# atom501/v-img

Measured on AMD Instinct MI355X. Metric: Mrays/sec (primary+secondary) at 512 spp, higher is better.
Workload: dtype f32; 1 GPU; disney_spheres.json, mis integrator, 512 spp, 1800x800; integrator=mis, spp=512, depth=unbounded, bvh=sweep SAH (host)

## Files before the change

v-img_amd/csrc/device_scene.h:

```cpp
#pragma once
#include <hip/hip_runtime.h>
#include <stdint.h>

#include "../../include/vimg_scene.h"
#include "material_record.h"

namespace vimg {

#define VIMG_GLOBAL __attribute__((address_space(1)))
#define VIMG_LDS __attribute__((address_space(3)))
template <typename T>
using gptr = const VIMG_GLOBAL T*;
typedef float v4f __attribute__((ext_vector_type(4)));
typedef uint32_t v2u __attribute__((ext_vector_type(2)));
typedef uint32_t v4u __attribute__((ext_vector_type(4)));

struct __attribute__((aligned(16))) DNode {
  v4f a;
  v4f b;
  v4f c;
  uint32_t left_ref, right_ref, pad0, pad1;
};
static_assert(sizeof(DNode) == 64, "DNode must be one 64-byte line");

struct __attribute__((aligned(16))) DLeafPrim {
  v4f a, b;
  float c0;
  uint32_t prim;
  uint32_t kind;
  uint32_t cls;
};
static_assert(sizeof(DLeafPrim) == 48, "DLeafPrim must be 48 bytes");

struct __attribute__((aligned(16))) DTriShade {
  float p[9];
  uint32_t mesh;
  uint32_t i0, i1, i2;
  float n[3];
};
static_assert(sizeof(DTriShade) == 64, "DTriShade must be 64 bytes");

struct __attribute__((aligned(16))) DLight {
  v4f a, b, c, d;
  uint32_t kind, index, pad0, pad1;
};
static_assert(sizeof(DLight) == 80, "DLight must be 80 bytes");

struct DScene {
  float cam_to_world[16];
  float p_size0, p_size1;
  float cone_spread;
  float aperture_radius, focal_dist;
  int32_t res_x, res_y;

  float root_min[3], root_max[3];
  uint32_t num_nodes, max_depth;
  uint32_t root_ref;
  gptr<DNode> nodes;
  gptr<DLeafPrim> leaf_prims;

  gptr<VimgPrim> prims;
  gptr<DTriShade> tri_shade;
  gptr<float> tri_area_pdf;
  gptr<VimgMesh> meshes;
  gptr<float> normals;
  gptr<float> uvs;
  gptr<VimgSphere> spheres;
  gptr<VimgMaterial> materials;
  gptr<uint32_t> material_flags;
  gptr<DMaterial> dmaterials;
  gptr<VimgTexture> textures;
  gptr<float> texels;
  gptr<VimgTextureRG> rg_textures;
  gptr<float> rg_texels;
  gptr<VimgLight> lights;
  gptr<DLight> dlights;
  uint32_t num_lights;
  gptr<float> cdf_pool;
  VimgBackground background;
  uint32_t background_emissive;
};

enum : uint32_t {
  MATF_NEEDS_UV = 1u,
  MATF_NEEDS_FRAME = 2u,
};

struct RenderArgs {
  uint32_t integrator, samples, depth;
  uint32_t tile_rank, tile_world;
  uint32_t tiles_x, tiles_y;
  uint32_t num_local_tiles;
  uint32_t full_stats;
  uint32_t stack_entries;
  uint32_t lds_nodes;
  uint32_t stack_lds;
  VIMG_GLOBAL uint32_t* stack_ovf;
  VIMG_GLOBAL v4u* pool_cold;
  uint32_t lds_leaf;
  VIMG_GLOBAL v4u* pool_state;
  uint32_t pool_segments;
  uint32_t pool_seg_len;
  uint32_t pool_epoch;
  uint32_t pool_slots;
  uint32_t pool_refill;
  uint32_t pool_vbatch;
  uint32_t pool_boxmin;
  uint32_t pool_starve;
  uint32_t pool_gbreak;
  uint32_t pool_classes;
  uint32_t cu_walkers;
  uint32_t cu_flex;
  uint32_t cu_lowwater;
  uint32_t cu_patience;
  uint32_t cu_join;
  uint32_t cu_sleep;
  uint32_t cu_watchdog;
  uint32_t cu_magic_v, cu_shift_v;
  uint32_t cu_magic_w, cu_shift_w;
  int32_t single_x, single_y;
  uint32_t sample_base;
  float spp_div;
  const VIMG_GLOBAL v4u* prog_in;
  VIMG_GLOBAL v4u* prog_out;
  const VIMG_GLOBAL uint32_t* item_list;
  uint32_t item_count;
};

struct DeviceStats {
  unsigned long long closest, shadow, internal, leaf, prim, sphere, nan_samples;
  unsigned long long trip_descend, trip_prim, iterations;
  unsigned long long prof[28];
  unsigned long long wait_cyc[5], wait_n[5];
  unsigned long long px_done[3];
  unsigned long long px_hops[3];
  unsigned long long ray_cyc[2];
  unsigned long long pv_cyc[7];
  unsigned long long walk_cyc[4];
};

}
```

v-img_amd/csrc/hip_internal.h:

```cpp
#pragma once
#include <hip/hip_runtime.h>

#include <algorithm>
#include <string>
#include <utility>
#include <vector>

#include "../../include/vimg_hip.h"
#include "device_mem.h"
#include "device_scene.h"
#include "kernel_tus.h"

#pragma GCC visibility push(hidden)
struct VimgDeviceScene {
  vimg::DScene d{};
  vimg::DevBuf nodes, leaf_prims;
  vimg::DevBuf chain_leaf;
  std::vector<vimg::DevBuf> tables;
  size_t total_bytes = 0;
  bool textured = false;
  VimgHipOptions opt{};
  int waves_per_simd = 2;
  bool too_wide = false;
  bool force_general = false;
  uint32_t num_cus = 0;
  uint32_t num_leaf_prims = 0;
  vimg::DevBuf stats;
  vimg::DevBuf counter;
  vimg::DevBuf root_box;
  vimg::DevBuf frame;
  vimg::DevBuf pool_cold;
  vimg::DevBuf stack_ovf;
  vimg::DevBuf pool_state;
  uint32_t pool_epoch = 0;
  uint64_t generation = 0;
  uint32_t num_vertices = 0, num_tris = 0, num_spheres = 0;
  std::vector<std::pair<uint32_t, uint32_t>> normal_rows;
  uint32_t n_internal = 0;
  uint32_t n_chain = 0;
  std::vector<uint32_t> level_begin;
  std::vector<VimgMaterial> materials;
  std::vector<VimgTexture> textures;
  std::vector<VimgLight> lights;
  uint32_t num_rg_textures = 0;
  uint64_t num_texels = 0, num_cdf = 0;
  size_t lights_table = 0, dlights_table = 0, dmaterials_table = 0;
  int query_launch = -1;
  bool query_ready = false;
  vimg::RenderArgs query_args{};
  uint32_t query_lds = 0;
  uint32_t query_per_cu[3] = {0, 0, 0};
};

struct VimgProgressive {
  VimgDeviceScene* scene = nullptr;
  VimgRenderParams params{};
  uint64_t items = 0;
  vimg::DevBuf rec[2];
  int cur = 0;
  uint32_t samples = 0;
  vimg::DevBuf scratch;
  uint64_t generation = 0;
  bool uniform = true;
  uint64_t valid_items = 0;
  uint64_t launches = 0;
  vimg::DevBuf item_list;
  vimg::DevBuf block_counts;
  vimg::DevBuf ctl;
};

namespace vimg {

extern hipStream_t g_stream;
extern int g_device;
inline hipStream_t stream_of(void* stream) { return stream ? static_cast<hipStream_t>(stream) : g_stream; }

inline uint32_t tiles_of(int n) { return (static_cast<uint32_t>(n) + 7u) / 8u; }
uint32_t local_tiles(const VimgDeviceScene* s, const VimgRenderParams* p);
inline bool is_feature_integrator(uint32_t i) { return i >= VIMG_INTEGRATOR_ALBEDO && i <= VIMG_INTEGRATOR_COVERAGE; }
inline uint32_t opt_or(int32_t v, uint32_t dflt) { return v == VIMG_OPT_AUTO ? dflt : static_cast<uint32_t>(v); }

struct LaunchCfg {
  RenderArgs args;
  uint32_t grid, lds_bytes;
  int sched;
  int wps;
  bool deep;
  int cu_waves;
  bool feature;
  size_t cold_bytes;
  size_t ovf_bytes;
};

struct DeviceTree {
  DevBuf nodes, bb, obj_indices;
  uint32_t num_nodes = 0, max_depth = 0;
  std::vector<uint32_t> level_internal;
};
int build_tree_device(uint32_t builder , uint32_t n, const float* d_bounds6, DeviceTree* out);

int validate_materials(const VimgMaterial* materials, uint32_t num_materials, const VimgTexture* textures, uint32_t num_textures,
                       uint32_t num_rg_textures);
int validate_lights(const VimgLight* lights, uint32_t num_lights, uint32_t num_prims);
bool tables_textured(const VimgMaterial* materials, uint32_t num_materials, const VimgTexture* textures, const VimgBackground& bg);
bool background_is_emissive(const VimgBackground& bg);

struct RelightPlan {
  bool any = false;
  DevBuf new_lights, new_dlights;
  DevBuf new_dmaterials;
  DevBuf sin_elev, lum, row_int, row_tot;
  std::vector<float> sin_table;
};
int check_relight(const VimgDeviceScene* s, const VimgGeometryUpdate* u);
int prepare_relight(const VimgDeviceScene* s, const VimgGeometryUpdate* u, RelightPlan* plan);
int enqueue_relight(VimgDeviceScene* s, const VimgGeometryUpdate* u, RelightPlan* plan, hipStream_t st);
void commit_relight(VimgDeviceScene* s, const VimgGeometryUpdate* u, RelightPlan* plan);
int enqueue_material_bake(const DScene& d, uint32_t num_materials, DMaterial* out, hipStream_t st);

struct EnvCdfScratch {
  float* sin_elev;
  float* lum;
  float* row_int;
  float* row_tot;
};
void enqueue_mip_levels(float* texels, const uint64_t* level_offset, uint32_t levels, uint32_t w, uint32_t h, uint32_t wrap_u,
                        uint32_t wrap_v, hipStream_t st);
std::vector<float> env_sin_table(uint32_t h);
void enqueue_env_cdfs(const float* img, uint32_t w, uint32_t h, const EnvCdfScratch& t, float* row_cdf, float* col_cdfs, hipStream_t st);

struct ProgLaunch {
  uint32_t base;
  const void* in;
  void* out;
  const uint32_t* item_list = nullptr;
  uint32_t item_count = 0;
  bool keep_stats = false;
};
int check_params(const VimgDeviceScene* s, const VimgRenderParams* p);
int check_render(const VimgDeviceScene* s, const VimgRenderParams* p, const void* d_out);
struct RenderLaunch {
  float* d_out;
  hipStream_t st;
  bool stats = false;
  int sx = -1, sy = -1;
  hipEvent_t ev0 = nullptr, ev1 = nullptr;
  const ProgLaunch* prog = nullptr;
};
int enqueue_render(VimgDeviceScene* s, const VimgRenderParams* p, const RenderLaunch& r);
int check_kernel_error(VimgDeviceScene* s);
uint64_t fetch_shard_pixels(const VimgDeviceScene* s, const VimgRenderParams* p);
int fetch_stats(VimgDeviceScene* s, const VimgRenderParams* p, VimgRenderStats* out);

LaunchCfg make_launch(const VimgDeviceScene* s, const VimgRenderParams* p, int sx, int sy);
LaunchCfg make_launch_lane(const VimgDeviceScene* s, const VimgRenderParams* p, int sx, int sy);
LaunchCfg make_launch_feature(const VimgDeviceScene* s, const VimgRenderParams* p, int sx, int sy);
RenderArgs base_args(const VimgDeviceScene* s, const VimgRenderParams* p, int sx, int sy);
uint32_t segments_for(const VimgDeviceScene* s, const VimgRenderParams* p, uint64_t items, uint64_t in_flight,
                      double per_gen, double most, RenderArgs* a);
const void* kernel_of(const VimgDeviceScene* s, const LaunchCfg& c);
const void* launched_kernel_of(const VimgDeviceScene* s, const LaunchCfg& c, bool stats);
bool plain_launch_serves(const VimgDeviceScene* s, const LaunchCfg& c, bool stats);

}
#pragma GCC visibility pop
```

v-img_amd/csrc/launch_policy.hip:

```cpp
#include <cmath>

#include "hip_internal.h"
#include "render_cu_kernel.h"

namespace vimg {

uint32_t local_tiles(const VimgDeviceScene* s, const VimgRenderParams* p) {
  const uint32_t total = tiles_of(s->d.res_x) * tiles_of(s->d.res_y);
  if (p->tile_rank >= total) return 0;
  return (total - p->tile_rank + p->tile_world - 1) / p->tile_world;
}

RenderArgs base_args(const VimgDeviceScene* s, const VimgRenderParams* p, int sx, int sy) {
  const VimgHipOptions& o = s->opt;
  RenderArgs a{};
  a.integrator = p->integrator;
  a.samples = p->samples;
  a.spp_div = static_cast<float>(p->samples);
  a.depth = p->depth;
  a.tile_rank = p->tile_rank;
  a.tile_world = p->tile_world;
  a.tiles_x = tiles_of(s->d.res_x);
  a.tiles_y = tiles_of(s->d.res_y);
  a.num_local_tiles = local_tiles(s, p);
  a.full_stats = 0;
  a.single_x = sx;
  a.single_y = sy;
  a.stack_entries = s->d.max_depth + 2;
  a.stack_ovf = nullptr;
  a.pool_refill = 16u;
  a.pool_vbatch = std::min(64u, std::max(1u, opt_or(o.pool_vbatch, 64u)));
  a.pool_boxmin = std::min(64u, opt_or(o.pool_boxmin, 16u));
  a.pool_segments = 1;
  a.pool_seg_len = p->samples;
  return a;
}

uint32_t segments_for(const VimgDeviceScene* s, const VimgRenderParams* p, uint64_t items, uint64_t in_flight,
                      double per_gen, double most, RenderArgs* a) {
  const double gens = double(items) / double(in_flight);
  uint32_t k = gens >= 10.0 ? 1u : uint32_t(std::min(most, std::max(1.0, std::floor(per_gen / gens + 0.5))));
  k = std::min<uint32_t>(k, std::max<uint32_t>(p->samples / 4u, 1u));
  if (items * 2u < in_flight * 3u) k = 1u;
  if (s->opt.pool_segments != VIMG_OPT_AUTO) k = uint32_t(std::max(1, s->opt.pool_segments));
  k = std::min<uint32_t>(k, 4096u);
  while (k > 1u && items * k >= 0xfff00000ull) --k;
  const uint32_t len = std::max<uint32_t>((p->samples + k - 1) / k, 1u);
  a->pool_seg_len = len;
  a->pool_segments = std::max<uint32_t>((p->samples + len - 1) / len, 1u);
  return len;
}

namespace {

CuKernel pick_cu_kernel(const VimgDeviceScene* s, bool deep, int nw, bool diag = false, bool early = false, bool plain = false) {
  if (plain) return early ? vimg_cu_kernel_plain_early() : vimg_cu_kernel_plain();
  return diag ? vimg_cu_kernel_diag(s->textured, deep, nw)
              : (early ? vimg_cu_kernel_early(s->textured, deep, nw) : vimg_cu_kernel(s->textured, deep, nw));
}

void magic_div(uint32_t d, uint32_t* magic, uint32_t* shift) {
  uint32_t l = 0;
  while ((1ull << l) < d) ++l;
  *magic = static_cast<uint32_t>((1ull << (31u + l)) / d + 1ull);
  *shift = l - 1u;
}

LaunchCfg make_launch_cu(const VimgDeviceScene* s, const VimgRenderParams* p, int sx, int sy) {
  LaunchCfg c{};
  const VimgHipOptions& o = s->opt;
  const uint64_t items = (sx >= 0) ? 1 : uint64_t(local_tiles(s, p)) * 64u;
  c.sched = VIMG_SCHED_CU;
  c.wps = 4;
  c.cu_waves = 16;
  const uint32_t nw = uint32_t(c.cu_waves);
  RenderArgs& a = c.args = base_args(s, p, sx, sy);
  a.stack_lds = std::min(a.stack_entries, std::max(1u, opt_or(o.lds_stack, 32u)));
  a.cu_walkers = 0;
  a.cu_flex = opt_or(o.cu_flex, 1u);
  a.cu_lowwater = std::max(1u, opt_or(o.cu_lowwater, 64u));
  a.cu_patience = opt_or(o.cu_patience, 4u);
  a.cu_join = std::max(1u, opt_or(o.cu_join, 1u));
  a.cu_sleep = std::min(127u, std::max(1u, opt_or(o.cu_sleep, 4u)));
  a.pool_starve = std::min(64u, std::max(1u, opt_or(o.pool_starve, 16u)));
  a.pool_classes = std::min(3u, std::max(1u, opt_or(o.pool_classes, 3u)));
  const uint32_t share = (160u * 1024u) / (16u / nw) - 1024u;
  uint32_t node_budget = 4608u;
  if (o.lds_budget_kb != VIMG_OPT_AUTO) node_budget = uint32_t(std::max(1, o.lds_budget_kb)) * 1024u;
  a.lds_nodes = std::min(node_budget / 56u, s->d.num_nodes);
  const uint32_t node_bytes = (a.lds_nodes * 56u + 255u) & ~255u;
  c.deep = a.lds_nodes < s->d.num_nodes || a.stack_lds < a.stack_entries;
  a.cu_walkers = std::min(nw, std::max(1u, opt_or(o.cu_walkers, c.deep ? 10u : 9u)));
  a.pool_refill = std::max(1u, opt_or(o.pool_refill, c.deep ? 2u : 16u));
  const uint32_t stack_rows = cu_stack_rows_of(a.stack_entries, a.stack_lds);
  uint32_t leaf_bytes = 0;
  a.lds_leaf = 0;
  if (s->num_leaf_prims * 48u <= 4096u && o.lds_leaf != 0) {
    a.lds_leaf = s->num_leaf_prims;
    leaf_bytes = a.lds_leaf * 48u;
  }
  auto slots_with = [&](uint32_t walkers) {
    const uint32_t fixed = node_bytes + walkers * stack_rows * 256u + cu_pool_bytes(0, nw) + leaf_bytes + 64u;
    uint32_t n = share > fixed ? (share - fixed) / CU_LDS_BYTES : 0u;
    n = std::min(n, 4096u);
    if (!c.deep && o.pool_slots == VIMG_OPT_AUTO) n = std::min(n, 1280u);
    if (o.pool_slots != VIMG_OPT_AUTO) n = std::min(n, uint32_t(std::max(0, o.pool_slots)));
    return n;
  };
  const uint32_t groups = s->num_cus * (16u / nw);
  const uint64_t per_group = (items + groups - 1) / groups;
  if (o.cu_walkers == VIMG_OPT_AUTO && !c.deep && o.pool_slots == VIMG_OPT_AUTO && per_group + 8u <= slots_with(nw)) a.cu_walkers = nw;
  if (a.cu_walkers == nw) a.cu_flex |= 1u;
  const uint32_t stack_bytes = a.cu_walkers * stack_rows * 256u;
  uint32_t slots = slots_with(a.cu_walkers);
  if (o.pool_slots == VIMG_OPT_AUTO && per_group > slots && per_group * 10u < uint64_t(slots) * 27u)
    slots = static_cast<uint32_t>(per_group * 10u / 27u);
  slots = static_cast<uint32_t>(std::min<uint64_t>(slots, per_group + 8u));
  slots = std::max(slots & ~7u, 8u);
  if (o.cu_flex == VIMG_OPT_AUTO && (c.deep || per_group * 10u <= uint64_t(slots) * 30u)) a.cu_flex |= 32u;
  if (c.deep && o.pool_boxmin == VIMG_OPT_AUTO && per_group + 8u >= slots && per_group <= slots) a.pool_boxmin = 8u;
  a.pool_slots = slots;
  magic_div(slots, &a.cu_magic_v, &a.cu_shift_v);
  magic_div(2u * slots, &a.cu_magic_w, &a.cu_shift_w);
  c.lds_bytes = node_bytes + stack_bytes + cu_pool_bytes(slots, nw) + leaf_bytes;
  int per_cu = 0;
  hipError_t oe = hipOccupancyMaxActiveBlocksPerMultiprocessor(&per_cu, launched_kernel_of(s, c, false), int(nw * 64u), c.lds_bytes);
  if (oe != hipSuccess || per_cu < 1) per_cu = 1;
  per_cu = std::min<int>(per_cu, int(16u / nw));
  const uint64_t need_blocks = (items + slots - 1) / slots;
  c.grid = static_cast<uint32_t>(std::max<uint64_t>(1, std::min<uint64_t>(need_blocks, uint64_t(s->num_cus) * per_cu)));
  a.cu_watchdog = static_cast<uint32_t>(1000000000ull >> 20);
  if (sx < 0) {
    const uint32_t len = segments_for(s, p, items, uint64_t(c.grid) * slots, 176.0, 64.0, &a);
    a.cu_watchdog = static_cast<uint32_t>(std::min<uint64_t>((1000000000ull + 5000000ull * len) >> 20, 0x7fffffffull));
  }
  return c;
}

void cu_scratch(const VimgDeviceScene* s, LaunchCfg& c) {
  const RenderArgs& a = c.args;
  c.cold_bytes = size_t(c.grid) * cu_cold_records(s->textured) * a.pool_slots * 16u;
  if (a.stack_lds < a.stack_entries)
    c.ovf_bytes = size_t(c.grid) * a.cu_walkers * (a.stack_entries - a.stack_lds) * 256u;
}

}

const void* kernel_of(const VimgDeviceScene* s, const LaunchCfg& c) {
  if (c.feature) return reinterpret_cast<const void*>(vimg_feature_kernel(s->textured));
  if (c.sched == VIMG_SCHED_CU) return reinterpret_cast<const void*>(pick_cu_kernel(s, c.deep, c.cu_waves));
  return reinterpret_cast<const void*>(vimg_lane_kernel(s->textured, c.wps));
}

bool plain_launch_serves(const VimgDeviceScene* s, const LaunchCfg& c, bool stats) {
  return plain_build_serves(plain_launch_of(c.sched == VIMG_SCHED_CU, s->textured, c.deep, c.cu_waves, stats, s->force_general, c.args));
}

const void* launched_kernel_of(const VimgDeviceScene* s, const LaunchCfg& c, bool stats) {
  if (c.sched != VIMG_SCHED_CU) return kernel_of(s, c);
  return reinterpret_cast<const void*>(pick_cu_kernel(s, c.deep, c.cu_waves, stats, (c.args.cu_flex & 32u) != 0u,
                                                      plain_launch_serves(s, c, stats)));
}

namespace {

LaunchCfg lane_shaped_launch(const VimgDeviceScene* s, const VimgRenderParams* p, int sx, int sy, bool feature) {
  LaunchCfg c{};
  c.feature = feature;
  const VimgHipOptions& o = s->opt;
  const uint64_t items = (sx >= 0) ? 1 : uint64_t(local_tiles(s, p)) * 64u;
  c.sched = VIMG_SCHED_LANE;
  c.wps = s->waves_per_simd;
  if (o.waves_per_simd != VIMG_OPT_AUTO) c.wps = o.waves_per_simd >= 3 ? 3 : 2;
  RenderArgs& a = c.args = base_args(s, p, sx, sy);
  a.stack_lds = a.stack_entries;
  const uint32_t stack_bytes = 4u * a.stack_entries * 64u * 4u;
  uint32_t budget = 40u * 1024u;
  if (o.lds_budget_kb != VIMG_OPT_AUTO) budget = uint32_t(std::max(1, o.lds_budget_kb)) * 1024u;
  uint32_t nodes = 0;
  if (stack_bytes + 512 < budget) nodes = (budget - stack_bytes - 256) / 56u;
  a.lds_nodes = std::min(nodes, s->d.num_nodes);
  c.lds_bytes = ((a.lds_nodes * 56u + 255u) & ~255u) + stack_bytes;
  int per_cu = 0;
  hipError_t oe = hipOccupancyMaxActiveBlocksPerMultiprocessor(&per_cu, kernel_of(s, c), 256, c.lds_bytes);
  if (oe != hipSuccess || per_cu < 1) per_cu = 1;
  const uint64_t need_blocks = (items + 255) / 256;
  c.grid = static_cast<uint32_t>(
      std::max<uint64_t>(1, std::min<uint64_t>(need_blocks, uint64_t(s->num_cus) * per_cu)));
  return c;
}

}

LaunchCfg make_launch_lane(const VimgDeviceScene* s, const VimgRenderParams* p, int sx, int sy) {
  return lane_shaped_launch(s, p, sx, sy, false);
}

LaunchCfg make_launch_feature(const VimgDeviceScene* s, const VimgRenderParams* p, int sx, int sy) {
  return lane_shaped_launch(s, p, sx, sy, true);
}

LaunchCfg make_launch(const VimgDeviceScene* s, const VimgRenderParams* p, int sx, int sy) {
  if (is_feature_integrator(p->integrator)) return make_launch_feature(s, p, sx, sy);
  if (s->too_wide || s->opt.scheduler == VIMG_SCHED_LANE) return make_launch_lane(s, p, sx, sy);
  LaunchCfg c = make_launch_cu(s, p, sx, sy);
  cu_scratch(s, c);
  return c;
}

}

using namespace vimg;

extern "C" {

const char* vimg_hip_launch_kernel(const VimgDeviceScene* s, const VimgRenderParams* p) {
  if (!s || !p) return "";
  static const char* lane_names[2][2] = {{"render_kernel<false,2>", "render_kernel<false,3>"},
                                         {"render_kernel<true,2>", "render_kernel<true,3>"}};
  static const char* cu_names[2][2] = {{"render_cu_kernel<false>", "render_cu_kernel<false,deep>"},
                                       {"render_cu_kernel<true>", "render_cu_kernel<true,deep>"}};
  if (p->tile_world == 0 || p->tile_rank >= p->tile_world) return "";
  if (is_feature_integrator(p->integrator)) return s->textured ? "feature_kernel<true>" : "feature_kernel<false>";
  const LaunchCfg c = make_launch(s, p, -1, -1);
  if (c.sched == VIMG_SCHED_CU && !s->textured && !c.deep && !plain_launch_serves(s, c, false)) return "render_cu_kernel<false,general>";
  if (c.sched == VIMG_SCHED_CU) return cu_names[s->textured ? 1 : 0][c.deep ? 1 : 0];
  return lane_names[s->textured ? 1 : 0][c.wps >= 3 ? 1 : 0];
}

const char* vimg_hip_scene_kernel(const VimgDeviceScene* s) {
  const VimgRenderParams whole{VIMG_INTEGRATOR_MIS, 64, 1, 0, 1};
  return vimg_hip_launch_kernel(s, &whole);
}

}
```

v-img_amd/csrc/plain_build.h:

```cpp
#pragma once
#include <cstdint>

namespace vimg {

enum : uint32_t {
  PF_INTEGRATOR = 1u,
  PF_CLASSES = 2u,
  PF_LEAF_LDS = 4u,
  PF_SINGLE = 8u,
  PF_ITEMS = 16u,
  PF_FLEX = 32u,
};
#ifdef VIMG_PLAIN_FOLD
constexpr uint32_t PLAIN_FOLD = VIMG_PLAIN_FOLD;
#else
constexpr uint32_t PLAIN_FOLD = PF_INTEGRATOR | PF_CLASSES | PF_LEAF_LDS | PF_SINGLE | PF_ITEMS | PF_FLEX;
#endif

struct PlainLaunch {
  bool cu_sched;
  bool textured, deep;
  int cu_waves;
  bool stats;
  bool force_general;
  uint32_t integrator, pool_classes, lds_leaf, cu_flex;
  int single_x;
  bool has_item_list;
};
constexpr uint32_t PLAIN_INTEGRATOR_MIS = 3u;
constexpr uint32_t PLAIN_FLEX_DEFAULT = 1u;

constexpr bool plain_build_serves(const PlainLaunch& l, uint32_t fold = PLAIN_FOLD) {
  if (l.force_general || !l.cu_sched || l.textured || l.deep || l.cu_waves != 16 || l.stats) return false;
  if ((fold & PF_INTEGRATOR) && l.integrator != PLAIN_INTEGRATOR_MIS) return false;
  if ((fold & PF_CLASSES) && l.pool_classes != 3u) return false;
  if ((fold & PF_LEAF_LDS) && l.lds_leaf == 0u) return false;
  if ((fold & PF_SINGLE) && l.single_x >= 0) return false;
  if ((fold & PF_ITEMS) && l.has_item_list) return false;
  if ((fold & PF_FLEX) && (l.cu_flex & ~32u) != PLAIN_FLEX_DEFAULT) return false;
  return true;
}

template <class Args>
constexpr PlainLaunch plain_launch_of(bool cu_sched, bool textured, bool deep, int cu_waves, bool stats, bool force_general,
                                      const Args& a) {
  return PlainLaunch{cu_sched, textured, deep, cu_waves, stats || a.full_stats != 0u, force_general,
                     a.integrator, a.pool_classes, a.lds_leaf, a.cu_flex, a.single_x, a.item_list != nullptr};
}

}
```

v-img_amd/csrc/render_cu_kernel.h:

```cpp
#pragma once
#include <type_traits>

#include "plain_build.h"
#include "render_kernels.h"

namespace vimg {

enum : uint32_t {
  SC_THROUGHPUT = 0,
  SC_RESULT,
  SC_NEE,
  SC4_RNG,
  SC4_MAIN
};
__host__ __device__ constexpr uint32_t cu_cold_records(bool tex) { return SC4_MAIN + 1u + (tex ? 1u : 0u); }
__host__ __device__ constexpr uint32_t cu_stack_rows_of(uint32_t entries, uint32_t in_lds) { return in_lds < entries ? in_lds + 1u : entries; }
constexpr uint32_t SLOT_IDLE = 0xffffffffu;

VD void state_store(VIMG_GLOBAL uint32_t* p, uint32_t v) {
  __hip_atomic_store(p, v, __ATOMIC_RELAXED, __HIP_MEMORY_SCOPE_AGENT);
}
VD uint32_t state_load(VIMG_GLOBAL uint32_t* p) {
  return __hip_atomic_load(p, __ATOMIC_RELAXED, __HIP_MEMORY_SCOPE_AGENT);
}
VD uint32_t lane_rank(unsigned long long mask, uint32_t lane) {
  return __popcll(mask & ((1ull << lane) - 1ull));
}

enum : uint32_t {
  CF_PRIMARY = 1u, CF_NONSPEC = 2u, CF_HAS_S = 4u, CF_HAS_R = 8u, CF_OCCLUDED = 16u, CF_FOUND = 32u,
  CF_FRESH = 64u, CF_KIND_SPHERE = 128u, CF_DONE_S = 256u, CF_DONE_R = 512u,
  CF_CLS_SHIFT = 10u,
  CF_DONE_V = 4096u,
  CF_KILL_R = 8192u,
  CF_BOUNCE_SHIFT = 16u
};
enum : uint32_t {
  CR_ORG = 0,
  CR_DIR,
  CR_SHD,
  CR_HIT,
  CR_COUNT
};
constexpr uint32_t CU_EMPTY = 0xffffu;
constexpr uint32_t CU_RAY_S = 0x8000u;
constexpr uint32_t CQ_WALK = 4u, CQ_COUNT = 5u;
constexpr uint32_t CU_LDS_BYTES = CR_COUNT * 16u + 8u + 4u * 2u + 2u * 2u + 4u;

struct CuCtl {
  int32_t avail[8];
  uint32_t tail[CQ_COUNT], head[CQ_COUNT];
  uint32_t live;
  uint32_t pixels_left;
  uint32_t abort;
  uint32_t t0_lo, t0_hi;
  uint32_t pad[1];
};
static_assert(sizeof(CuCtl) == 96, "CuCtl layout");
struct CuWaveRec {
  unsigned long long cyc[6], nbatch[4], nslots[4];
  uint32_t internal, leaf, prim, sphere;
  unsigned long long box_pass, box_lanes, leaf_round, leaf_lanes, sessions, refills, refill_rays, pad;
  unsigned long long looks, q_sum[4];
  unsigned long long w_cyc[4];
  unsigned long long wait_cyc[5], wait_n[5];
  unsigned long long ray_cyc, ray_n;
  unsigned long long pv_cyc[6], pv_n;
};
static_assert(sizeof(CuWaveRec) == 416, "CuWaveRec layout");
__host__ __device__ constexpr uint32_t cu_pool_bytes(uint32_t slots, uint32_t waves) {
  return CU_LDS_BYTES * slots + uint32_t(sizeof(CuCtl)) + waves * uint32_t(sizeof(CuWaveRec));
}
VD uint32_t cu_mod(uint32_t n, uint32_t d, uint32_t magic, uint32_t shift) { return n - d * (__umulhi(n, magic) >> shift); }
VD int32_t lds_add_rtn(VIMG_LDS int32_t* p, int32_t v) { return __hip_atomic_fetch_add(p, v, __ATOMIC_RELAXED, __HIP_MEMORY_SCOPE_WORKGROUP); }
VD uint32_t lds_add_rtn(VIMG_LDS uint32_t* p, uint32_t v) { return __hip_atomic_fetch_add(p, v, __ATOMIC_RELAXED, __HIP_MEMORY_SCOPE_WORKGROUP); }
VD uint32_t lds_load(VIMG_LDS uint32_t* p) { return __hip_atomic_load(p, __ATOMIC_RELAXED, __HIP_MEMORY_SCOPE_WORKGROUP); }
VD int32_t lds_load(VIMG_LDS int32_t* p) { return __hip_atomic_load(p, __ATOMIC_RELAXED, __HIP_MEMORY_SCOPE_WORKGROUP); }
VD uint32_t cu_uni(uint32_t v) { return static_cast<uint32_t>(__builtin_amdgcn_readfirstlane(static_cast<int>(v))); }

static_assert(PLAIN_INTEGRATOR_MIS == uint32_t(VIMG_INTEGRATOR_MIS), "plain_build.h");
template <uint32_t PLAIN> VD uint32_t opt_integrator(const RenderArgs& A) {
  if constexpr (PLAIN & PF_INTEGRATOR) return uint32_t(VIMG_INTEGRATOR_MIS); else return A.integrator;
}
template <uint32_t PLAIN> VD uint32_t opt_classes(const RenderArgs& A) {
  if constexpr (PLAIN & PF_CLASSES) return 3u; else return A.pool_classes;
}
template <uint32_t PLAIN> VD bool opt_leaf_in_lds(const RenderArgs& A) {
  if constexpr (PLAIN & PF_LEAF_LDS) return true; else return A.lds_leaf != 0u;
}
template <uint32_t PLAIN> VD bool opt_single(const RenderArgs& A) {
  if constexpr (PLAIN & PF_SINGLE) return false; else return A.single_x >= 0;
}
template <uint32_t PLAIN> VD bool opt_has_items(const RenderArgs& A) {
  if constexpr (PLAIN & PF_ITEMS) return false; else return A.item_list != nullptr;
}
template <uint32_t PLAIN> VD uint32_t opt_flex(const RenderArgs& A) {
  if constexpr (PLAIN & PF_FLEX) return PLAIN_FLEX_DEFAULT; else return A.cu_flex;
}


struct CuKArgs {
  DScene g;
  RenderArgs A;
  float* out;
  DeviceStats* stats;
  unsigned int* work_counter;
};
typedef const __attribute__((address_space(4))) CuKArgs* CuKPtr;
VD CuKPtr cu_kargs() {
  unsigned long long p = reinterpret_cast<unsigned long long>(__builtin_amdgcn_kernarg_segment_ptr());
  asm volatile("" : "+s"(p));
  return (CuKPtr)p;
}

#define CU_STAGE_LOCALS(K)                                                                                              \
  extern __shared__ __attribute__((aligned(16))) unsigned char lds_raw[];                                               \
  [[maybe_unused]] const DScene& g = *(const DScene*)&(K)->g;                                                           \
  [[maybe_unused]] const RenderArgs& A = *(const RenderArgs*)&(K)->A;                                                   \
  [[maybe_unused]] float* __restrict__ out = (K)->out;                                                                  \
  [[maybe_unused]] unsigned int* __restrict__ work_counter = (K)->work_counter;                                         \
  [[maybe_unused]] const uint32_t lane = threadIdx.x & 63, wave = cu_uni(threadIdx.x >> 6);                             \
  [[maybe_unused]] const bool full_stats = DIAG && A.full_stats != 0;    \
  [[maybe_unused]] const uint32_t stat_inc = full_stats ? 1u : 0u;                                                      \
  [[maybe_unused]] const uint32_t W = static_cast<uint32_t>(g.res_x), H = static_cast<uint32_t>(g.res_y);               \
  [[maybe_unused]] const bool single = opt_single<PLAIN>(A);                                                            \
  [[maybe_unused]] const uint32_t total_items =                                                                         \
      single ? 1u : (opt_has_items<PLAIN>(A) ? A.item_count : A.num_local_tiles * 64u);                                 \
  [[maybe_unused]] const uint32_t n_seg = A.pool_segments, seg_len = A.pool_seg_len;                                    \
  [[maybe_unused]] const uint32_t total_claims = total_items * n_seg;                                                   \
  [[maybe_unused]] constexpr uint32_t roulette_threshold = 5;                                                           \
  [[maybe_unused]] const bool material_mode = (opt_integrator<PLAIN>(A) == VIMG_INTEGRATOR_MATERIAL);                   \
  [[maybe_unused]] const uint32_t P = A.pool_slots;                                                                     \
  [[maybe_unused]] const bool can_walk = wave < A.cu_walkers;                                                           \
  const uint32_t stack_rows_ = cu_stack_rows_of(A.stack_entries, A.stack_lds);                                          \
  const uint32_t node_bytes_ = (lds_node_bytes(A.lds_nodes) + 255u) & ~255u;                                            \
  [[maybe_unused]] VIMG_LDS uint32_t* stack0 =                                                                          \
      reinterpret_cast<VIMG_LDS uint32_t*>((VIMG_LDS unsigned char*)lds_raw + node_bytes_) +                            \
      size_t(can_walk ? wave : 0u) * stack_rows_ * 64u + lane;                                                          \
  VIMG_LDS unsigned char* base_ = (VIMG_LDS unsigned char*)lds_raw + node_bytes_ + A.cu_walkers * stack_rows_ * 256u;   \
  [[maybe_unused]] VIMG_LDS v4u* recs = reinterpret_cast<VIMG_LDS v4u*>(base_);                                         \
  [[maybe_unused]] VIMG_LDS v2u* hitx = reinterpret_cast<VIMG_LDS v2u*>(recs + CR_COUNT * P);                           \
  [[maybe_unused]] VIMG_LDS uint16_t* ring_v = reinterpret_cast<VIMG_LDS uint16_t*>(hitx + P);                          \
  [[maybe_unused]] VIMG_LDS uint16_t* ring_w = ring_v + 4u * P;                                                         \
  [[maybe_unused]] VIMG_LDS uint32_t* tq = reinterpret_cast<VIMG_LDS uint32_t*>(ring_w + 2u * P);                       \
  [[maybe_unused]] VIMG_LDS CuCtl* G = reinterpret_cast<VIMG_LDS CuCtl*>(tq + P);                                       \
  [[maybe_unused]] VIMG_LDS CuWaveRec* wrec = reinterpret_cast<VIMG_LDS CuWaveRec*>(G + 1) + wave;                      \
  [[maybe_unused]] VIMG_LDS v4f* lds_leaf = reinterpret_cast<VIMG_LDS v4f*>(reinterpret_cast<VIMG_LDS CuWaveRec*>(G + 1) + NW); \
  [[maybe_unused]] VIMG_LDS uint32_t* recw = reinterpret_cast<VIMG_LDS uint32_t*>(recs);                                \
  [[maybe_unused]] auto rd = [&](uint32_t r, uint32_t slot) -> v4u { return recs[r * P + slot]; };                      \
  [[maybe_unused]] auto wr = [&](uint32_t r, uint32_t slot, v4u v) { recs[r * P + slot] = v; };                         \
  [[maybe_unused]] auto flag_word = [&](uint32_t slot) -> VIMG_LDS uint32_t* { return recw + (CR_DIR * P + slot) * 4u + 3u; }; \
  [[maybe_unused]] auto fu = [](float f) { return __float_as_uint(f); };                                                \
  [[maybe_unused]] auto uf = [](uint32_t u) { return __uint_as_float(u); };                                             \
  [[maybe_unused]] auto mod_v = [&](uint32_t t) { return cu_mod(t, P, A.cu_magic_v, A.cu_shift_v); };                   \
  [[maybe_unused]] auto mod_w = [&](uint32_t t) { return cu_mod(t, 2u * P, A.cu_magic_w, A.cu_shift_w); };              \
  [[maybe_unused]] auto ring_at = [&](uint32_t q, uint32_t t) -> VIMG_LDS uint16_t* {                                   \
    return q >= CQ_WALK ? ring_w + mod_w(t) : ring_v + q * P + mod_v(t);                                                \
  };                                                                                                                    \
  [[maybe_unused]] const bool leaf_in_lds = opt_leaf_in_lds<PLAIN>(A);                                                  \
  [[maybe_unused]] const uint32_t box_min = A.pool_boxmin;                                                              \
                                                  \
  [[maybe_unused]] VIMG_GLOBAL v4u* cold = A.pool_cold + size_t(blockIdx.x) * (size_t(cu_cold_records(TEX)) * P);       \
  [[maybe_unused]] VIMG_GLOBAL v4u* cold_acc = cold + size_t(SC4_MAIN) * P;                                             \
  [[maybe_unused]] VIMG_GLOBAL v4u* cold_cone = cold_acc + P;                                                           \
  [[maybe_unused]] auto crd = [&](uint32_t r, uint32_t slot) -> v4u { return cold[slot * SC4_MAIN + r]; };              \
  [[maybe_unused]] auto cwr = [&](uint32_t r, uint32_t slot, v4u v) { cold[slot * SC4_MAIN + r] = v; };                 \
                          \
  [[maybe_unused]] auto raise = [&](uint32_t bit) {                                                                     \
    atomicOr(work_counter + 1, bit);                                                                                    \
    __hip_atomic_store(&G->abort, 1u, __ATOMIC_RELAXED, __HIP_MEMORY_SCOPE_WORKGROUP);                                  \
  };                                                                                                                    \
                                                         \
  [[maybe_unused]] auto push = [&](uint32_t q, unsigned long long mask, uint32_t entry) {                               \
    const uint32_t n_ = static_cast<uint32_t>(__popcll(mask));                                                          \
    if (n_ == 0u) return;                                                                                               \
    uint32_t t_ = 0;                                                                                                    \
    if (lane == 0) {                                                                                                    \
      t_ = lds_add_rtn(&G->tail[q], n_);                                                                                \
      if (t_ > 0x7ff00000u) raise(8u);                   \
    }                                                                                                                   \
    t_ = cu_uni(t_);                                                                                                    \
    if ((mask >> lane) & 1ull) *ring_at(q, t_ + lane_rank(mask, lane)) = static_cast<uint16_t>(entry);                  \
    __builtin_amdgcn_fence(__ATOMIC_RELEASE, "workgroup");                                                              \
    if (lane == 0) lds_add_rtn(&G->avail[q], static_cast<int32_t>(n_));                                                 \
  };                                                                                                                    \
                                         \
  [[maybe_unused]] auto slot_complete = [&](uint32_t nw) -> bool {                                                      \
    return (nw & CF_DONE_V) && (!(nw & CF_HAS_S) || (nw & CF_DONE_S)) && (!(nw & CF_HAS_R) || (nw & CF_DONE_R));        \
  };                                                                                                                    \
    \
  [[maybe_unused]] auto hand_to_vertex = [&](bool complete, uint32_t nw, uint32_t slot_) {                              \
    uint32_t cls_ = 0;                                                                                                  \
    if (complete && (nw & CF_FOUND) && !(nw & CF_KILL_R) && opt_integrator<PLAIN>(A) >= VIMG_INTEGRATOR_MATERIAL) {     \
      cls_ = (nw >> CF_CLS_SHIFT) & 3u;                                                                                 \
      if (cls_ == 0 && material_mode) cls_ = 3;                            \
      if (cls_ != 0) {                                                                                                  \
        if (opt_classes<PLAIN>(A) == 1) cls_ = 1;                                                                       \
        else if (opt_classes<PLAIN>(A) == 2) cls_ = (cls_ == 2) ? 2u : 1u;                                              \
      }                                                                                                                 \
    }                                                                                                                   \
    const unsigned long long m0_ = __ballot(complete && cls_ == 0), m1_ = __ballot(complete && cls_ == 1),              \
                             m2_ = __ballot(complete && cls_ == 2), m3_ = __ballot(complete && cls_ == 3);              \
    if ((m0_ | m1_ | m2_ | m3_) == 0ull) return;                                                                        \
    const uint32_t n_me_ = static_cast<uint32_t>(__popcll(lane == 0 ? m0_ : (lane == 1 ? m1_ : (lane == 2 ? m2_ : m3_)))); \
    uint32_t t_me_ = 0;                                                                                                 \
    if (lane < 4u && n_me_ != 0u) {                                                                                     \
      t_me_ = lds_add_rtn(&G->tail[lane], n_me_);                                                                       \
      if (t_me_ > 0x7ff00000u) raise(8u);                                                                               \
    }                                                                                                                   \
    const uint32_t t0_ = __shfl(t_me_, 0), t1_ = __shfl(t_me_, 1), t2_ = __shfl(t_me_, 2), t3_ = __shfl(t_me_, 3);      \
    if (complete) {                                                                                                     \
      const uint32_t tt_ = cls_ == 0 ? t0_ : (cls_ == 1 ? t1_ : (cls_ == 2 ? t2_ : t3_));                               \
      const unsigned long long mm_ = cls_ == 0 ? m0_ : (cls_ == 1 ? m1_ : (cls_ == 2 ? m2_ : m3_));                     \
      *ring_at(cls_, tt_ + lane_rank(mm_, lane)) = static_cast<uint16_t>(slot_);                                        \
      if (full_stats) tq[slot_] = static_cast<uint32_t>(__builtin_readcyclecounter());                                  \
    }                                                                                                                   \
    __builtin_amdgcn_fence(__ATOMIC_RELEASE, "workgroup");                                                              \
    if (lane < 4u && n_me_ != 0u) lds_add_rtn(&G->avail[lane], static_cast<int32_t>(n_me_));                            \
  };                                                                                                                    \
                     \
  [[maybe_unused]] auto push_rays = [&](bool is_s, bool is_r, uint32_t slot_) {                                         \
    const unsigned long long ms_ = __ballot(is_s), mr_ = __ballot(is_r);                                                \
    const uint32_t n_s_ = static_cast<uint32_t>(__popcll(ms_)), n_r_ = static_cast<uint32_t>(__popcll(mr_));            \
    if (n_s_ + n_r_ == 0u) return;                                                                                      \
    uint32_t t_ = 0;                                                                                                    \
    if (lane == 0) {                                                                                                    \
      t_ = lds_add_rtn(&G->tail[CQ_WALK], n_s_ + n_r_);                                                                 \
      if (t_ > 0x7ff00000u) raise(8u);                                                                                  \
    }                                                                                                                   \
    t_ = cu_uni(t_);                                                                                                    \
    if (is_s) *ring_at(CQ_WALK, t_ + lane_rank(ms_, lane)) = static_cast<uint16_t>(slot_ | CU_RAY_S);                   \
// ... 41 lines not shown
VD void cu_vertex(uint32_t n, uint32_t slot, bool& all_pending, uint32_t& n_nan, uint32_t& n_dead) {
  const CuKPtr K = cu_kargs();
  CU_STAGE_LOCALS(K);
  constexpr bool finisher_batch = FIN;
  constexpr bool CAN_SPLIT = !FIN && MTC != int(VIMG_MAT_LAMBERTIAN);
  const bool split = CAN_SPLIT && n <= 32u && !(opt_flex<PLAIN>(A) & 16u);
  const bool mirror = split && lane >= 32u;
  if (split) slot = static_cast<uint32_t>(__shfl(static_cast<int>(slot), static_cast<int>(lane & 31u)));
  const bool on = (split ? (lane & 31u) : lane) < n;
  if (!on) slot = 0u;
  const v4u r_ray = on ? rd(CR_DIR, slot) : v4u{0u, 0u, 0u, 0u};
  uint32_t flags = r_ray.w;
  const bool fresh = on && (flags & CF_FRESH);
  const bool have = on && !fresh;
  uint32_t px = 0, py = 0, smp = 0, item = 0, bounce = 0;
  Rng rng{0};
  f3 acc{0.f, 0.f, 0.f}, ray_o{0.f, 0.f, 0.f}, ray_d{0.f, 0.f, 1.f};
  f3 throughput{1.f, 1.f, 1.f}, result{0.f, 0.f, 0.f};
  RayCone cone{0.f, 0.f};
  float eta_scale = 1.f, prev_pdf = 0.f;
  bool primary = true, non_specular_bounce = false;
  v4u r_origin{0u, 0u, 0u, 0u}, r_hit{0u, 0u, 0u, 0u}, r_nee{0u, 0u, 0u, 0u};
  v2u r_hx{0u, 0u};
  constexpr bool PV = DIAG && MTC == int(VIMG_MAT_PRINCIPLED);
  [[maybe_unused]] unsigned long long pv_t = PV ? __builtin_readcyclecounter() : 0ull;
  [[maybe_unused]] auto pv_lap = [&](int k) {
    if constexpr (PV) {
      if (full_stats) {
        const unsigned long long now = __builtin_readcyclecounter();
        if (lane == 0) wrec->pv_cyc[k] += now - pv_t;
        pv_t = now;
      }
    }
  };
  uint32_t hops = 0;
  if (full_stats && have) hops = recw[(CR_SHD * P + slot) * 4u + 3u] + 1u;
  if (have) {
    const v4u r_t = crd(SC_THROUGHPUT, slot), r_r = crd(SC_RESULT, slot);
    v4u r_a{0u, 0u, 0u, 0u};
    if (finisher_batch) r_a = cold_acc[slot];
    if (r_ray.w & CF_HAS_S) r_nee = crd(SC_NEE, slot);
    r_origin = rd(CR_ORG, slot);
    r_hit = rd(CR_HIT, slot);
    r_hx = hitx[slot];
    const v4u r_g = crd(SC4_RNG, slot);
    px = r_g.z & 0xffffu, py = r_g.z >> 16;
    smp = r_g.w;
    item = r_a.w;
    rng.s = uint64_t(r_g.x) | (uint64_t(r_g.y) << 32);
    acc = f3{uf(r_a.x), uf(r_a.y), uf(r_a.z)};
    ray_o = f3{uf(r_origin.x), uf(r_origin.y), uf(r_origin.z)};
    ray_d = f3{uf(r_ray.x), uf(r_ray.y), uf(r_ray.z)};
    throughput = f3{uf(r_t.x), uf(r_t.y), uf(r_t.z)};
    result = f3{uf(r_r.x), uf(r_r.y), uf(r_r.z)};
    eta_scale = uf(r_t.w);
    prev_pdf = uf(r_r.w);
    bounce = flags >> CF_BOUNCE_SHIFT;
    primary = (flags & CF_PRIMARY) != 0;
    non_specular_bounce = (flags & CF_NONSPEC) != 0;
    if constexpr (TEX) {
      const v4u r_c = cold_cone[slot];
      cone = RayCone{uf(r_c.x), uf(r_c.y)};
    }
  }

  pv_lap(0);
  bool finish = false, at_vertex = false;
  Hit hit;
  hit.p = f3{0.f, 0.f, 0.f};
  if (have) {
    if ((flags & CF_HAS_S) && !(flags & CF_OCCLUDED))
      result = result + f3{uf(r_nee.x), uf(r_nee.y), uf(r_nee.z)};
    if (!(flags & CF_HAS_R) || (flags & CF_KILL_R)) {
      finish = true;
    } else {
      const bool hit_any = (flags & CF_FOUND) != 0;
      if (hit_any) {
        HitRec hr;
        hr.e0 = uf(r_hit.x), hr.e1 = uf(r_hit.y), hr.e2 = uf(r_hit.z);
        hr.inv_det = uf(r_hit.w);
        hr.prim = r_hx.x;
        hr.kind = (flags & CF_KIND_SPHERE) ? 1u : 0u;
        TravRay tr{ray_o, ray_d, 0.0001f, uf(r_hx.y)};
        make_hit_info<TEX>(g, hr, tr, hit);
      }
      if (material_mode) {
        if (!hit_any) {
          result = throughput * background_emit<TEX>(g, ray_d, cone);
          finish = true;
        } else {
          at_vertex = true;
        }
      } else if (opt_integrator<PLAIN>(A) != VIMG_INTEGRATOR_MIS) {
        if (hit_any) {
          f3 nn = (opt_integrator<PLAIN>(A) == VIMG_INTEGRATOR_G_NORMAL) ? hit.ng : hit.ns;
          result = (nn + 1.0f) / 2.0f;
        } else {
          f3 unit_dir = normalize(ray_d);
          float a = 0.5 * (unit_dir.y + 1.0);
          result = (1.0f - a) * f3{1.0f, 1.0f, 1.0f} + a * f3{0.5f, 0.7f, 1.0f};
        }
        finish = true;
      } else if (primary) {
        if (!hit_any) {
          result = background_emit<TEX>(g, ray_d, cone);
          finish = true;
        } else {
          gptr<VimgMaterial> m = g.materials + hit.mat;
          if (m->type == VIMG_MAT_DIFFUSE_LIGHT) {
            result = mat_emitted(m, ray_d, hit.ns);
            finish = true;
          } else {
            bounce = 0;
            at_vertex = true;
          }
        }
      } else {
        if (hit_any) {
          gptr<VimgMaterial> m = g.materials + hit.mat;
          if (m->type == VIMG_MAT_DIFFUSE_LIGHT) {
            const f3 le = mat_emitted(m, ray_d, hit.ns);
            if (prev_pdf != 0) {
              float light_pdf = surf_pdf(g, hit.prim, ray_o, hit.p, ray_d) / g.num_lights;
              float Gt = geometric_term(ray_o, hit.p, hit.ng);
              float mis_weight = balance_heuristic(prev_pdf * Gt, light_pdf);
              result = result + throughput * mis_weight * le;
            } else {
              result = result + throughput * le;
            }
            finish = true;
          } else {
            bool survive = true;
            if (bounce > roulette_threshold) {
              float rr = static_cast<float>(pcg_next(rng)) / 4294967296.0f;
              f3 rr_t = (1.f / eta_scale) * throughput;
              float max_val = sel_min(sel_max(sel_max(rr_t.x, rr_t.y), rr_t.z), 0.95f);
              if (rr > max_val)
                survive = false;
              else
                throughput = throughput / max_val;
            }
            if (survive) {
              bounce += 1;
              at_vertex = true;
            } else {
              finish = true;
            }
          }
        } else {
          if (prev_pdf != 0 && g.background_emissive) {
            float light_pdf = background_pdf<TEX>(g, ray_d) / g.num_lights;
            float mis_weight = balance_heuristic(prev_pdf, light_pdf);
            result = result + throughput * mis_weight * background_emit<TEX>(g, ray_d, cone);
          }
          finish = true;
        }
      }
      if (at_vertex && !(bounce < A.depth)) {
        at_vertex = false;
        finish = true;
      }
    }
  }

  pv_lap(1);
  if constexpr (!finisher_batch) {
    if (have && !mirror) {
      VIMG_GLOBAL uint32_t* rw = reinterpret_cast<VIMG_GLOBAL uint32_t*>(cold + (slot * SC4_MAIN + SC_RESULT));
      rw[0] = fu(result.x), rw[1] = fu(result.y), rw[2] = fu(result.z);
    }
  }
  bool has_s = false, has_r = false;
  bool early = false, pushed_r = false;
  bool rec_written = false;
  f3 shadow_d{0.f, 0.f, 1.f}, nee_contrib{0.f, 0.f, 0.f};
  float shadow_max_t = 0.f;
  if constexpr (!finisher_batch) {
    if (material_mode && at_vertex) {
      gptr<VimgMaterial> m = g.materials + hit.mat;
      const f3 emitted_col = mat_emitted(m, ray_d, hit.ns);
      Scatter sc = sample_mat<TEX>(g, hit, ray_d, rng, non_specular_bounce);
      if (!sc.valid) {
        result = throughput * emitted_col;
        finish = true;
      } else {
        if (!sc.is_specular) non_specular_bounce = true;
        if constexpr (TEX) {
          const float hd = length(ray_o - hit.p);
          const float ssa = spread_angle_from_curvature(hit.curvature, cone.cone_width, ray_d, hit.ns);
          if (sc.eta != 0.f)
            cone = propagate_refract_cone(cone, ray_d, ssa, sc.eta, sc.wo);
          else
            cone = propagate_reflect_cone(cone, ssa * 2.f, hd);
        }
        if (sc.eta != 0.f) eta_scale /= (sc.eta * sc.eta);
        f3 fdiv{0.f, 0.f, 0.f};
        const uint32_t type = m->type;
        if (type == VIMG_MAT_LAMBERTIAN) {
          fdiv = col_at_ray_hit<TEX>(g, m->tex, ray_d, cone, hit);
        } else if (type == VIMG_MAT_DIELECTRIC) {
          fdiv = splat3(1.f);
        } else if (type == VIMG_MAT_PRINCIPLED) {
          f3 f;
          float pdf;
          principled_eval_pdf<TEX>(g, m, ray_d, sc.wo, hit, cone, non_specular_bounce, f, pdf);
          fdiv = f / pdf;
        }
        throughput = throughput * (emitted_col + fdiv);
        bool survive = true;
        if (bounce > roulette_threshold) {
          float rr = static_cast<float>(pcg_next(rng)) / 4294967296.0f;
          f3 rr_t = (1.f / eta_scale) * throughput;
          float max_val = sel_min(sel_max(sel_max(rr_t.x, rr_t.y), rr_t.z), 0.95f);
          if (rr > max_val)
            survive = false;
          else
            throughput = throughput / max_val;
        }
        bounce += 1;
        if (!survive || !(bounce < A.depth)) {
          result = f3{0.f, 0.f, 0.f};
          finish = true;
        } else {
          ray_o = hit.p;
          ray_d = sc.wo;
          primary = false;
          has_r = true;
        }
      }
      at_vertex = false;
    }
    constexpr int MT = MTC;
    constexpr bool LAMB = MT == int(VIMG_MAT_LAMBERTIAN);
    constexpr bool LIGHT_FIRST = EARLY == 0 && LAMB;
    const bool early_on = EARLY == 2 ? (A.cu_flex & 32u) != 0u : (EARLY == 1);
    uint32_t mat_type = 0u;
    float hit_dist = 0.f, surface_spread_angle = 0.f;
    f3 light_col{0.f, 0.f, 0.f};
    EmitterInfo li{f3{0.f, 0.f, 1.f}, 0.f, 0.f, 0.f};
    bool nee = false, reg_before = false;
    RayCone nee_cone = cone;
    Scatter sc = no_scatter();
    Rng rng_l{0};
    if (at_vertex) {
      mat_type = MT >= 0 ? uint32_t(MT) : g.materials[hit.mat].type;
      if constexpr (TEX) {
        hit_dist = length(ray_o - hit.p);
        surface_spread_angle = spread_angle_from_curvature(hit.curvature, cone.cone_width, ray_d, hit.ns);
      }
      reg_before = non_specular_bounce;
      if constexpr (LIGHT_FIRST) {
        lights_sample<TEX>(g, hit.p, rng, light_col, li);
        nee = (li.pdf != 0.f);
      } else {
        rng_l = rng;
        if (mat_type != VIMG_MAT_DIELECTRIC) pcg_skip6(rng);
      }
      sc = sample_mat<TEX, MT>(g, hit, ray_d, rng, reg_before);
      if constexpr (TEX) nee_cone = propagate_reflect_cone(cone, surface_spread_angle * 2.f, hit_dist);
      if (sc.valid) {
        if (!sc.is_specular) non_specular_bounce = true;
        if (sc.eta != 0.f) {
          eta_scale /= (sc.eta * sc.eta);
          if constexpr (TEX) cone = propagate_refract_cone(cone, ray_d, surface_spread_angle, sc.eta, sc.wo);
        } else {
          if constexpr (TEX) cone = nee_cone;
        }
      }
    }
    early = early_on && at_vertex && !mirror;
    pushed_r = early && sc.valid;
    rec_written = at_vertex && !mirror;
    if (rec_written) {
      wr(CR_ORG, slot, v4u{fu(hit.p.x), fu(hit.p.y), fu(hit.p.z), 0u});
      wr(CR_DIR, slot, v4u{fu(sc.wo.x), fu(sc.wo.y), fu(sc.wo.z),
                           (sc.valid ? CF_HAS_R : 0u) | (non_specular_bounce ? CF_NONSPEC : 0u) | (bounce << CF_BOUNCE_SHIFT)});
      if (full_stats && early) tq[slot] = static_cast<uint32_t>(__builtin_readcyclecounter());
    }
    if (early_on) push_rays(false, pushed_r, slot);
    pv_lap(3);
    if constexpr (!LIGHT_FIRST) {
      if (at_vertex && mat_type != VIMG_MAT_DIELECTRIC) {
        lights_sample<TEX>(g, hit.p, rng_l, light_col, li);
        nee = (li.pdf != 0.f);
      }
    }
    if (rec_written && nee) {
      recw[(CR_ORG * P + slot) * 4u + 3u] = fu(li.dist - 0.0001f);
      wr(CR_SHD, slot, v4u{fu(li.wi.x), fu(li.wi.y), fu(li.wi.z), hops});
      if (early) __hip_atomic_fetch_or(flag_word(slot), CF_HAS_S, __ATOMIC_RELEASE, __HIP_MEMORY_SCOPE_WORKGROUP);
    } else if (rec_written && full_stats) {
      recw[(CR_SHD * P + slot) * 4u + 3u] = hops;
    }
    if (early_on) push_rays(early && nee, false, slot);
    pv_lap(2);
    if (at_vertex) {
      f3 f_l{0.f, 0.f, 0.f}, f_s{0.f, 0.f, 0.f};
      float pdf_l = 0.f, pdf_s = 0.f;
      if constexpr (LAMB) {
        if (nee || sc.valid) {
          gptr<DMaterial> dm = g.dmaterials + hit.mat;
          const f3 col = (dm->bits & DMAT_COLOUR) ? load3(dm->base)
                                                  : col_at_ray_hit<TEX>(g, g.materials[hit.mat].tex, ray_d, nee_cone, hit);
          const float cos_l = sel_max(0.0f, dot(li.wi, hit.ns)), cos_s = sel_max(0.0f, dot(sc.wo, hit.ns));
          const float dp_l = static_cast<float>(cos_l / kPi), dp_s = static_cast<float>(cos_s / kPi);
          if (nee) f_l = col * dp_l, pdf_l = dp_l;
          if (sc.valid) f_s = col * dp_s, pdf_s = dp_s;
        }
      } else {
#pragma unroll 1
        for (int pass = 0; pass < (split ? 1 : 2); ++pass) {
          const bool second = split ? mirror : (pass == 1);
          const bool run = second ? sc.valid : nee;
          f3 f{0.f, 0.f, 0.f};
          float pdf = 0.f;
          if (run) {
            const v4u w4 = rd(second ? CR_DIR : CR_SHD, slot);
            const f3 wo{uf(w4.x), uf(w4.y), uf(w4.z)};
            const RayCone c = second ? cone : nee_cone;
            const bool reg = second ? non_specular_bounce : reg_before;
            eval_pdf_pair<TEX, MT>(g, hit, ray_d, wo, c, reg, f, pdf);
          }
          if (second) f_s = f, pdf_s = pdf;
          else f_l = f, pdf_l = pdf;
        }
      }
      pv_lap(4);
      if (split) {
        const float sx = __shfl_xor(f_s.x, 32), sy = __shfl_xor(f_s.y, 32), sz = __shfl_xor(f_s.z, 32), sp = __shfl_xor(pdf_s, 32);
        if (!mirror) f_s = f3{sx, sy, sz}, pdf_s = sp;
      }
      if (nee) {
        if (pdf_l != 0 && !is_nan(pdf_l)) {
          float Gt = li.G;
          float mis_weight = balance_heuristic(li.pdf, pdf_l * Gt);
          nee_contrib = throughput * f_l * mis_weight * Gt * light_col / li.pdf;
        }
      }
      if (sc.valid) {
        if (is_nan(pdf_s)) {
          sc.valid = false;
        } else {
          throughput = throughput * (f_s / pdf_s);
          prev_pdf = pdf_s;
        }
      }
      has_s = nee;
      has_r = sc.valid;
      primary = false;
      if (!has_s && !has_r) finish = true;
    }
  }

  bool need_pixel = fresh;
  bool retire = false;
  bool have_claim = fresh && (flags & CF_PRIMARY);
  uint32_t claim = have_claim ? crd(SC4_RNG, slot).w : 0u;
  bool pending = false;
  if constexpr (!finisher_batch) {
    if (finish) has_s = false, has_r = false;
    all_pending = false;
  } else {
    bool pixels_left = cu_uni(lds_load(&G->pixels_left)) != 0u;
    bool is_nan_sample = false;
    if (finish) {
      is_nan_sample = is_nan(result.x) || is_nan(result.y) || is_nan(result.z);
      acc = acc + result;
      smp += 1;
      if (smp == A.samples) {
        const f3 px_col = acc / A.spp_div;
        if (A.prog_out) {
          A.prog_out[size_t(item) * 2u] = v4u{static_cast<uint32_t>(rng.s), static_cast<uint32_t>(rng.s >> 32), 0u, 0u};
          A.prog_out[size_t(item) * 2u + 1u] = v4u{fu(acc.x), fu(acc.y), fu(acc.z), 0u};
        }
        size_t o;
        if (single)
          o = 0;
        else if (A.tile_world == 1)
          o = (size_t(px) + size_t(H - 1 - py) * W) * 3;
        else
          o = size_t(item) * 3;
        out[o + 0] = px_col.x;
        out[o + 1] = px_col.y;
        out[o + 2] = px_col.z;
        need_pixel = true;
        if (full_stats) {
          const unsigned long long dt = __builtin_amdgcn_s_memrealtime() - (static_cast<unsigned long long>(G->t0_lo) | (static_cast<unsigned long long>(G->t0_hi) << 32));
          DeviceStats* __restrict__ stp = K->stats;
          if (stp) {
            atomicAdd(&stp->px_done[0], dt), atomicAdd(&stp->px_done[1], 1ull), atomicMax(&stp->px_done[2], dt);
            atomicMax(&stp->px_hops[2], (dt << 24) | static_cast<unsigned long long>(hops & 0xffffffu));
            atomicAdd(&stp->px_hops[0], static_cast<unsigned long long>(hops)), atomicMax(&stp->px_hops[1], static_cast<unsigned long long>(hops));
          }
          hops = 0;
        }
      } else if (n_seg > 1u && smp % seg_len == 0u) {
        VIMG_GLOBAL uint32_t* st = reinterpret_cast<VIMG_GLOBAL uint32_t*>(A.pool_state + size_t(item) * 2u);
        state_store(st + 0, static_cast<uint32_t>(rng.s));
        state_store(st + 1, static_cast<uint32_t>(rng.s >> 32));
        state_store(st + 4, fu(acc.x));
        state_store(st + 5, fu(acc.y));
        state_store(st + 6, fu(acc.z));
        __builtin_amdgcn_fence(__ATOMIC_RELEASE, "workgroup");
        __builtin_amdgcn_s_waitcnt(0x0F70);
// ... 314 lines not shown
          }
          ray.max_t = hit ? t : ray.max_t;
          w_found = w_found || hit;
          const bool keep_rec = hit && !w_any;
          rec.e0 = keep_rec ? e0 : rec.e0, rec.e1 = keep_rec ? e1 : rec.e1;
          rec.e2 = keep_rec ? e2 : rec.e2, rec.inv_det = keep_rec ? idet : rec.inv_det;
          rec.prim = keep_rec ? lp_prim : rec.prim;
          rec.kind = keep_rec ? kind : rec.kind;
          w_cls = keep_rec ? lp_cls : w_cls;
          stop = hit && w_any;
        }
        const uint32_t sp_below = sp != 0 ? sp - 1 : 0u;
        uint32_t popped = stack0[(DEEP ? (sp_below < S ? sp_below : S) : sp_below) * 64];
        if constexpr (DEEP) {
          if (!stop && sp_below >= S) popped = ovf0[(sp_below - S) * 64];
        }
        cur = (stop || sp == 0) ? REF_DONE : popped;
        sp = sp_below;
      }
      wlap(wc2);
      const uint32_t n_fin = static_cast<uint32_t>(__popcll(__ballot(w_slot != SLOT_IDLE && cur == REF_DONE)));
      const uint32_t n_act = static_cast<uint32_t>(__popcll(__ballot(w_slot != SLOT_IDLE && cur != REF_DONE)));
      if (n_act == 0 || n_fin >= A.pool_refill) break;
    }

    {
      const bool done = w_slot != SLOT_IDLE && cur == REF_DONE;
      bool complete = false;
      uint32_t nw = 0;
      if (done) {
        uint32_t orv;
        if (w_type == 0u) {
          orv = CF_DONE_S | (w_found ? CF_OCCLUDED : 0u);
        } else {
          orv = CF_DONE_R;
          if (w_found) {
            orv |= CF_FOUND | (rec.kind == 1 ? CF_KIND_SPHERE : 0u) | (w_cls << CF_CLS_SHIFT);
            wr(CR_HIT, w_slot, v4u{fu(rec.e0), fu(rec.e1), fu(rec.e2), fu(rec.inv_det)});
            hitx[w_slot] = v2u{rec.prim, fu(ray.max_t)};
          }
        }
        nw = __hip_atomic_fetch_or(flag_word(w_slot), orv, __ATOMIC_ACQ_REL, __HIP_MEMORY_SCOPE_WORKGROUP) | orv;
        complete = slot_complete(nw);
      }
      if (__any(done)) {
        hand_to_vertex(complete, nw, w_slot);
        if (full_stats && done) d_rayc += static_cast<unsigned long long>(static_cast<uint32_t>(__builtin_readcyclecounter()) - t_in), d_rayn += 1u;
        if (done) w_slot = SLOT_IDLE;
      }
    }
    wlap(wc3);
    if (cu_uni(lds_load(&G->abort)) != 0u) break;
  }
  if (full_stats) {
    if (lane == 0) wrec->w_cyc[0] += wc0, wrec->w_cyc[1] += wc1, wrec->w_cyc[2] += wc2, wrec->w_cyc[3] += wc3;
    auto wsum = [](unsigned long long v) {
      for (int o = 32; o; o >>= 1) v += __shfl_xor(v, o);
      return v;
    };
    const unsigned long long s_int = wsum(c_internal), s_leaf = wsum(c_leaf), s_prim = wsum(c_prim), s_sph = wsum(c_sphere);
    const unsigned long long s_wc = wsum(d_waitc), s_wn = wsum(d_waitn), s_rc = wsum(d_rayc), s_rn = wsum(d_rayn);
    if (lane == 0) {
      wrec->internal += static_cast<uint32_t>(s_int), wrec->leaf += static_cast<uint32_t>(s_leaf);
      wrec->prim += static_cast<uint32_t>(s_prim), wrec->sphere += static_cast<uint32_t>(s_sph);
      wrec->wait_cyc[4] += s_wc, wrec->wait_n[4] += s_wn, wrec->ray_cyc += s_rc, wrec->ray_n += s_rn;
    }
    if (lane == 0) {
      wrec->box_pass += d_box, wrec->box_lanes += d_boxl, wrec->leaf_round += d_leaf, wrec->leaf_lanes += d_leafl;
      wrec->sessions += 1, wrec->refills += d_ref, wrec->refill_rays += d_refr;
    }
  }
}

template <bool TEX, bool DEEP, int NW, int WPS, bool DIAG, int EARLY, uint32_t PLAIN = 0u>
__global__ void __launch_bounds__(NW * 64, WPS)
render_cu_kernel(const CuKArgs ka) {
  {
    const CuKPtr K = cu_kargs();
    CU_STAGE_LOCALS(K);
    stage_lds(g, A, (VIMG_LDS unsigned char*)lds_raw);
    for (uint32_t i = lane; i < sizeof(CuWaveRec) / 4u; i += 64u) reinterpret_cast<VIMG_LDS uint32_t*>(wrec)[i] = 0u;
    for (uint32_t i = threadIdx.x; i < A.lds_leaf * 3u; i += blockDim.x)
      lds_leaf[i] = reinterpret_cast<gptr<v4f>>(g.leaf_prims)[i];
    for (uint32_t s = threadIdx.x; s < P; s += blockDim.x) {
      recw[(CR_DIR * P + s) * 4u + 3u] = CF_FRESH;
      ring_v[s] = static_cast<uint16_t>(s);
      ring_v[P + s] = CU_EMPTY, ring_v[2u * P + s] = CU_EMPTY, ring_v[3u * P + s] = CU_EMPTY;
      ring_w[s] = CU_EMPTY, ring_w[P + s] = CU_EMPTY;
      tq[s] = static_cast<uint32_t>(__builtin_readcyclecounter());
    }
    if (threadIdx.x == 0) {
      for (uint32_t q = 0; q < 8u; ++q) G->avail[q] = (q == 0u) ? static_cast<int32_t>(P) : 0;
      G->live = P, G->pixels_left = 1u, G->abort = 0u;
      for (uint32_t q = 0; q < CQ_COUNT; ++q) G->tail[q] = (q == 0u) ? P : 0u, G->head[q] = 0u;
      const unsigned long long t0 = __builtin_amdgcn_s_memrealtime();
      G->t0_lo = static_cast<uint32_t>(t0), G->t0_hi = static_cast<uint32_t>(t0 >> 32);
    }
    __syncthreads();
  }
  uint32_t n_closest = 0, n_shadow = 0, n_nan = 0, iter_wave = 0;
  uint32_t n_dead = 0;
  unsigned long long t_mark = __builtin_readcyclecounter();
  bool skip_fin = false;
  uint32_t polls = 0;
  unsigned long long idle_since = 0;
  for (;;) {
    const CuKPtr K = cu_kargs();
    CU_STAGE_LOCALS(K);
    auto lap = [&](uint32_t k) {
      if (full_stats) {
        const unsigned long long now = __builtin_readcyclecounter();
        if (lane == 0) wrec->cyc[k] += now - t_mark;
        t_mark = now;
      }
    };
    if (cu_uni(lds_load(&G->abort)) != 0u) break;
    const v4u av4 = *reinterpret_cast<VIMG_LDS v4u*>(&G->avail[0]);
    const int32_t a0 = skip_fin ? 0 : static_cast<int32_t>(cu_uni(av4.x)), a1 = static_cast<int32_t>(cu_uni(av4.y)),
                  a2 = static_cast<int32_t>(cu_uni(av4.z)), a3 = static_cast<int32_t>(cu_uni(av4.w));
    const int32_t aw = static_cast<int32_t>(cu_uni(static_cast<uint32_t>(lds_load(&G->avail[CQ_WALK]))));
    const int32_t m01 = a0 > a1 ? a0 : a1, m23 = a2 > a3 ? a2 : a3, qmax = m01 > m23 ? m01 : m23;
    if (full_stats && lane == 0) {
      wrec->looks += 1;
      wrec->q_sum[0] += static_cast<uint32_t>(a0 > 0 ? a0 : 0), wrec->q_sum[1] += static_cast<uint32_t>(a1 > 0 ? a1 : 0);
      wrec->q_sum[2] += static_cast<uint32_t>(a2 > 0 ? a2 : 0), wrec->q_sum[3] += static_cast<uint32_t>(aw > 0 ? aw : 0);
    }
    if (can_walk && aw > 0 && (aw >= static_cast<int32_t>(A.cu_join) || polls >= A.cu_patience)) {
      lap(5);
      skip_fin = false, polls = 0, idle_since = 0;
      if (full_stats) iter_wave++;
      if (opt_flex<PLAIN>(A) & 4u) __builtin_amdgcn_s_setprio(1);
      cu_walk<TEX, DEEP, NW, DIAG, PLAIN>(n_closest, n_shadow);
      if (opt_flex<PLAIN>(A) & 4u) __builtin_amdgcn_s_setprio(0);
      lap(4);
      continue;
    }
    const bool may_shade = !can_walk || (opt_flex<PLAIN>(A) & 1u);
    const bool run = may_shade && qmax > 0 &&
                     (qmax >= static_cast<int32_t>(A.pool_vbatch) ||
                      (aw < static_cast<int32_t>(A.cu_lowwater) && (qmax >= static_cast<int32_t>(A.pool_starve) || polls >= A.cu_patience)));
    if (run) {
      const uint32_t cls = (a0 == qmax) ? 0u : (a1 == qmax ? 1u : (a2 == qmax ? 2u : 3u));
      const uint32_t want = qmax < 64 ? static_cast<uint32_t>(qmax) : 64u;
      uint32_t e = 0;
      const uint32_t n = pop(cls, want, ~0ull, e);
      if (n == 0u) continue;
      lap(5);
      if (full_stats) iter_wave++;
      if (full_stats && lane == 0) wrec->nbatch[cls] += 1, wrec->nslots[cls] += n;
      if (full_stats) {
        unsigned long long w = lane < n ? static_cast<unsigned long long>(static_cast<uint32_t>(__builtin_readcyclecounter()) - tq[e]) : 0ull;
        for (int o = 32; o; o >>= 1) w += __shfl_xor(w, o);
        if (lane == 0) wrec->wait_cyc[cls] += w, wrec->wait_n[cls] += n;
      }
      bool all_pending = false;
      const bool by_class = opt_classes<PLAIN>(A) == 3u;
      if (opt_flex<PLAIN>(A) & 2u) __builtin_amdgcn_s_setprio(1);
      if (cls == 0u)
        cu_vertex<TEX, NW, DIAG, EARLY, true, -1, PLAIN>(n, e, all_pending, n_nan, n_dead);
      else if (cls == 1u && by_class)
        cu_vertex<TEX, NW, DIAG, EARLY, false, int(VIMG_MAT_LAMBERTIAN), PLAIN>(n, e, all_pending, n_nan, n_dead);
      else if (cls == 2u && by_class)
        cu_vertex<TEX, NW, DIAG, EARLY, false, int(VIMG_MAT_PRINCIPLED), PLAIN>(n, e, all_pending, n_nan, n_dead);
      else
        cu_vertex<TEX, NW, DIAG, EARLY, false, -1, PLAIN>(n, e, all_pending, n_nan, n_dead);
      if (opt_flex<PLAIN>(A) & 2u) __builtin_amdgcn_s_setprio(0);
// ... 58 lines not shown
```

v-img_amd/csrc/render_kernels.h:

```cpp
#pragma once
#include "device_math.h"
#include "device_scene.h"
#include "material_terms.h"

namespace vimg {


struct Rng {
  uint64_t s;
};
VD uint32_t pcg_next(Rng& r) {
  uint64_t old = r.s;
  r.s = old * 6364136223846793005ULL + 1ULL;
  uint32_t xorshifted = static_cast<uint32_t>(((old >> 18u) ^ old) >> 27u);
  uint32_t rot = static_cast<uint32_t>(old >> 59u);
  return (xorshifted >> rot) | (xorshifted << ((0u - rot) & 31u));
}
VD void pcg_seed(Rng& r, uint64_t initstate) {
  r.s = 0;
  pcg_next(r);
  r.s += initstate;
  pcg_next(r);
}
constexpr uint64_t kPcgA = 6364136223846793005ULL;
constexpr uint64_t pcg_a_pow(int n) { uint64_t r = 1; for (int i = 0; i < n; ++i) r *= kPcgA; return r; }
constexpr uint64_t pcg_c_sum(int n) { uint64_t r = 0; for (int i = 0; i < n; ++i) r += pcg_a_pow(i); return r; }
constexpr uint64_t pcg_step_n(uint64_t s, int n) { for (int i = 0; i < n; ++i) s = s * kPcgA + 1ULL; return s; }
static_assert(pcg_step_n(0x853c49e6748fea9bULL, 6) == 0x853c49e6748fea9bULL * pcg_a_pow(6) + pcg_c_sum(6), "six LCG steps in one");
VD void pcg_skip6(Rng& r) { r.s = r.s * pcg_a_pow(6) + pcg_c_sum(6); }
VD float rand_float(Rng& r) {
  uint64_t r1 = pcg_next(r);
  uint64_t r2 = pcg_next(r);
  uint64_t u = (r1 << 32) | r2;
  uint32_t z = (u == 0) ? 64u : static_cast<uint32_t>(__builtin_clzll(u));
  if (z <= 40) {
    uint32_t e = 126 - z;
    uint32_t m = static_cast<uint32_t>(u) & 0x7fffffu;
    return __uint_as_float((e << 23) | m);
  }
  return 0x1.0p-64f * static_cast<float>(static_cast<uint32_t>(u));
}
VD f2 random_x_y_r2(uint32_t n) {
  constexpr float g = 1.32471795724474602596;
  constexpr float a1 = 1.0 - (1.0 / g);
  constexpr float a2 = 1.0 - (1.0 / (g * g));
  float x = a1 * static_cast<float>(n);
  float y = a2 * static_cast<float>(n);
  return f2{x - __builtin_floorf(x), y - __builtin_floorf(y)};
}

VD f2 sample_disk(float rand1, float rand2) {
  float r = sqrt_f(rand1);
  float phi = 2.f * kPi * rand2;
  double sn, cs;
  D_sincos(phi, sn, cs);
  return f2{r * static_cast<float>(cs), r * static_cast<float>(sn)};
}
VD f3 sample_sphere(float rand1, float rand2) {
  float phi = 2 * kPi * rand1;
  float cos_theta = 2 * rand2 - 1;
  float sin_theta = static_cast<float>(__builtin_sqrt(static_cast<double>(1 - cos_theta * cos_theta)));
  double sn, cs;
  D_sincos(phi, sn, cs);
  float x = cs * sin_theta;
  float y = sn * sin_theta;
  return f3{x, y, cos_theta};
}
VD float std_lerp(float a, float b, float t) {
  if ((a <= 0 && b >= 0) || (a >= 0 && b <= 0)) return t * b + (1 - t) * a;
  if (t == 1) return b;
  const float x = a + t * (b - a);
  return (t > 1) == (b > a) ? (b < x ? x : b) : (b > x ? x : b);
}
VD f3 sample_sphere_cap(float rand1, float rand2, float cos_theta_max) {
  float phi = 2 * kPi * rand1;
  float cos_theta = std_lerp(cos_theta_max, 1.0f, rand2);
  float sin_theta = sqrt_f(1 - cos_theta * cos_theta);
  double sn, cs;
  D_sincos(phi, sn, cs);
  float x = cs * sin_theta;
  float y = sn * sin_theta;
  return f3{x, y, cos_theta};
}

struct RayCone {
  float cone_width, spread_angle;
// ... 372 lines not shown
  uint32_t cur = g.root_ref;
  bool found = false;
  const uint32_t stat_inc = full_stats ? 1u : 0u;
  auto box_loop = [&](auto exact_possible) {
    while (cur != REF_DONE && ref_count(cur) == 0) {
      v4f na, nb, nc;
      v2u refs;
      if (cur < L.n_nodes) {
        na = L.na[cur], nb = L.nb[cur], nc = L.nc[cur];
        refs = L.nm[cur];
      } else {
        gptr<DNode> n = g.nodes + cur;
        na = n->a, nb = n->b, nc = n->c;
        refs = v2u{n->left_ref, n->right_ref};
      }
      const uint32_t sp_below = sp != 0 ? sp - 1 : 0u;
      const uint32_t popped = L.stack[sp_below * 64];
      cnt.internal += stat_inc;
      float h1, h2;
      if (decltype(exact_possible)::value && exact_slab) {
        h1 = slab(f3{na.x, na.y, na.z}, f3{na.w, nb.x, nb.y}, ray.o, inv, ray.min_t, ray.max_t);
        h2 = slab(f3{nb.z, nb.w, nc.x}, f3{nc.y, nc.z, nc.w}, ray.o, inv, ray.min_t, ray.max_t);
      } else {
        h1 = slab_fast(f3{na.x, na.y, na.z}, f3{na.w, nb.x, nb.y}, ray.o, inv, ray.min_t, ray.max_t);
        h2 = slab_fast(f3{nb.z, nb.w, nc.x}, f3{nc.y, nc.z, nc.w}, ray.o, inv, ray.min_t, ray.max_t);
      }
      const bool in1 = !is_inf(h1), in2 = !is_inf(h2);
      const uint32_t c1 = refs.x, c2 = refs.y;
      const bool both = in1 && in2, any = in1 || in2;
      const bool first_is_near = ANY_HIT ? false : (h2 > h1);
      const uint32_t near_c = first_is_near ? c1 : c2;
      const uint32_t far_c = first_is_near ? c2 : c1;
      L.stack[sp * 64] = far_c;
      const uint32_t one_c = in1 ? c1 : c2;
      cur = both ? near_c : (any ? one_c : (sp != 0 ? popped : REF_DONE));
      sp = both ? sp + 1 : (any ? sp : sp_below);
    }
  };
  while (cur != REF_DONE) {
    if (__any(exact_slab))
      box_loop(std::true_type{});
    else
      box_loop(std::false_type{});
    if (cur != REF_DONE) {
      const uint32_t first = ref_index(cur), count = ref_count(cur);
      cnt.leaf += stat_inc;
      for (uint32_t i = 0; i < count; ++i) {
        gptr<DLeafPrim> lp = g.leaf_prims + (first + i);
        const v4f a = lp->a, b = lp->b;
        const float c0 = lp->c0;
        const uint32_t kind = lp->kind;
        cnt.prim += stat_inc;
        bool hit = false;
        float t = 0.f, e0 = 0.f, e1 = 0.f, e2 = 0.f, idet = 0.f;
        if (kind == 0) {
          hit = tri_test_flat(f3{a.x, a.y, a.z}, f3{a.w, b.x, b.y}, f3{b.z, b.w, c0}, ray, rc, t, e0,
                              e1, e2, idet);
        } else if (kind == 1) {
          cnt.sphere += stat_inc;
          hit = sphere_test(f3{a.x, a.y, a.z}, a.w, ray, dir_len2, t);
        }
        if (hit) {
          ray.max_t = t;
          found = true;
          if (ANY_HIT) break;
          rec.e0 = e0, rec.e1 = e1, rec.e2 = e2, rec.inv_det = idet;
          rec.prim = lp->prim;
          rec.kind = kind;
        }
      }
      if (ANY_HIT && found) {
        cur = REF_DONE;
      } else if (sp != 0) {
        --sp;
        cur = L.stack[sp * 64];
      } else {
        cur = REF_DONE;
      }
    }
  }
  return found;
}

VD f2 load_uv(const DScene& g, gptr<VimgMesh> m, uint32_t set, uint32_t vtx) {
  gptr<float> p = g.uvs + 2 * (size_t(m->uv_offset[set]) + (vtx - m->first_vertex));
  return f2{p[0], p[1]};
}
template <bool TEX>
VD void tri_hit_info(const DScene& g, uint32_t tri, const HitRec& rec, uint32_t prim_id, Hit& h) {
  gptr<DTriShade> ts = g.tri_shade + tri;
  const f3 p0{ts->p[0], ts->p[1], ts->p[2]}, p1{ts->p[3], ts->p[4], ts->p[5]},
      p2{ts->p[6], ts->p[7], ts->p[8]};
  gptr<VimgMesh> mesh = g.meshes + ts->mesh;
  const uint32_t i0 = ts->i0, i1 = ts->i1, i2 = ts->i2;
  const uint32_t mat = mesh->material;
  const uint32_t mflags = g.material_flags[mat];
  f3 edge1 = p1 - p0, edge2 = p2 - p0;
  float u = rec.e0 * rec.inv_det, v = rec.e1 * rec.inv_det, w = rec.e2 * rec.inv_det;
  const f3 tri_normal{ts->n[0], ts->n[1], ts->n[2]};
  f3 n0 = tri_normal, n1 = tri_normal, n2 = tri_normal, shading_normal = tri_normal;
  if (mesh->has_normals) {
    n0 = load3(g.normals + 3 * size_t(i0));
    n1 = load3(g.normals + 3 * size_t(i1));
    n2 = load3(g.normals + 3 * size_t(i2));
    shading_normal = normalize(u * n0 + v * n1 + w * n2);
  }
  h.p = u * p0 + v * p1 + w * p2;
  h.ng = tri_normal;
  h.mat = mat;
  h.prim = prim_id;
  h.ns = shading_normal;
  const bool need = TEX || (mflags & (MATF_NEEDS_UV | MATF_NEEDS_FRAME));
  if (!need) return;
  f2 uv{u, v};
  f2 uv0{0.f, 0.f}, uv1{1.f, 0.f}, uv2{1.f, 1.f};
  const uint32_t cset = mesh->color_tex_uv;
  if (cset != VIMG_NO_UV) {
    uv0 = load_uv(g, mesh, cset, i0), uv1 = load_uv(g, mesh, cset, i1), uv2 = load_uv(g, mesh, cset, i2);
    uv = u * uv0 + v * uv1 + w * uv2;
  }
  h.uv = uv;
  h.mr_uv = uv;
  if constexpr (TEX) {
    const uint32_t mset = mesh->metallic_roughness_tex_uv;
    if (mset != VIMG_NO_UV) {
      f2 m0 = load_uv(g, mesh, mset, i0), m1 = load_uv(g, mesh, mset, i1),
         m2 = load_uv(g, mesh, mset, i2);
      h.mr_uv = u * m0 + v * m1 + w * m2;
    }
  }
  f2 duvds = uv2 - uv0;
  f2 duvdt = uv2 - uv1;
  float det = duvds.x * duvdt.y - duvdt.x * duvds.y;
  float dsdu = 0.f, dtdu = 0.f, dsdv = 0.f, dtdv = 0.f;
  f3 dpdu, dpdv;
  if (absf(det) > 1e-8f && !is_nan(det)) {
    dsdu = duvdt.y / det;
    dtdu = -duvds.y / det;
    dsdv = duvdt.x / det;
    dtdv = -duvds.x / det;
    f3 dpds = p2 - p0;
    f3 dpdt = p2 - p1;
    dpdu = dpds * dsdu + dpdt * dtdu;
    dpdv = dpds * dsdv + dpdt * dtdv;
  } else {
    get_axis(shading_normal, dpdu, dpdv);
  }
  if constexpr (TEX) {
    const int nmap = g.materials[mat].normal_map;
    if (nmap >= 0) {
      f2 n_uv{u, v};
      const uint32_t nset = mesh->normal_tex_uv;
      if (nset != VIMG_NO_UV) {
        f2 q0 = load_uv(g, mesh, nset, i0), q1 = load_uv(g, mesh, nset, i1),
           q2 = load_uv(g, mesh, nset, i2);
        n_uv = u * q0 + v * q1 + w * q2;
      }
      f3 n_tangent_space = normalize(col_at_uv_mipmap(g, g.textures + nmap, 0, n_uv));
      Onb onb_n_map = init_onb(shading_normal);
      f3 local_space_normal = xform_with_onb(onb_n_map, n_tangent_space);
      float ulen = length(dpdu), vlen = length(dpdv);
      dpdu = normalize(gram_schmidt(dpdu, local_space_normal)) * ulen;
      dpdv = normalize(cross(local_space_normal, dpdu)) * vlen;
      shading_normal = local_space_normal;
      h.ns = shading_normal;
    }
  }
  f3 tangent = normalize(dpdu - shading_normal * dot(shading_normal, dpdu));
  f3 bitangent = normalize(cross(shading_normal, tangent));
  h.tu = tangent;
  h.tv = bitangent;
  if constexpr (TEX) {
    f3 dnds = n2 - n0;
    f3 dndt = n2 - n1;
    f3 dndu = dnds * dsdu + dndt * dtdu;
    f3 dndv = dnds * dsdv + dndt * dtdv;
    h.curvature = (dot(dndu, tangent) + dot(dndv, bitangent)) / 2.f;
    h.prim_area = length(cross(p1 - p0, p2 - p0));
    h.tex_area = absf((uv1.x - uv0.x) * (uv2.y - uv0.y) - (uv2.x - uv0.x) * (uv1.y - uv0.y));
  }
}
template <bool TEX>
VD void sphere_hit_info(const DScene& g, uint32_t sphere, const TravRay& r, uint32_t prim_id,
                        Hit& h) {
  gptr<VimgSphere> sp = g.spheres + sphere;
  const f3 center = load3(sp->center);
  const float radius = sp->radius;
  const uint32_t mat = sp->material;
  const uint32_t mflags = g.material_flags[mat];
  h.p = r.o + r.d * r.max_t;
  const f3 normal = normalize(h.p - center);
  h.ns = normal;
  h.ng = normal;
  h.mat = mat;
  h.prim = prim_id;
  if (TEX || (mflags & MATF_NEEDS_UV)) {
    float theta = F_acos(-normal.y);
    float phi = F_atan2(-normal.z, normal.x) + kPi;
    float u = phi / (2.f * kPi);
    float v = theta / kPi;
    h.uv = f2{u, v};
    h.mr_uv = f2{u, v};
  }
  if (TEX || (mflags & MATF_NEEDS_FRAME)) {
    f3 dpdu{-radius * normal.y, radius * normal.x, 0.f};
    f3 tangent = normalize(dpdu - normal * dot(normal, dpdu));
    h.tu = tangent;
    h.tv = normalize(cross(normal, tangent));
  }
  if constexpr (TEX) {
    h.curvature = 1.f / radius;
    h.prim_area = 1.f;
    h.tex_area = 0.000001f;
  }
}
template <bool TEX>
VD void make_hit_info(const DScene& g, const HitRec& rec, const TravRay& ray, Hit& h) {
  const VimgPrim p = load_prim(g.prims + rec.prim);
  if (p.type == VIMG_PRIM_TRIANGLE)
    tri_hit_info<TEX>(g, p.index, rec, rec.prim, h);
  else
    sphere_hit_info<TEX>(g, p.index, ray, rec.prim, h);
}

VD f3 mat_emitted(gptr<VimgMaterial> m, f3 ray_dir, f3 shading_normal) {
  if (m->type != VIMG_MAT_DIFFUSE_LIGHT) return f3{0.f, 0.f, 0.f};
  return (dot(shading_normal, ray_dir) < 0) ? load3(m->emit) : f3{0.f, 0.f, 0.f};
}

VD f3 reflect_dir(f3 wi, f3 n) { return wi - (2.f * dot(wi, n) * n); }
VD float schlick_apprx(float cosine, float in_ior, float out_ior) {
  float r0 = (in_ior - out_ior) / (in_ior + out_ior);
  r0 = r0 * r0;
  return r0 + (1.f - r0) * pow5(1.f - cosine);
}
VD f3 refract_dir(f3 wi, f3 n, float i_over_o, float cos_i, float sin2_t) {
  float normal_mul = (i_over_o * cos_i) - sqrt_f(1.f - sin2_t);
  return (i_over_o * wi) + (normal_mul * n);
}
VD Scatter dielectric_sample(gptr<VimgMaterial> m, const Hit& hit, f3 wi, Rng& rng) {
  const float ior = m->ior;
  f3 wo;
  float eta;
  bool front_face = dot(wi, hit.ns) < 0;
  f3 n = front_face ? hit.ns : -hit.ns;
  const float cos_i = -1.f * (dot(wi, n));
  float randf = rand_float(rng);
  if (front_face) {
    eta = ior;
    const float schlick = schlick_apprx(cos_i, 1.0f, ior);
    if (schlick > randf) {
      wo = reflect_dir(wi, n);
    } else {
      const float i_over_o = 1.f / ior;
      const float sin2 = (i_over_o * i_over_o) * (1.f - (cos_i * cos_i));
      wo = refract_dir(wi, n, i_over_o, cos_i, sin2);
    }
  } else {
    eta = 1.f / ior;
    const float i_over_o = ior;
    const float sin2 = (i_over_o * i_over_o) * (1.f - (cos_i * cos_i));
    if ((sin2 > 1.f) || (schlick_apprx(sqrt_f(1.f - sin2), ior, 1.f) > randf)) {
      wo = reflect_dir(wi, n);
    } else {
      wo = refract_dir(wi, n, i_over_o, cos_i, sin2);
    }
  }
  return Scatter{wo, eta, true, true};
}

VD float g_w(f3 w, float alphax, float alphay, const Onb& frame) {
  const f3 wl = project_onto_onb(frame, w);
  float vec_alpha = ((wl.x * alphax) * (wl.x * alphax) + (wl.y * alphay) * (wl.y * alphay))
                    / (wl.z * wl.z);
  float caret = (__builtin_sqrt(1. + static_cast<double>(vec_alpha)) - 1.) / 2.;
  return 1. / (1. + static_cast<double>(caret));
}

VD void sincos_azimuth(float phi_f, double& s_out, double& c_out) {
  const double x = static_cast<double>(phi_f);
  const double kd = __builtin_rint(x * 6.36619772367581382433e-01);
  const int k = static_cast<int>(kd);
  double r = __builtin_fma(-kd, 1.57079632673412561417e+00, x);
  r = __builtin_fma(-kd, 6.07710050650619224932e-11, r);
  const double z = r * r;
  double ps = __builtin_fma(z, 1.58969099521155010221e-10, -2.50507602534068634195e-08);
  ps = __builtin_fma(z, ps, 2.75573137070700676789e-06);
  ps = __builtin_fma(z, ps, -1.98412698298579493134e-04);
  ps = __builtin_fma(z, ps, 8.33333333332248946124e-03);
  const double sn = __builtin_fma(z * r, __builtin_fma(z, ps, -1.66666666666666324348e-01), r);
  double pc = __builtin_fma(z, -1.13596475577881948265e-11, 2.08757232129817482790e-09);
  pc = __builtin_fma(z, pc, -2.75573143513906633035e-07);
  pc = __builtin_fma(z, pc, 2.48015872894767294178e-05);
  pc = __builtin_fma(z, pc, -1.38888888888741095749e-03);
  pc = __builtin_fma(z, pc, 4.16666666666666019037e-02);
  const double hz = 0.5 * z;
  const double wv = 1.0 - hz;
  const double cs = wv + (((1.0 - wv) - hz) + z * (z * pc));
  const bool swap = (k & 1) != 0;
  double s = swap ? cs : sn;
  double c = swap ? sn : cs;
  if (k & 2) s = -s;
  if ((k + 1) & 2) c = -c;
  s_out = s, c_out = c;
}

enum : uint32_t {
  LOBE_NONE = 0,
  LOBE_COSINE = 1,
  LOBE_CLEARCOAT = 2,
  LOBE_METAL = 3,
  LOBE_GLASS = 4,
  LOBE_DIELECTRIC = 5
};

VD float fresnel_dielectric(float n_dot_i, float eta) {
  float n_dot_t_sq = 1.f - (1.f - n_dot_i * n_dot_i) / (eta * eta);
  if (n_dot_t_sq < 0) return 1;
  float n_dot_t = sqrt_f(n_dot_t_sq);
  n_dot_i = absf(n_dot_i);
  float rs = (n_dot_i - eta * n_dot_t) / (n_dot_i + eta * n_dot_t);
  float rp = (eta * n_dot_i - n_dot_t) / (eta * n_dot_i + n_dot_t);
  return (rs * rs + rp * rp) / 2;
}
VD float fd_term(f3 n, f3 w, float fd90) {
  return 1.f + (fd90 - 1.f) * pow5(1.f - sel_max(dot(n, w), 0.f));
}

VD DMatCoat load_coat(gptr<DMatCoat> p) {
  DMatCoat c;
  c.alpha_g = p->alpha_g, c.ag2 = p->ag2, c.ag2m1 = p->ag2m1, c.pad = 0.f, c.ag2m1_d = p->ag2m1_d, c.pi_log = p->pi_log;
  return c;
}
VD DMatWeights load_weights(gptr<DMatWeights> p) {
  DMatWeights w;
  w.choose_diff = p->choose_diff, w.choose_clearcoat = p->choose_clearcoat, w.choose_metal = p->choose_metal;
  w.choose_glass = p->choose_glass, w.sum2 = p->sum2, w.sum3 = p->sum3, w.sum4 = p->sum4;
  w.mix_diff = p->mix_diff, w.mix_sheen = p->mix_sheen, w.mix_coat = p->mix_coat, w.mix_metal = p->mix_metal;
  w.mix_glass = p->mix_glass;
  return w;
}
VD gptr<DMaterial> dmat_at(const DScene& g, uint32_t mat) {
  asm volatile("" : "+v"(mat));
  return g.dmaterials + mat;
}
template <bool TEX>
VD bool dmat_scalars(uint32_t bits) {
  return !TEX || (bits & DMAT_SCALARS) != 0;
}

struct PrincipledCommon {
  f3 dir_in;
  Onb frame;
  float metallic, roughness;
};
template <bool TEX>
VD PrincipledCommon principled_prologue(const DScene& g, gptr<VimgMaterial> m, f3 wi, const Hit& hit) {
  PrincipledCommon p;
  p.dir_in = -wi;
  p.frame = Onb{hit.tu, hit.tv, hit.ns};
  if ((dot(hit.ns, p.dir_in) * dot(hit.ng, p.dir_in)) < 0) {
    p.frame.u = -p.frame.u;
    p.frame.v = -p.frame.v;
    p.frame.w = -p.frame.w;
  }
  f2 m_r{1.f, 1.f};
  if constexpr (TEX) {
    if (m->mr_tex >= 0) m_r = rg_get_at_uv(g, m->mr_tex, hit.mr_uv);
  }
  m_r = m_r * f2{m->metallic_factor, m->roughness_factor};
  p.metallic = m_r.x;
  p.roughness = m_r.y;
  return p;
}

template <bool TEX>
VD void principled_eval_pdf(const DScene& g, gptr<VimgMaterial> m, f3 wi,
                                                 f3 wo, const Hit& hit, RayCone cone,
                                                 bool regularize, f3& f_out, float& pdf_out) {
  const PrincipledCommon pc = principled_prologue<TEX>(g, m, wi, hit);
  const f3 dir_in = pc.dir_in;
  const Onb& frame = pc.frame;
  const float metallic = pc.metallic, roughness = pc.roughness;
  const uint32_t mat = hit.mat;
  const int reg = regularize ? 1 : 0;
  float alphax, alphay;
  f3 base_color;
  bool scalars, colour;
  {
    gptr<DMaterial> dm = dmat_at(g, mat);
    const uint32_t bits = dm->bits;
    scalars = dmat_scalars<TEX>(bits), colour = (bits & DMAT_COLOUR) != 0;
    base_color = colour ? load3(dm->base) : col_at_ray_hit<TEX>(g, m->tex, wi, cone, hit);
    if (scalars) {
      alphax = dm->alpha[reg].ax, alphay = dm->alpha[reg].ay;
    } else {
      mat_alphas(clampf(roughness, 0.01f, 1.f), m->anisotropic, regularize, alphax, alphay);
    }
  }
  auto alpha_products = [&](float& ax2, float& ay2, double& pi_axay) {
    if (scalars) {
      gptr<DMatAlpha> a = dmat_at(g, mat)->alpha + reg;
      ax2 = a->ax2, ay2 = a->ay2, pi_axay = a->pi_axay;
    } else {
      ax2 = alphax * alphax, ay2 = alphay * alphay, pi_axay = kPi * alphax * alphay;
    }
  };
  const f3 half_vector = normalize(dir_in + wo);
  const float g_in = g_w(dir_in, alphax, alphay, frame);
  const float G = g_in * g_w(wo, alphax, alphay, frame);
  const float ng_in = dot(hit.ng, dir_in);
  const float ng_out = dot(hit.ng, wo);

  f3 eval_glass;
  float pdf_glass;
  {
    float in_geo_dot = dot(dir_in, hit.ng);
    bool reflect = (in_geo_dot * dot(hit.ng, wo)) >= 0;
    const DMatEta et = mat_eta_terms(m->eta, in_geo_dot >= 0);
    float ax2, ay2;
    double pi_axay;
    alpha_products(ax2, ay2, pi_axay);
    const float eta = et.eta;
    f3 hv = half_vector;
    if (!reflect) hv = normalize(dir_in + wo * eta);
    float h_dot_in = dot(hv, dir_in);
    float F = fresnel_dielectric(h_dot_in, eta);
    const f3 lh = project_onto_onb(frame, hv);
    float had = (lh.x * lh.x) / ax2 + (lh.y * lh.y) / ay2 + (lh.z * lh.z);
    float D = 1. / (pi_axay * (had * had));
    float normal_in_dot = dot(frame.w, dir_in);
    if (reflect) {
      eval_glass = base_color * (F * D * G) / (4.f * absf(normal_in_dot));
      pdf_glass = (F * D * g_in) / (4.f * absf(normal_in_dot));
    } else {
      float eta_factor = et.inv_eta2;
      float h_dot_out = dot(hv, wo);
      float sqrt_denom = h_dot_in + eta * h_dot_out;
      eval_glass = (colour ? load3(dmat_at(g, mat)->sqrt_base) : mat_sqrt3(base_color))
                   * (eta_factor * (1 - F) * D * G * eta * eta * absf(h_dot_out * h_dot_in))
                   / (absf(normal_in_dot) * sqrt_denom * sqrt_denom);
      float dh_dout = et.eta2 * h_dot_out / (sqrt_denom * sqrt_denom);
      pdf_glass = (1.f - F) * D * g_in * absf(dh_dout * h_dot_in / normal_in_dot);
    }
  }
  if (ng_in < 0) {
    const float mix_glass = mat_weight_terms(metallic, m->specular_transmission, m->clearcoat, m->sheen).mix_glass;
    f_out = mix_glass * eval_glass;
    pdf_out = pdf_glass;
    return;
  }
  const bool below = (ng_in < 0 || ng_out < 0);

  f3 eval_sheen{0.f, 0.f, 0.f};
  f3 eval_diff{0.f, 0.f, 0.f};
  float pdf_diff = 0.f;
  f3 eval_clearcoat{0.f, 0.f, 0.f};
  float pdf_clearcoat = 0.f;
  f3 eval_metal{0.f, 0.f, 0.f};
  float pdf_metal = 0.f;

  if (!below) {
    f3 c_tint{0.f, 0.f, 0.f};
    if (!colour) c_tint = mat_c_tint(base_color);
    {
      const f3 c_sheen = colour ? load3(dmat_at(g, mat)->c_sheen) : mat_c_sheen(c_tint, m->sheen_tint);
      eval_sheen = c_sheen * pow5(1.f - sel_max(dot(half_vector, wo), 0.f))
                   * sel_max(dot(frame.w, wo), 0.f);
    }
    {
      const float subsurface = m->subsurface;
      float normal_dirout_dot = dot(frame.w, wo);
      const float cos_theta_out = sel_max(normal_dirout_dot, 0.f);
      const float cos_theta_in = sel_max(dot(frame.w, dir_in), 0.f);
      const float dot_h_out = sel_max(dot(half_vector, wo), 0.f);
      const float fd90 = 0.5 + 2.0 * roughness * dot_h_out * dot_h_out;
      const f3 base_diffuse = base_color * kInvPiF * fd_term(frame.w, dir_in, fd90)
                              * fd_term(frame.w, wo, fd90) * cos_theta_out;
      const float fss90 = roughness * dot_h_out * dot_h_out;
      f3 ss_diffuse = base_color * 1.25f * kInvPiF
                      * (fd_term(frame.w, dir_in, fss90) * fd_term(frame.w, wo, fss90)
                             * ((1.f / (cos_theta_out + cos_theta_in)) - 0.5f)
                         + 0.5f)
                      * cos_theta_out;
      eval_diff = (1.f - subsurface) * base_diffuse + subsurface * ss_diffuse;
      pdf_diff = sel_max(normal_dirout_dot, 0.f) * kInvPiF;
    }
    {
      constexpr float R0 = ((1.5f - 1.f) * (1.5f - 1.f)) / ((1.5f + 1.f) * (1.5f + 1.f));
      float h_dirout_dot = absf(dot(half_vector, wo));
      float fresnel = R0 + (1. - R0) * pow5(1.f - h_dirout_dot);
      float Gc = g_w(dir_in, 0.25, 0.25, frame) * g_w(wo, 0.25, 0.25, frame);
      const DMatCoat cc = scalars ? load_coat(dmat_at(g, mat)->coat + reg) : mat_coat_terms(m->clearcoat_gloss, regularize);
      const f3 lh = project_onto_onb(frame, half_vector);
      float D = cc.ag2m1 / (cc.pi_log * (1. + cc.ag2m1_d * lh.z * lh.z));
      float clearcoat_eval = (fresnel * D * Gc) / (4.f * absf(dot(frame.w, dir_in)));
      pdf_clearcoat = (D * absf(dot(frame.w, half_vector))) / (4.f * h_dirout_dot);
      eval_clearcoat = splat3(clearcoat_eval);
    }
    {
      const f3 k_s = colour ? load3(dmat_at(g, mat)->k_s) : mat_k_s(c_tint, m->specular_tint);
      const f3 c_0 = mat_c_0(mat_spec_r0(m->specular, mat_r0(m->eta), metallic), k_s, metallic, base_color);
      const f3 one_minus_c_0 = mat_one_minus(c_0);
      f3 fresnel = c_0 + one_minus_c_0 * pow5(1.f - dot(half_vector, wo));
      const f3 lh = project_onto_onb(frame, half_vector);
      float ax2, ay2;
      double pi_axay;
      alpha_products(ax2, ay2, pi_axay);
      float had = (lh.x * lh.x) / ax2 + (lh.y * lh.y) / ay2 + (lh.z * lh.z);
      float D = 1. / (pi_axay * (had * had));
      float d_mul_denominator = D / (4.f * absf(dot(frame.w, dir_in)));
      eval_metal = fresnel * G * d_mul_denominator;
      pdf_metal = g_in * d_mul_denominator;
    }
  }
  const DMatWeights w = mat_weight_terms(metallic, m->specular_transmission, m->clearcoat, m->sheen);
  f3 eval_principled = (w.mix_diff * eval_diff)
                       + (w.mix_sheen * eval_sheen)
                       + (w.mix_coat * eval_clearcoat)
                       + (w.mix_metal * eval_metal)
                       + (w.mix_glass * eval_glass);
  pdf_out = w.choose_diff * pdf_diff + w.choose_clearcoat * pdf_clearcoat + w.choose_metal * pdf_metal
            + w.choose_glass * pdf_glass;
  f_out = eval_principled;
}

template <bool TEX, int MT = -1>
VD Scatter sample_mat(const DScene& g, const Hit& hit, f3 wi, Rng& rng, bool regularize) {
  gptr<VimgMaterial> m = g.materials + hit.mat;
  const uint32_t type = MT >= 0 ? uint32_t(MT) : m->type;
  const f3 dir_in = -wi;
  uint32_t lobe = LOBE_NONE;
  Onb frame{f3{1.f, 0.f, 0.f}, f3{0.f, 1.f, 0.f}, f3{0.f, 0.f, 1.f}};
  float alphax = 0.f, alphay = 0.f, eta = 0.f, alpha_g = 0.f;
  bool lambert_front = true;

  if (type == VIMG_MAT_LAMBERTIAN) {
    lobe = LOBE_COSINE;
    lambert_front = dot(wi, hit.ns) < 0;
    frame = init_onb(lambert_front ? hit.ns : -hit.ns);
  } else if (type == VIMG_MAT_DIELECTRIC) {
    lobe = LOBE_DIELECTRIC;
  } else if (type == VIMG_MAT_PRINCIPLED) {
    const PrincipledCommon pc = principled_prologue<TEX>(g, m, wi, hit);
    frame = pc.frame;
    const float metallic = pc.metallic;
    float roughness = pc.roughness;
    const float ng_in = dot(hit.ng, dir_in);
    gptr<DMaterial> dm = g.dmaterials + hit.mat;
    const bool scalars = dmat_scalars<TEX>(dm->bits);
    const int reg = regularize ? 1 : 0;
    if (ng_in < 0) {
      lobe = LOBE_GLASS;
    } else {
      const DMatWeights w = scalars ? load_weights(&dm->w) : mat_weight_terms(metallic, m->specular_transmission, m->clearcoat, m->sheen);
      float rnd = rand_float(rng);
      if (rnd <= w.choose_diff) {
        lobe = LOBE_COSINE;
      } else if (rnd > w.choose_diff && rnd <= w.sum2) {
        lobe = LOBE_CLEARCOAT;
      } else if (rnd > w.sum2 && rnd <= w.sum3) {
        lobe = LOBE_METAL;
      } else if (rnd > w.sum3 && rnd <= w.sum4) {
        lobe = LOBE_GLASS;
      }
    }
    if (lobe == LOBE_CLEARCOAT) {
      alpha_g = scalars ? dm->coat[reg].alpha_g : mat_alpha_g(m->clearcoat_gloss, regularize);
    } else if (lobe == LOBE_METAL || lobe == LOBE_GLASS) {
      if (scalars) {
        alphax = lobe == LOBE_GLASS ? dm->alpha[reg].ax : dm->salpha[reg][0];
        alphay = lobe == LOBE_GLASS ? dm->alpha[reg].ay : dm->salpha[reg][1];
        eta = dm->eta[ng_in >= 0 ? 0 : 1].eta;
      } else {
        if (lobe == LOBE_GLASS) roughness = clampf(roughness, 0.01f, 1.f);
        mat_alphas(roughness, m->anisotropic, regularize, alphax, alphay);
        eta = mat_eta_terms(m->eta, ng_in >= 0).eta;
      }
    }
  }
  if (lobe == LOBE_DIELECTRIC) return dielectric_sample(m, hit, wi, rng);
  if (lobe == LOBE_NONE) return no_scatter();

  const float ra = rand_float(rng);
  const float rb = rand_float(rng);
  const float phi = 2 * kPi * ((lobe == LOBE_CLEARCOAT) ? rb : ra);
  double sin_phi, cos_phi;
  sincos_azimuth(phi, sin_phi, cos_phi);

  if (lobe == LOBE_COSINE) {
    float cos_theta = sqrt_f(rb);
    float sin_theta = sqrt_f(1 - cos_theta * cos_theta);
    f3 local{static_cast<float>(cos_phi) * sin_theta, static_cast<float>(sin_phi) * sin_theta,
             cos_theta};
    f3 dir = xform_with_onb(frame, local);
    if (type == VIMG_MAT_LAMBERTIAN) {
      if (lambert_front) return Scatter{dir, 0.f, false, true};
      return no_scatter();
    }
    if (dot(hit.ng, dir) <= 0) return no_scatter();
    return Scatter{dir, 0.f, false, true};
  }
  if (lobe == LOBE_CLEARCOAT) {
    const float alpha = alpha_g;
    float cos2 = (1.f - ::pow(static_cast<double>(alpha * alpha), 1. - ra)) / (1.f - (alpha * alpha));
    float cos_elevation = sqrt_f(cos2);
    float sin_elevation = sqrt_f(1 - cos2);
    f3 local_h{sin_elevation * static_cast<float>(cos_phi), sin_elevation * static_cast<float>(sin_phi),
               cos_elevation};
    if (dot(frame.w, dir_in) < 0) {
      frame.u = -frame.u;
      frame.v = -frame.v;
      frame.w = -frame.w;
    }
    const f3 H = normalize(xform_with_onb(frame, local_h));
    f3 reflected = normalize(-dir_in + 2 * dot(dir_in, H) * H);
    if (dot(hit.ng, reflected) <= 0) return no_scatter();
    return Scatter{reflected, 0.f, true, true};
  }
  const f3 local_dir_in = project_onto_onb(frame, dir_in);
  f3 micro;
  {
    float sign = 1.f;
    f3 top = local_dir_in;
    if (local_dir_in.z < 0.f) {
      sign = -1.f;
      top = -top;
    }
    f3 hemi_dir_in = normalize(f3{alphax * top.x, alphay * top.y, top.z});
    float z = __builtin_fmaf((1.0f - rb), (1.0f + hemi_dir_in.z), -hemi_dir_in.z);
    float sin_theta = sqrt_f(clampf(1.0f - z * z, 0.0f, 1.0f));
    float x = sin_theta * cos_phi;
    float y = sin_theta * sin_phi;
    const f3 hemi_n = f3{x, y, z} + hemi_dir_in;
    micro = sign * normalize(f3{alphax * hemi_n.x, alphay * hemi_n.y, sel_max(0.f, hemi_n.z)});
  }
  if (lobe == LOBE_METAL) {
    f3 half_vector = normalize(xform_with_onb(frame, micro));
    f3 reflected = normalize(-dir_in + 2 * dot(dir_in, half_vector) * half_vector);
    if (dot(reflected, hit.ng) <= 0) return no_scatter();
    return Scatter{reflected, 0.f, true, true};
  }
  f3 half_vec = xform_with_onb(frame, micro);
  float h_dot_in = dot(half_vec, dir_in);
  float F = fresnel_dielectric(h_dot_in, eta);
  float rnd = rand_float(rng);
  if (rnd <= F) {
    f3 reflected = normalize(-dir_in + 2 * dot(dir_in, half_vec) * half_vec);
    if (dot(reflected, hit.ng) * dot(dir_in, hit.ng) <= 0) return no_scatter();
    return Scatter{reflected, 0.f, true, true};
  }
  float h_dot_out_sq = 1 - (1 - h_dot_in * h_dot_in) / (eta * eta);
  if (h_dot_out_sq <= 0) return no_scatter();
  if (h_dot_in < 0) half_vec = -half_vec;
  float h_dot_out = static_cast<float>(__builtin_sqrt(static_cast<double>(h_dot_out_sq)));
  f3 refracted = -dir_in / eta + (absf(h_dot_in) / eta - h_dot_out) * half_vec;
  if (dot(refracted, hit.ng) * dot(dir_in, hit.ng) >= 0) return no_scatter();
  f3 generalized_h = normalize(dir_in + refracted * eta);
  float g_h_dot_in = dot(generalized_h, dir_in);
  if ((1 - (1 - g_h_dot_in * g_h_dot_in) / (eta * eta)) <= 0) return no_scatter();
  return Scatter{refracted, eta, true, true};
}
template <bool TEX, int MT = -1>
VD void eval_pdf_pair(const DScene& g, const Hit& hit, f3 wi, f3 wo, RayCone cone, bool regularize,
                      f3& f, float& pdf) {
  gptr<VimgMaterial> m = g.materials + hit.mat;
  const uint32_t type = MT >= 0 ? uint32_t(MT) : m->type;
  if (type == VIMG_MAT_LAMBERTIAN) {
    float dot_product = static_cast<float>(sel_max(0.0f, dot(wo, hit.ns)) / kPi);
    gptr<DMaterial> dm = g.dmaterials + hit.mat;
    const f3 col = (dm->bits & DMAT_COLOUR) ? load3(dm->base) : col_at_ray_hit<TEX>(g, m->tex, wi, cone, hit);
    f = col * dot_product;
    pdf = dot_product;
  } else if (type == VIMG_MAT_PRINCIPLED) {
    principled_eval_pdf<TEX>(g, m, wi, wo, hit, cone, regularize, f, pdf);
  } else {
    f = f3{0.f, 0.f, 0.f};
    pdf = 1.0f;
  }
}

VD void tri_light_sample_with(f3 p0, f3 p1, f3 p2, f3 n0, f3 n1, f3 n2, float pdf, f3 look_from, Rng& rng, f3& hit_n,
                              EmitterInfo& info) {
  float rand1 = rand_float(rng);
  float rand2 = rand_float(rng);
  float u, v;
  if (rand1 < rand2) {
    u = rand1 / 2.f;
    v = rand2 - u;
  } else {
    v = rand2 / 2.f;
    u = rand1 - v;
  }
  float w = 1.f - u - v;
  const f3 hit_p = p0 * u + p1 * v + p2 * w;
  hit_n = normalize(u * n0 + v * n1 + w * n2);
  f3 dir_vec = hit_p - look_from;
  float dist2 = length2(dir_vec);
  dir_vec = normalize(dir_vec);
  float cosine = absf(dot(hit_n, -dir_vec));
  float G = cosine / dist2;
  info = EmitterInfo{dir_vec, pdf, sqrt_f(dist2), G};
}
VD void tri_light_sample_at(f3 p0, f3 p1, f3 p2, f3 tri_normal, float pdf, f3 look_from, Rng& rng, f3& hit_n, EmitterInfo& info) {
  tri_light_sample_with(p0, p1, p2, tri_normal, tri_normal, tri_normal, pdf, look_from, rng, hit_n, info);
}
VD void tri_light_sample(const DScene& g, uint32_t tri, f3 look_from, Rng& rng, f3& le,
                         EmitterInfo& info) {
  gptr<DTriShade> ts = g.tri_shade + tri;
  const f3 p0{ts->p[0], ts->p[1], ts->p[2]}, p1{ts->p[3], ts->p[4], ts->p[5]},
      p2{ts->p[6], ts->p[7], ts->p[8]};
  gptr<VimgMesh> mesh = g.meshes + ts->mesh;
  f3 tri_normal{ts->n[0], ts->n[1], ts->n[2]};
  f3 n0 = tri_normal, n1 = tri_normal, n2 = tri_normal;
  if (mesh->has_normals) {
    n0 = load3(g.normals + 3 * size_t(ts->i0));
    n1 = load3(g.normals + 3 * size_t(ts->i1));
    n2 = load3(g.normals + 3 * size_t(ts->i2));
  }
  f3 hit_n;
  tri_light_sample_with(p0, p1, p2, n0, n1, n2, g.tri_area_pdf[tri] , look_from,
                        rng, hit_n, info);
  le = mat_emitted(g.materials + mesh->material, info.wi, hit_n);
}
VD float tri_surf_pdf(const DScene& g, uint32_t tri) { return g.tri_area_pdf[tri]; }
VD void sphere_light_sample_at(f3 center, float radius, f3 look_from, Rng& rng, f3& shading_normal, EmitterInfo& info) {
  float rand1 = rand_float(rng);
  float rand2 = rand_float(rng);
  if (length2(look_from - center) <= radius * radius) {
    f3 unit = sample_sphere(rand1, rand2);
    f3 point_on_sphere = (unit * radius) + center;
    f3 to_pos = point_on_sphere - look_from;
    shading_normal = unit;
    const float sphere_sa = 4.f * kPi * radius * radius;
    f3 dir_to_surf = normalize(to_pos);
    float dist2 = length2(to_pos);
    float cosine = absf(dot(shading_normal, -dir_to_surf));
    float G = cosine / dist2;
    float pdf = 1.f / sphere_sa;
    info = EmitterInfo{dir_to_surf, pdf, sqrt_f(dist2), G};
  } else {
    float cos_theta_max = static_cast<float>(__builtin_sqrt(
        static_cast<double>(1.0f - ((radius * radius) / length2(look_from - center)))));
    f3 dir_center_to_lf = normalize(look_from - center);
    Onb onb = init_onb(dir_center_to_lf);
    f3 sample_z_dir = sample_sphere_cap(rand1, rand2, cos_theta_max);
    f3 sampled_point = normalize(xform_with_onb(onb, sample_z_dir)) * radius + center;
    float dist2 = length2(sampled_point - look_from);
    shading_normal = normalize(sampled_point - center);
    f3 sampled_dir = normalize(sampled_point - look_from);
    float cosine = absf(dot(shading_normal, -sampled_dir));
    float G = cosine / dist2;
    float pdf_solid_angle = 1.0f / (2.f * kPi * (1.0f - cos_theta_max));
    float pdf = pdf_solid_angle * G;
    info = EmitterInfo{sampled_dir, pdf, sqrt_f(dist2), G};
  }
}
VD float sphere_surf_pdf(gptr<VimgSphere> sp, f3 look_from, f3 point_on_light, f3 dir) {
  const f3 center = load3(sp->center);
  const float radius = sp->radius;
  if (length2(look_from - center) <= radius * radius) {
    const float sphere_sa = 4.f * kPi * radius * radius;
    return 1.f / sphere_sa;
  }
  float cos_theta_max = static_cast<float>(__builtin_sqrt(
      static_cast<double>(1.0f - ((radius * radius) / length2(look_from - center)))));
  float pdf_solid_angle = 1.0f / (2.f * kPi * (1.0f - cos_theta_max));
  f3 shading_normal = normalize(point_on_light - center);
  float cosine = absf(dot(shading_normal, -dir));
  float dist2 = length2(point_on_light - look_from);
  return pdf_solid_angle * cosine / dist2;
}

VD void env_dir_to_uv(const DScene& g, f3 in_dir, float& u, float& v) {
  f3 dir = normalize(mat_dir(g.background.world_to_env, in_dir));
  u = (1.f + F_atan2(-dir.x, dir.z) * kInvPi) * 0.5f;
  v = F_acos(dir.y) * kInvPi;
}
template <bool TEX>
VD f3 background_emit(const DScene& g, f3 in_dir, RayCone cone) {
  if constexpr (TEX) {
    if (g.background.type == VIMG_BG_ENVMAP) {
      gptr<VimgTexture> img = g.textures + g.background.env_tex;
      float u, v;
      env_dir_to_uv(g, in_dir, u, v);
      float lambda = ::log2(absf(cone.spread_angle) * (img->height / kPi));
      lambda = is_nan(lambda) ? 0.f : lambda;
      return col_mipmap_interpolate(g, img, lambda - 2.f, f2{u, v}) * g.background.radiance_scale;
    }
  }
  return load3k(g.background.col);
}
template <bool TEX>
VD float background_pdf(const DScene& g, f3 in_dir) {
  if constexpr (TEX) {
    if (g.background.type == VIMG_BG_ENVMAP) {
      gptr<VimgTexture> img = g.textures + g.background.env_tex;
      const uint32_t W = img->width, H = img->height;
      float u, v;
      env_dir_to_uv(g, in_dir, u, v);
      int pixel_u = u * W;
      int pixel_v = v * H;
      int column_index = clampi(pixel_u, 0, static_cast<int>(W) - 1);
      int row_index = clampi(pixel_v, 0, static_cast<int>(H) - 1);
      gptr<float> row_cdf = g.cdf_pool + g.background.row_cdf_offset;
      gptr<float> col_cdf = g.cdf_pool + g.background.col_cdf_offset + size_t(row_index) * (W + 1);
      float pdf_y = row_cdf[row_index + 1] - row_cdf[row_index];
      float pdf_x = col_cdf[column_index + 1] - col_cdf[column_index];
      float sin_elevation = ::sin(kPi * v);
      return (pdf_y * pdf_x * W * H) / (2.f * kPi * kPi * sin_elevation);
    }
  }
  return 1.f / (4 * kPi);
}
VD void cdf_sample(gptr<float> cdf, uint32_t n_plus_1, float u, uint32_t& index, float& du) {
  uint32_t lo = 0, len = n_plus_1;
  while (len > 0) {
    uint32_t half = len >> 1;
    uint32_t mid = lo + half;
    if (!(u < cdf[mid])) {
      lo = mid + 1;
      len = len - half - 1;
    } else {
      len = half;
    }
  }
  index = lo - 1;
  du = u - cdf[index];
  if (cdf[index + 1] - cdf[index] > 0) du /= cdf[index + 1] - cdf[index];
}
template <bool TEX>
VD void background_sample(const DScene& g, Rng& rng, f3& le, EmitterInfo& info) {
  float r1 = rand_float(rng);
  float r2 = rand_float(rng);
  if constexpr (TEX) {
    if (g.background.type == VIMG_BG_ENVMAP) {
      gptr<VimgTexture> img = g.textures + g.background.env_tex;
      const uint32_t W = img->width, H = img->height;
      gptr<float> row_cdf = g.cdf_pool + g.background.row_cdf_offset;
      uint32_t row_index, column_index;
      float dv, du;
      cdf_sample(row_cdf, H + 1, r1, row_index, dv);
      gptr<float> col_cdf = g.cdf_pool + g.background.col_cdf_offset + size_t(row_index) * (W + 1);
      cdf_sample(col_cdf, W + 1, r2, column_index, du);
      const float u_env = (static_cast<float>(column_index) + du) / W;
      const float v_env = (static_cast<float>(row_index) + dv) / H;
      float pdf_y = row_cdf[row_index + 1] - row_cdf[row_index];
      float pdf_x = col_cdf[column_index + 1] - col_cdf[column_index];
      float choose_sample_pdf = pdf_y * pdf_x;
      float elevation = v_env * kPi;
      float y = ::cos(v_env * kPi);
      const float azimuth = u_env * 2.f * kPi;
      float x = F_sin(azimuth) * F_sin(elevation);
      float z = -1 * F_cos(azimuth) * F_sin(elevation);
      f3 wi = normalize(mat_dir(g.background.env_to_world, f3{x, y, z}));
      float sin_elevation = F_sin(elevation);
      float pdf = (choose_sample_pdf * W * H) / (2.f * kPi * kPi * sin_elevation);
      le = col_at_uv_mipmap(g, img, 0, f2{u_env, v_env}) * g.background.radiance_scale;
      info = EmitterInfo{wi, pdf, VIMG_INF, 1.f};
      return;
    }
  }
  f3 wi = sample_sphere(r1, r2);
  constexpr float pdf = 1.f / (4 * kPi);
  le = load3k(g.background.col);
  info = EmitterInfo{wi, pdf, VIMG_INF, 1.f};
}
template <bool TEX>
VD void lights_sample(const DScene& g, f3 look_from, Rng& rng, f3& le, EmitterInfo& info) {
  float rnd = rand_float(rng);
  float sx = rnd * g.num_lights;
  const int index_obj = clampi(static_cast<int>(sx), 0, static_cast<int>(g.num_lights) - 1);
  const float prob_obj = 1.f / g.num_lights;
  gptr<DLight> L = g.dlights + index_obj;
  const uint32_t kind = L->kind;
  if (kind == 0u) {
    background_sample<TEX>(g, rng, le, info);
  } else if (kind == 2u) {
    tri_light_sample(g, L->index, look_from, rng, le, info);
  } else {
    f3 shading_normal;
    const v4f la = L->a;
    if (kind == 1u) {
      const v4f lb = L->b, lc = L->c;
      tri_light_sample_at(f3{la.x, la.y, la.z}, f3{la.w, lb.x, lb.y}, f3{lb.z, lb.w, lc.x}, f3{lc.y, lc.z, lc.w}, L->d.w, look_from,
                          rng, shading_normal, info);
    } else {
      sphere_light_sample_at(f3{la.x, la.y, la.z}, la.w, look_from, rng, shading_normal, info);
    }
    const v4f ld = L->d;
    le = (dot(shading_normal, info.wi) < 0) ? f3{ld.x, ld.y, ld.z} : f3{0.f, 0.f, 0.f};
  }
  info.pdf *= prob_obj;
}
VD float surf_pdf(const DScene& g, uint32_t prim_id, f3 look_from, f3 look_at, f3 dir) {
  const VimgPrim p = load_prim(g.prims + prim_id);
  if (p.type == VIMG_PRIM_TRIANGLE) return tri_surf_pdf(g, p.index);
  return sphere_surf_pdf(g.spheres + p.index, look_from, look_at, dir);
}

VD float balance_heuristic(float pdf1, float pdf2) { return pdf1 / (pdf1 + pdf2); }
VD float geometric_term(f3 look_from, f3 point_on_surface, f3 surface_normal) {
  f3 d = look_from - point_on_surface;
  float distance2 = length2(d);
  d = normalize(d);
  return absf(dot(surface_normal, d)) / distance2;
}

VD uint32_t lds_node_bytes(uint32_t n) { return n * (3 * 16 + 8); }
VD Lds lds_layout(const RenderArgs& A, VIMG_LDS unsigned char* lds_raw) {
  const uint32_t n = A.lds_nodes;
  VIMG_LDS v4f* na = reinterpret_cast<VIMG_LDS v4f*>(lds_raw);
  VIMG_LDS v4f* nb = na + n;
  VIMG_LDS v4f* nc = nb + n;
  VIMG_LDS v2u* nm = reinterpret_cast<VIMG_LDS v2u*>(nc + n);
  uint32_t stack_off = (lds_node_bytes(n) + 255u) & ~255u;
  VIMG_LDS uint32_t* stacks = reinterpret_cast<VIMG_LDS uint32_t*>(lds_raw + stack_off);
  const uint32_t wave = threadIdx.x >> 6, lane = threadIdx.x & 63;
  Lds L;
  L.na = na, L.nb = nb, L.nc = nc, L.nm = nm;
  L.stack = stacks + size_t(wave) * A.stack_entries * 64 + lane;
  L.n_nodes = n;
  return L;
}
VD Lds stage_lds(const DScene& g, const RenderArgs& A, VIMG_LDS unsigned char* lds_raw) {
  const uint32_t n = A.lds_nodes;
  VIMG_LDS v4f* na = reinterpret_cast<VIMG_LDS v4f*>(lds_raw);
  VIMG_LDS v4f* nb = na + n;
  VIMG_LDS v4f* nc = nb + n;
  VIMG_LDS v2u* nm = reinterpret_cast<VIMG_LDS v2u*>(nc + n);
  for (uint32_t i = threadIdx.x; i < n; i += blockDim.x) {
    gptr<DNode> src = g.nodes + i;
    na[i] = src->a;
    nb[i] = src->b;
    nc[i] = src->c;
    nm[i] = v2u{src->left_ref, src->right_ref};
  }
  __syncthreads();
  return lds_layout(A, lds_raw);
}

template <bool TEX, int WPS>
__global__ void __launch_bounds__(256, WPS)
render_kernel(const DScene g, const RenderArgs A, float* __restrict__ out,
              DeviceStats* __restrict__ stats, unsigned int* __restrict__ work_counter) {
  extern __shared__ __attribute__((aligned(16))) unsigned char lds_raw[];
  const Lds L = stage_lds(g, A, (VIMG_LDS unsigned char*)lds_raw);
  const uint32_t lane = threadIdx.x & 63;
  const bool full_stats = A.full_stats != 0;
  const uint32_t W = static_cast<uint32_t>(g.res_x), H = static_cast<uint32_t>(g.res_y);
  const bool single = A.single_x >= 0;
  const uint32_t total_items = single ? 1u : (A.item_list ? A.item_count : A.num_local_tiles * 64u);
  constexpr uint32_t roulette_threshold = 5;

  Counters cnt{0, 0, 0, 0, 0, 0, 0, 0};
  uint32_t nan_samples = 0, iter_wave = 0;

  bool alive = true, need_pixel = true;
  uint32_t item = 0, px = 0, py = 0, smp = 0;
  Rng rng{0};
  f3 acc{0.f, 0.f, 0.f};
  bool new_path = true, primary = true, non_specular_bounce = false;
  f3 ray_o{0.f, 0.f, 0.f}, ray_d{0.f, 0.f, 1.f};
  RayCone cone{0.f, 0.f};
  f3 throughput{1.f, 1.f, 1.f}, result{0.f, 0.f, 0.f};
  float eta_scale = 1.f, prev_pdf = 0.f;
  uint32_t bounce = 0;

  for (;;) {
    {
      const bool want = alive && need_pixel;
      const unsigned long long mask = __ballot(want);
      if (mask != 0ull) {
        const uint32_t n = __popcll(mask);
        uint32_t base = 0;
        const uint32_t leader = __ffsll(static_cast<long long>(mask)) - 1;
        if (lane == leader) base = atomicAdd(work_counter, n);
        base = __shfl(base, leader);
        if (want) {
          const uint32_t rank = __popcll(mask & ((1ull << lane) - 1ull));
          item = base + rank;
// ... 344 lines not shown
```

v-img_amd/csrc/scene_upload.hip:

```cpp
#include <cmath>
#include <cstdlib>
#include <cstring>
#include <memory>
#include <numbers>

#include "hip_internal.h"
#include "scene_bake.h"
#include "scene_update.h"

using namespace vimg;

namespace {

template <typename T>
int upload(VimgDeviceScene* s, DevBuf& b, const T* host, size_t count) {
  if (int rc = b.alloc(std::max<size_t>(count, 1) * sizeof(T))) return rc;
  s->total_bytes += b.bytes;
  if (count) HIP_TRY(hipMemcpy(b.p, host, count * sizeof(T), hipMemcpyHostToDevice));
  return VIMG_OK;
}

}

int vimg::validate_materials(const VimgMaterial* materials, uint32_t num_materials, const VimgTexture* textures, uint32_t num_textures,
// ... 299 lines not shown
    } else {
      bake_leaf_sphere(sc->spheres[p.index], lp);
      lp.kind = 1u;
    }
    leaf[j] = lp;
  }
  return leaf;
}

std::vector<DLight> bake_lights(const VimgScene* sc, const std::vector<DTriShade>& shade, const std::vector<float>& area_pdf) {
  std::vector<DLight> dlights(sc->num_lights);
  for (uint32_t i = 0; i < sc->num_lights; ++i)
    dlights[i] = bake_light(sc->lights[i], sc->prims, shade.data(), area_pdf.data(), sc->meshes, sc->spheres, sc->materials);
  return dlights;
}

std::vector<uint32_t> material_flags(const VimgScene* sc, bool* textured) {
  std::vector<uint32_t> mflags(sc->num_materials, 0);
  for (uint32_t i = 0; i < sc->num_materials; ++i) mflags[i] = bake_material_flags(sc->materials[i], sc->textures);
  *textured = tables_textured(sc->materials, sc->num_materials, sc->textures, sc->background);
  return mflags;
}

int upload_tables(VimgDeviceScene* s, const VimgScene* sc, const Tree& t, const std::vector<DTriShade>& shade,
                  const std::vector<float>& area_pdf, const std::vector<DLeafPrim>& leaf,
                  const std::vector<DLight>& dlights, const std::vector<uint32_t>& mflags) {
  DScene& d = s->d;
#define UP_TO(owner, field, host, count)                     \
  do {                                                       \
    DevBuf& b_ = owner;                                      \
    if (int rc_ = upload(s, b_, host, count)) return rc_;    \
    d.field = (decltype(d.field))b_.p;                       \
  } while (0)
#define UP(field, host, count) UP_TO(s->tables.emplace_back(), field, host, count)
  UP_TO(s->nodes, nodes, t.nodes.data(), t.nodes.size());
  UP_TO(s->leaf_prims, leaf_prims, leaf.data(), leaf.size());
  s->num_leaf_prims = static_cast<uint32_t>(leaf.size());
  UP(prims, sc->prims, sc->num_prims);
  UP(tri_shade, shade.data(), shade.size());
  UP(tri_area_pdf, area_pdf.data(), area_pdf.size());
  UP(meshes, sc->meshes, sc->num_meshes);
  UP(normals, sc->normals, size_t(sc->num_vertices) * 3);
  UP(uvs, sc->uvs, sc->num_uvs * 2);
  UP(spheres, sc->spheres, sc->num_spheres);
  UP(materials, sc->materials, sc->num_materials);
  UP(material_flags, mflags.data(), mflags.size());
  UP(textures, sc->textures, sc->num_textures);
  UP(texels, sc->texels, sc->num_texels * 3);
  UP(rg_textures, sc->rg_textures, sc->num_rg_textures);
  UP(rg_texels, sc->rg_texels, sc->num_rg_texels * 2);
  UP(lights, sc->lights, sc->num_lights);
  s->lights_table = s->tables.size() - 1;
  UP(dlights, dlights.data(), dlights.size());
  s->dlights_table = s->tables.size() - 1;
  UP(cdf_pool, sc->cdf_pool, sc->num_cdf);
#undef UP
#undef UP_TO
  {
    DevBuf& b = s->tables.emplace_back();
    if (int rc = b.alloc(std::max<size_t>(sc->num_materials, 1) * sizeof(DMaterial))) return rc;
    s->total_bytes += b.bytes;
    s->dmaterials_table = s->tables.size() - 1;
    d.dmaterials = (decltype(d.dmaterials))b.p;
    if (int rc = enqueue_material_bake(d, sc->num_materials, b.as<DMaterial>(), nullptr)) return rc;
    HIP_TRY(hipStreamSynchronize(nullptr));
  }
  if (!t.chain_leaf.empty()) {
    if (int rc = s->chain_leaf.alloc(t.chain_leaf.size() * sizeof(uint32_t))) return rc;
    HIP_TRY(hipMemcpy(s->chain_leaf.p, t.chain_leaf.data(), s->chain_leaf.bytes, hipMemcpyHostToDevice));
  }
  return VIMG_OK;
}

void record_for_updates(VimgDeviceScene* s, const VimgScene* sc) {
  s->materials.assign(sc->materials, sc->materials + sc->num_materials);
  s->textures.assign(sc->textures, sc->textures + sc->num_textures);
  s->lights.assign(sc->lights, sc->lights + sc->num_lights);
  s->num_rg_textures = sc->num_rg_textures;
  s->num_texels = sc->num_texels;
  s->num_cdf = sc->num_cdf;
  s->num_vertices = sc->num_vertices;
  s->num_tris = sc->num_tris;
  s->num_spheres = sc->num_spheres;
  for (uint32_t i = 0; i < sc->num_meshes; ++i) {
    const VimgMesh& m = sc->meshes[i];
    if (!m.has_normals || m.num_vertices == 0) continue;
    auto& r = s->normal_rows;
    if (!r.empty() && r.back().first + r.back().second == m.first_vertex)
      r.back().second += m.num_vertices;
    else
      r.push_back({m.first_vertex, m.num_vertices});
  }
}

int resolve_options(VimgDeviceScene* s, const VimgHipOptions* opts) {
  s->waves_per_simd = (s->total_bytes > (32u << 20)) ? 3 : 2;
  vimg_hip_options_default(&s->opt);
  if (opts) {
    const size_t n = std::min<size_t>(opts->struct_size, sizeof(VimgHipOptions));
    if (n >= sizeof(uint32_t)) std::memcpy(&s->opt, opts, n);
    s->opt.struct_size = sizeof(VimgHipOptions);
  }
  options_from_env(&s->opt);
  if (const char* e = getenv("VIMG_HIP_QUERY_BLOCKS")) s->query_launch = atoi(e) != 0 ? 1 : 0;
  if (const char* e = getenv("VIMG_HIP_PLAIN")) s->force_general = atoi(e) == 0;
  if (s->opt.scheduler != VIMG_OPT_AUTO && (s->opt.scheduler < VIMG_SCHED_LANE || s->opt.scheduler > VIMG_SCHED_CU))
    return fail(VIMG_E_INVALID, "options: unknown scheduler");
  if (s->opt.scheduler != VIMG_OPT_AUTO && s->opt.scheduler != VIMG_SCHED_LANE && s->opt.scheduler != VIMG_SCHED_CU)
    return fail(VIMG_E_UNSUPPORTED, "options: the schedulers POOL, POOL4, POOL4G and STAGE are retired; "
                                    "the library renders with CU (AUTO) or LANE");
  s->too_wide = (s->d.res_x > 65535 || s->d.res_y > 65535);
  return VIMG_OK;
}

int alloc_scratch(VimgDeviceScene* s) {
  hipDeviceProp_t prop{};
  if (hipGetDeviceProperties(&prop, g_device) != hipSuccess) return fail(VIMG_E_DEVICE, "hipGetDeviceProperties failed");
  s->num_cus = static_cast<uint32_t>(prop.multiProcessorCount);
  if (int rc = s->stats.alloc(sizeof(DeviceStats))) return rc;
  if (int rc = s->counter.alloc(2 * sizeof(unsigned int))) return rc;
  if (int rc = s->root_box.alloc(6 * sizeof(float))) return rc;
  HIP_TRY(hipMemset(s->counter.p, 0, s->counter.bytes));
  return VIMG_OK;
}

int build_scene(VimgDeviceScene* s, const VimgScene* sc, const VimgHipOptions* opts) {
  DScene& d = s->d;
  bake_camera(sc->camera, d);
  Tree tree;
  if (int rc = renumber_bvh(sc->bvh, tree)) return rc;
  d.root_ref = tree.root_ref;
  for (int a = 0; a < 3; ++a) {
    d.root_min[a] = sc->bvh.bb_mins_maxes[0 * 3 + a];
    d.root_max[a] = sc->bvh.bb_mins_maxes[2 * 3 + a];
  }
  d.num_nodes = static_cast<uint32_t>(tree.nodes.size());
  d.max_depth = sc->bvh.max_depth + tree.chain_depth;
  s->n_internal = tree.n_internal;
  s->n_chain = static_cast<uint32_t>(tree.chain.size());
  s->level_begin = tree.level_begin;
  std::vector<DTriShade> shade;
  std::vector<float> area_pdf;
  bake_triangles(sc, shade, area_pdf);
  const std::vector<DLeafPrim> leaf = bake_leaves(sc, shade);
  const std::vector<DLight> dlights = bake_lights(sc, shade, area_pdf);
  const std::vector<uint32_t> mflags = material_flags(sc, &s->textured);
  if (int rc = upload_tables(s, sc, tree, shade, area_pdf, leaf, dlights, mflags)) return rc;
  record_for_updates(s, sc);
  d.num_lights = sc->num_lights;
  d.background = sc->background;
  d.background_emissive = background_is_emissive(sc->background);
  if (int rc = resolve_options(s, opts)) return rc;
  return alloc_scratch(s);
}

}

extern "C" {

int vimg_hip_scene_upload(const VimgScene* sc, VimgDeviceScene** out) {
  return vimg_hip_scene_upload_opts(sc, nullptr, out);
}

int vimg_hip_scene_upload_opts(const VimgScene* sc, const VimgHipOptions* opts, VimgDeviceScene** out) {
  if (!out) return fail(VIMG_E_INVALID, "null output pointer");
  *out = nullptr;
  if (g_device < 0) {
    int rc = vimg_hip_init(0);
    if (rc) return rc;
  }
  int rc = validate(sc);
  if (rc) return rc;
  auto s = std::make_unique<VimgDeviceScene>();
  rc = build_scene(s.get(), sc, opts);
  if (rc) return rc;
  *out = s.release();
  return VIMG_OK;
}

int vimg_hip_scene_free(VimgDeviceScene* s) {
  if (!s) return VIMG_OK;
  delete s;
  return VIMG_OK;
}

int64_t vimg_hip_scene_bytes(const VimgDeviceScene* s) {
  return s ? static_cast<int64_t>(s->total_bytes) : 0;
}
// ... 51 lines not shown
```

v-img_amd/csrc/vimg_hip.hip:

```cpp
#include <cstdio>
#include <cstdlib>
#include <memory>

#include "hip_internal.h"
#include "aux_kernels.h"
#include "render_cu_kernel.h"
#include "heatmap_kernel.h"

namespace vimg {

hipStream_t g_stream = nullptr;
int g_device = -1;

namespace {
thread_local std::string g_err;
}

int fail(int code, const std::string& msg) {
  g_err = msg;
  return code;
}

}

using namespace vimg;

namespace vimg {

int check_params(const VimgDeviceScene* s, const VimgRenderParams* p) {
  if (!s || !p) return fail(VIMG_E_INVALID, "null scene or params");
  if (p->tile_world == 0 || p->tile_rank >= p->tile_world)
    return fail(VIMG_E_INVALID, "tile_rank must be < tile_world");
  if (p->samples == 0) return fail(VIMG_E_INVALID, "samples must be > 0");
  if (p->integrator == VIMG_INTEGRATOR_MATERIAL && p->depth == 0)
    return fail(VIMG_E_INVALID, "material integrator with depth 0 renders nothing");
  if (p->integrator > VIMG_INTEGRATOR_COVERAGE) return fail(VIMG_E_INVALID, "unknown integrator");
  if (p->integrator == VIMG_INTEGRATOR_MIS && s->d.num_lights == 0)
    return fail(VIMG_E_INVALID, "mis integrator needs at least one light (the reference's "
                                "GroupOfEmitters::sample is undefined without one)");
  return VIMG_OK;
}

int check_render(const VimgDeviceScene* s, const VimgRenderParams* p, const void* d_out) {
  if (int rc = check_params(s, p)) return rc;
  if (!d_out) return fail(VIMG_E_INVALID, "null output pointer");
  return VIMG_OK;
}

}

namespace {

int ensure_pool(VimgDeviceScene* s, LaunchCfg& c) {
  c.args.pool_cold = nullptr;
  if (!c.cold_bytes) return VIMG_OK;
  if (int rc = s->pool_cold.grow(c.cold_bytes)) return rc;
  c.args.pool_cold = (VIMG_GLOBAL v4u*)s->pool_cold.p;
  if (c.ovf_bytes) {
    if (int rc = s->stack_ovf.grow(c.ovf_bytes)) return rc;
    c.args.stack_ovf = (VIMG_GLOBAL uint32_t*)s->stack_ovf.p;
  }
  c.args.pool_state = nullptr;
  c.args.pool_epoch = 0;
  if (c.args.pool_segments > 1) {
    const size_t had = s->pool_state.bytes;
    if (int rc = s->pool_state.grow(size_t(c.args.num_local_tiles) * 64u * 32u)) return rc;
    if (s->pool_state.bytes != had) s->pool_epoch = 0xffff0000u;
    s->pool_epoch += 4096u;
    if (s->pool_epoch >= 0xffff0000u) {
      HIP_TRY(hipMemset(s->pool_state.p, 0, s->pool_state.bytes));
      s->pool_epoch = 4096u;
    }
    c.args.pool_state = (VIMG_GLOBAL v4u*)s->pool_state.p;
    c.args.pool_epoch = s->pool_epoch;
  }
  return VIMG_OK;
}

}

namespace vimg {

int enqueue_render(VimgDeviceScene* s, const VimgRenderParams* p, const RenderLaunch& r) {
  const ProgLaunch* prog = r.prog;
  const hipStream_t st = r.st;
  float* d_out = r.d_out;
  LaunchCfg c = make_launch(s, p, r.sx, r.sy);
  if (prog) {
    c.args.sample_base = prog->base;
    c.args.spp_div = static_cast<float>(prog->base + p->samples);
    c.args.prog_in = (const VIMG_GLOBAL v4u*)prog->in;
    c.args.prog_out = (VIMG_GLOBAL v4u*)prog->out;
    c.args.item_list = (const VIMG_GLOBAL uint32_t*)prog->item_list;
    c.args.item_count = prog->item_count;
  }
  if (int rc = ensure_pool(s, c)) return rc;
  c.args.full_stats = r.stats ? 1u : 0u;
  if (c.args.num_local_tiles == 0 && r.sx < 0) return VIMG_OK;
  HIP_TRY(hipMemsetAsync(s->counter.p, 0, sizeof(unsigned int), st));
  if (r.stats && !(prog && prog->keep_stats)) HIP_TRY(hipMemsetAsync(s->stats.p, 0, sizeof(DeviceStats), st));
  DeviceStats* stats = r.stats ? s->stats.as<DeviceStats>() : nullptr;
  const void* kernel = launched_kernel_of(s, c, r.stats);
  if (c.lds_bytes > 48u * 1024u)
    HIP_TRY(hipFuncSetAttribute(kernel, hipFuncAttributeMaxDynamicSharedMemorySize, int(c.lds_bytes)));
  if (r.ev0) HIP_TRY(hipEventRecord(r.ev0, st));
  if (c.sched == VIMG_SCHED_CU) {
    CuKArgs ka{s->d, c.args, d_out, stats, s->counter.as<unsigned int>()};
    void* kargs[] = {&ka};
    HIP_TRY(hipLaunchKernel(kernel, dim3(c.grid), dim3(uint32_t(c.cu_waves) * 64u), kargs, c.lds_bytes, st));
  } else {
    void* kargs[] = {&s->d, &c.args, &d_out, &stats, &s->counter.p};
    HIP_TRY(hipLaunchKernel(kernel, dim3(c.grid), dim3(256), kargs, c.lds_bytes, st));
  }
  if (r.ev1) HIP_TRY(hipEventRecord(r.ev1, st));
  HIP_TRY(hipGetLastError());
  return VIMG_OK;
}

int check_kernel_error(VimgDeviceScene* s) {
  unsigned int words[2] = {0, 0};
  HIP_TRY(hipMemcpy(words, s->counter.p, sizeof(words), hipMemcpyDeviceToHost));
  if (words[1] != 0) HIP_TRY(hipMemset(s->counter.as<unsigned int>() + 1, 0, sizeof(unsigned int)));
  if (words[1] != 0) {
    const std::string what = (words[1] & 8u) ? "a compute unit queued more than 2^31 rays in one launch: render fewer samples per launch "
                                               "(vimg_hip_progressive_render adds a frame's samples in increments)"
                                             : "a wave waited for work that never came";
    return fail(VIMG_E_DEVICE, "render kernel watchdog: " + what + " (the frame is incomplete), code " +
                                   std::to_string(words[1]));
  }
  return VIMG_OK;
}

uint64_t fetch_shard_pixels(const VimgDeviceScene* s, const VimgRenderParams* p) {
  const uint32_t W = s->d.res_x, H = s->d.res_y, ty_n = tiles_of(H), total = tiles_of(W) * ty_n;
  uint64_t px = 0;
  for (uint32_t t = p->tile_rank; t < total; t += p->tile_world) {
    uint32_t tx = t / ty_n, ty = t % ty_n;
    px += uint64_t(std::min(8u, W - tx * 8)) * std::min(8u, H - ty * 8);
  }
  return px;
}

int fetch_stats(VimgDeviceScene* s, const VimgRenderParams* p, VimgRenderStats* out) {
  DeviceStats ds{};
  HIP_TRY(hipMemcpy(&ds, s->stats.p, sizeof(ds), hipMemcpyDeviceToHost));
  *out = VimgRenderStats{};
  out->closest_rays = ds.closest;
  out->shadow_rays = ds.shadow;
  out->internal_visits = ds.internal;
  out->leaf_visits = ds.leaf;
  out->prim_tests = ds.prim;
  out->sphere_tests = ds.sphere;
  out->nan_samples = ds.nan_samples;
  out->paths = fetch_shard_pixels(s, p) * p->samples;
  if (getenv("VIMG_HIP_DIAG"))
    std::fprintf(stderr, "[vimg diag] wave trips: descend %llu (lane visits %llu, util %.3f)  prim %llu (lane tests %llu, util %.3f)  main-loop iterations %llu\n",
                 ds.trip_descend, ds.internal, ds.trip_descend ? double(ds.internal) / (64.0 * ds.trip_descend) : 0.0,
                 ds.trip_prim, ds.prim, ds.trip_prim ? double(ds.prim) / (64.0 * ds.trip_prim) : 0.0, ds.iterations);
  if (getenv("VIMG_HIP_DIAG") && ds.prof[6 + 4]) {
    static const char* st_names[6] = {"finisher", "lambertian", "principled", "other", "walk", "looking for work"};
    unsigned long long total = 0;
    for (int k = 0; k < 6; ++k) total += ds.prof[k];
    for (int k = 0; k < 6; ++k)
      std::fprintf(stderr, "[vimg stage] %-18s %14llu cyc %6.2f %%  batches %10llu  slots/batch %7.2f\n", st_names[k],
                   ds.prof[k], 100.0 * double(ds.prof[k]) / double(total ? total : 1), k < 5 ? ds.prof[6 + k] : 0ull,
                   (k < 5 && ds.prof[6 + k]) ? double(ds.prof[11 + k]) / double(ds.prof[6 + k]) : 0.0);
    if (ds.prof[16])
      std::fprintf(stderr, "[vimg walk] box passes %llu lanes/pass %.2f   leaf rounds %llu lanes/round %.2f   sessions %llu   refills %llu rays/refill %.2f\n",
                   ds.prof[16], double(ds.prof[17]) / double(ds.prof[16]), ds.prof[18], double(ds.prof[19]) / double(ds.prof[18] ? ds.prof[18] : 1),
                   ds.prof[20], ds.prof[21], double(ds.prof[22]) / double(ds.prof[21] ? ds.prof[21] : 1));
    if (ds.wait_n[4])
      std::fprintf(stderr, "[vimg wait] mean cycles in a ring before a wave takes the slot: finisher %.0f  lambertian %.0f  principled %.0f  other %.0f  walk %.0f\n",
                   double(ds.wait_cyc[0]) / double(ds.wait_n[0] ? ds.wait_n[0] : 1), double(ds.wait_cyc[1]) / double(ds.wait_n[1] ? ds.wait_n[1] : 1),
                   double(ds.wait_cyc[2]) / double(ds.wait_n[2] ? ds.wait_n[2] : 1), double(ds.wait_cyc[3]) / double(ds.wait_n[3] ? ds.wait_n[3] : 1),
                   double(ds.wait_cyc[4]) / double(ds.wait_n[4]));
    if (ds.ray_cyc[1])
      std::fprintf(stderr, "[vimg wait] mean cycles of a ray in a walking lane (pop to hand-over) %.0f; of a vertex batch: finisher %.0f lambertian %.0f principled %.0f other %.0f\n",
                   double(ds.ray_cyc[0]) / double(ds.ray_cyc[1]), double(ds.prof[0]) / double(ds.prof[6] ? ds.prof[6] : 1), double(ds.prof[1]) / double(ds.prof[7] ? ds.prof[7] : 1),
                   double(ds.prof[2]) / double(ds.prof[8] ? ds.prof[8] : 1), double(ds.prof[3]) / double(ds.prof[9] ? ds.prof[9] : 1));
    if (ds.pv_cyc[6])
// ... 231 lines not shown
```

Measured before the change: 15230 Mrays/s.

## Stage small hit and material tables into LDS for plain CU kernel

When the plain CU kernel path is taken and there is spare LDS, the prims, triangle shading, sphere, material-flag and mesh tables are copied into LDS at block start. Shading and light-sampling code is templated over a table view, so those lookups read LDS instead of global memory. The launch code now fits node and stack budgets under the 160 KB LDS limit and drops the staged tables when the launched kernel would not read them. In exchange, every block pays a staging copy at start, and the larger LDS footprint can lower occupancy.

```diff
diff --git a/v-img_amd/csrc/device_scene.h b/v-img_amd/csrc/device_scene.h
--- a/v-img_amd/csrc/device_scene.h
+++ b/v-img_amd/csrc/device_scene.h
@@ -82,6 +82,25 @@
 };
 
 enum : uint32_t {
+  TAB_PRIMS = 0, TAB_TRI_SHADE, TAB_SPHERES, TAB_MATERIAL_FLAGS, TAB_MESHES,
+  TAB_MATERIALS, TAB_DMATERIALS,
+  TAB_COUNT
+};
+struct __attribute__((aligned(16))) LSphere {
+  float center[3];
+  float radius;
+  uint32_t material;
+  uint32_t pad[3];
+};
+static_assert(sizeof(LSphere) == 32, "LSphere must be 32 bytes");
+__host__ __device__ constexpr uint32_t tab_row_bytes(uint32_t t) {
+  return t == TAB_PRIMS ? uint32_t(sizeof(VimgPrim)) : t == TAB_TRI_SHADE ? uint32_t(sizeof(DTriShade)) :
+         t == TAB_SPHERES ? uint32_t(sizeof(LSphere)) : t == TAB_MATERIAL_FLAGS ? 4u :
+         t == TAB_MESHES ? uint32_t(sizeof(VimgMesh)) : t == TAB_MATERIALS ? uint32_t(sizeof(VimgMaterial)) :
+         uint32_t(sizeof(DMaterial));
+}
+
+enum : uint32_t {
   MATF_NEEDS_UV = 1u,
   MATF_NEEDS_FRAME = 2u,
 };
@@ -125,6 +144,8 @@
   VIMG_GLOBAL v4u* prog_out;
   const VIMG_GLOBAL uint32_t* item_list;
   uint32_t item_count;
+  uint32_t lds_tables;
+  uint32_t tab_off[TAB_COUNT], tab_rows[TAB_COUNT];
 };
 
 struct DeviceStats {
diff --git a/v-img_amd/csrc/hip_internal.h b/v-img_amd/csrc/hip_internal.h
--- a/v-img_amd/csrc/hip_internal.h
+++ b/v-img_amd/csrc/hip_internal.h
@@ -23,6 +23,7 @@
   int waves_per_simd = 2;
   bool too_wide = false;
   bool force_general = false;
+  bool no_lds_tables = false;
   uint32_t num_cus = 0;
   uint32_t num_leaf_prims = 0;
   vimg::DevBuf stats;
@@ -35,6 +36,7 @@
   uint32_t pool_epoch = 0;
   uint64_t generation = 0;
   uint32_t num_vertices = 0, num_tris = 0, num_spheres = 0;
+  uint32_t num_meshes = 0;
   std::vector<std::pair<uint32_t, uint32_t>> normal_rows;
   uint32_t n_internal = 0;
   uint32_t n_chain = 0;
@@ -81,8 +83,10 @@
 inline uint32_t opt_or(int32_t v, uint32_t dflt) { return v == VIMG_OPT_AUTO ? dflt : static_cast<uint32_t>(v); }
 
 struct LaunchCfg {
+  const char* error;
   RenderArgs args;
   uint32_t grid, lds_bytes;
+  uint32_t table_bytes;
   int sched;
   int wps;
   bool deep;
@@ -161,6 +165,7 @@
 const void* kernel_of(const VimgDeviceScene* s, const LaunchCfg& c);
 const void* launched_kernel_of(const VimgDeviceScene* s, const LaunchCfg& c, bool stats);
 bool plain_launch_serves(const VimgDeviceScene* s, const LaunchCfg& c, bool stats);
+void drop_unread_tables(const VimgDeviceScene* s, LaunchCfg& c, bool stats);
 
 }
 #pragma GCC visibility pop
diff --git a/v-img_amd/csrc/launch_policy.hip b/v-img_amd/csrc/launch_policy.hip
--- a/v-img_amd/csrc/launch_policy.hip
+++ b/v-img_amd/csrc/launch_policy.hip
@@ -66,7 +66,9 @@
   *shift = l - 1u;
 }
 
-LaunchCfg make_launch_cu(const VimgDeviceScene* s, const VimgRenderParams* p, int sx, int sy) {
+constexpr uint32_t CU_LDS_LIMIT = 160u * 1024u;
+
+LaunchCfg cu_launch_with(const VimgDeviceScene* s, const VimgRenderParams* p, int sx, int sy, uint32_t node_budget, uint32_t stack_cap) {
   LaunchCfg c{};
   const VimgHipOptions& o = s->opt;
   const uint64_t items = (sx >= 0) ? 1 : uint64_t(local_tiles(s, p)) * 64u;
@@ -75,7 +77,7 @@
   c.cu_waves = 16;
   const uint32_t nw = uint32_t(c.cu_waves);
   RenderArgs& a = c.args = base_args(s, p, sx, sy);
-  a.stack_lds = std::min(a.stack_entries, std::max(1u, opt_or(o.lds_stack, 32u)));
+  a.stack_lds = std::min(a.stack_entries, std::max(1u, stack_cap));
   a.cu_walkers = 0;
   a.cu_flex = opt_or(o.cu_flex, 1u);
   a.cu_lowwater = std::max(1u, opt_or(o.cu_lowwater, 64u));
@@ -85,8 +87,6 @@
   a.pool_starve = std::min(64u, std::max(1u, opt_or(o.pool_starve, 16u)));
   a.pool_classes = std::min(3u, std::max(1u, opt_or(o.pool_classes, 3u)));
   const uint32_t share = (160u * 1024u) / (16u / nw) - 1024u;
-  uint32_t node_budget = 4608u;
-  if (o.lds_budget_kb != VIMG_OPT_AUTO) node_budget = uint32_t(std::max(1, o.lds_budget_kb)) * 1024u;
   a.lds_nodes = std::min(node_budget / 56u, s->d.num_nodes);
   const uint32_t node_bytes = (a.lds_nodes * 56u + 255u) & ~255u;
   c.deep = a.lds_nodes < s->d.num_nodes || a.stack_lds < a.stack_entries;
@@ -123,8 +123,34 @@
   magic_div(slots, &a.cu_magic_v, &a.cu_shift_v);
   magic_div(2u * slots, &a.cu_magic_w, &a.cu_shift_w);
   c.lds_bytes = node_bytes + stack_bytes + cu_pool_bytes(slots, nw) + leaf_bytes;
+  a.lds_tables = 0u;
+  c.table_bytes = 0u;
+  if (!s->no_lds_tables && plain_build_serves(plain_launch_of(true, s->textured, c.deep, c.cu_waves, false, s->force_general, a))) {
+    const uint32_t n_mat = uint32_t(s->materials.size());
+    uint32_t rows[TAB_COUNT];
+    rows[TAB_PRIMS] = s->num_leaf_prims, rows[TAB_TRI_SHADE] = s->num_tris, rows[TAB_SPHERES] = s->num_spheres;
+    rows[TAB_MATERIAL_FLAGS] = n_mat, rows[TAB_MESHES] = s->num_meshes;
+    rows[TAB_MATERIALS] = n_mat, rows[TAB_DMATERIALS] = n_mat;
+    static const struct { uint32_t bit, first, end; } groups[2] = {{PF_TAB_HIT, TAB_PRIMS, TAB_MATERIALS}, {PF_TAB_MAT, TAB_MATERIALS, TAB_COUNT}};
+    const uint64_t used = uint64_t(c.lds_bytes) + 64u;
+    uint64_t room = share > used ? share - used : 0u;
+    for (const auto& gr : groups) {
+      if (!(PLAIN_FOLD & gr.bit)) continue;
+      uint64_t bytes = 0;
+      for (uint32_t t = gr.first; t < gr.end; ++t) bytes += (uint64_t(rows[t]) * tab_row_bytes(t) + 15u) & ~uint64_t(15);
+      if (bytes > room) continue;
+      for (uint32_t t = gr.first; t < gr.end; ++t) {
+        a.tab_off[t] = c.lds_bytes, a.tab_rows[t] = rows[t];
+        c.lds_bytes += (rows[t] * tab_row_bytes(t) + 15u) & ~15u;
+      }
+      c.table_bytes += uint32_t(bytes);
+      room -= bytes;
+      a.lds_tables |= gr.bit;
+    }
+  }
   int per_cu = 0;
-  hipError_t oe = hipOccupancyMaxActiveBlocksPerMultiprocessor(&per_cu, launched_kernel_of(s, c, false), int(nw * 64u), c.lds_bytes);
+  hipError_t oe = c.lds_bytes > CU_LDS_LIMIT ? hipErrorInvalidValue
+                                             : hipOccupancyMaxActiveBlocksPerMultiprocessor(&per_cu, launched_kernel_of(s, c, false), int(nw * 64u), c.lds_bytes);
   if (oe != hipSuccess || per_cu < 1) per_cu = 1;
   per_cu = std::min<int>(per_cu, int(16u / nw));
   const uint64_t need_blocks = (items + slots - 1) / slots;
@@ -137,6 +163,28 @@
   return c;
 }
 
+LaunchCfg make_launch_cu(const VimgDeviceScene* s, const VimgRenderParams* p, int sx, int sy) {
+  const VimgHipOptions& o = s->opt;
+  const bool own_nodes = o.lds_budget_kb == VIMG_OPT_AUTO, own_stack = o.lds_stack == VIMG_OPT_AUTO;
+  uint32_t node_budget = own_nodes ? 4608u : uint32_t(std::min(std::max(1, o.lds_budget_kb), 1 << 20)) * 1024u;
+  uint32_t stack_cap = opt_or(o.lds_stack, 32u);
+  const uint32_t limit = CU_LDS_LIMIT;
+  LaunchCfg c = cu_launch_with(s, p, sx, sy, node_budget, stack_cap);
+  if (c.lds_bytes > limit && own_nodes) c = cu_launch_with(s, p, sx, sy, node_budget = 1024u, stack_cap);
+  for (int round = 0; round < 8 && c.lds_bytes > limit && own_stack && c.args.stack_lds > 1u; ++round) {
+    const uint32_t per_row = std::max(1u, c.args.cu_walkers) * 256u;
+    const uint32_t rows_over = (c.lds_bytes - limit + per_row - 1u) / per_row;
+    stack_cap = c.args.stack_lds > rows_over + 1u ? c.args.stack_lds - rows_over - 1u : 1u;
+    c = cu_launch_with(s, p, sx, sy, node_budget, stack_cap);
+  }
+  if (c.lds_bytes > limit)
+    c.error = !own_nodes && !own_stack ? "options: lds_budget_kb and lds_stack together are beyond the compute unit's 160 KB of LDS"
+              : !own_nodes           ? "options: lds_budget_kb is beyond the compute unit's 160 KB of LDS"
+              : !own_stack           ? "options: lds_stack is beyond the compute unit's 160 KB of LDS"
+                                     : "the launch does not fit the compute unit's 160 KB of LDS";
+  return c;
+}
+
 void cu_scratch(const VimgDeviceScene* s, LaunchCfg& c) {
   const RenderArgs& a = c.args;
   c.cold_bytes = size_t(c.grid) * cu_cold_records(s->textured) * a.pool_slots * 16u;
@@ -153,7 +201,15 @@
 }
 
 bool plain_launch_serves(const VimgDeviceScene* s, const LaunchCfg& c, bool stats) {
-  return plain_build_serves(plain_launch_of(c.sched == VIMG_SCHED_CU, s->textured, c.deep, c.cu_waves, stats, s->force_general, c.args));
+  return plain_build_serves(plain_launch_of(c.sched == VIMG_SCHED_CU, s->textured, c.deep, c.cu_waves, stats, s->force_general, c.args)) &&
+         plain_tables_serve(c.args.lds_tables);
+}
+
+void drop_unread_tables(const VimgDeviceScene* s, LaunchCfg& c, bool stats) {
+  if (c.sched != VIMG_SCHED_CU || c.args.lds_tables == 0u || plain_launch_serves(s, c, stats)) return;
+  c.lds_bytes -= c.table_bytes;
+  c.table_bytes = 0u;
+  c.args.lds_tables = 0u;
 }
 
 const void* launched_kernel_of(const VimgDeviceScene* s, const LaunchCfg& c, bool stats) {
@@ -204,6 +260,7 @@
   if (is_feature_integrator(p->integrator)) return make_launch_feature(s, p, sx, sy);
   if (s->too_wide || s->opt.scheduler == VIMG_SCHED_LANE) return make_launch_lane(s, p, sx, sy);
   LaunchCfg c = make_launch_cu(s, p, sx, sy);
+  if (c.error) return c;
   cu_scratch(s, c);
   return c;
 }
@@ -223,6 +280,7 @@
   if (p->tile_world == 0 || p->tile_rank >= p->tile_world) return "";
   if (is_feature_integrator(p->integrator)) return s->textured ? "feature_kernel<true>" : "feature_kernel<false>";
   const LaunchCfg c = make_launch(s, p, -1, -1);
+  if (c.error) return "";
   if (c.sched == VIMG_SCHED_CU && !s->textured && !c.deep && !plain_launch_serves(s, c, false)) return "render_cu_kernel<false,general>";
   if (c.sched == VIMG_SCHED_CU) return cu_names[s->textured ? 1 : 0][c.deep ? 1 : 0];
   return lane_names[s->textured ? 1 : 0][c.wps >= 3 ? 1 : 0];
diff --git a/v-img_amd/csrc/plain_build.h b/v-img_amd/csrc/plain_build.h
--- a/v-img_amd/csrc/plain_build.h
+++ b/v-img_amd/csrc/plain_build.h
@@ -10,11 +10,14 @@
   PF_SINGLE = 8u,
   PF_ITEMS = 16u,
   PF_FLEX = 32u,
+  PF_TAB_HIT = 64u,
+  PF_TAB_MAT = 128u,
+  PF_TABLES = PF_TAB_HIT | PF_TAB_MAT,
 };
 #ifdef VIMG_PLAIN_FOLD
 constexpr uint32_t PLAIN_FOLD = VIMG_PLAIN_FOLD;
 #else
-constexpr uint32_t PLAIN_FOLD = PF_INTEGRATOR | PF_CLASSES | PF_LEAF_LDS | PF_SINGLE | PF_ITEMS | PF_FLEX;
+constexpr uint32_t PLAIN_FOLD = PF_INTEGRATOR | PF_CLASSES | PF_LEAF_LDS | PF_SINGLE | PF_ITEMS | PF_FLEX | PF_TAB_HIT;
 #endif
 
 struct PlainLaunch {
@@ -41,6 +44,10 @@
   return true;
 }
 
+constexpr bool plain_tables_serve(uint32_t staged, uint32_t fold = PLAIN_FOLD) {
+  return (staged & fold & PF_TABLES) == (fold & PF_TABLES);
+}
+
 template <class Args>
 constexpr PlainLaunch plain_launch_of(bool cu_sched, bool textured, bool deep, int cu_waves, bool stats, bool force_general,
                                       const Args& a) {
diff --git a/v-img_amd/csrc/render_cu_kernel.h b/v-img_amd/csrc/render_cu_kernel.h
--- a/v-img_amd/csrc/render_cu_kernel.h
+++ b/v-img_amd/csrc/render_cu_kernel.h
@@ -96,6 +96,31 @@
 }
 template <uint32_t PLAIN> VD uint32_t opt_flex(const RenderArgs& A) {
   if constexpr (PLAIN & PF_FLEX) return PLAIN_FLEX_DEFAULT; else return A.cu_flex;
+}
+
+template <class T>
+VD void stage_rows(VIMG_LDS unsigned char* lds_raw, const RenderArgs& A, uint32_t t, gptr<T> src) {
+  constexpr uint32_t src_w = uint32_t(sizeof(T)) / 4u;
+  const uint32_t dst_w = tab_row_bytes(t) / 4u, words = A.tab_rows[t] * src_w;
+  VIMG_LDS uint32_t* dst = reinterpret_cast<VIMG_LDS uint32_t*>(lds_raw + A.tab_off[t]);
+  gptr<uint32_t> w = reinterpret_cast<gptr<uint32_t>>(src);
+  for (uint32_t i = threadIdx.x; i < words; i += blockDim.x) {
+    const uint32_t r = i / src_w;
+    dst[r * dst_w + (i - r * src_w)] = w[i];
+  }
+}
+VD void stage_tables(const DScene& g, const RenderArgs& A, VIMG_LDS unsigned char* lds_raw) {
+  if (A.lds_tables & PF_TAB_HIT) {
+    stage_rows(lds_raw, A, TAB_PRIMS, g.prims);
+    stage_rows(lds_raw, A, TAB_TRI_SHADE, g.tri_shade);
+    stage_rows(lds_raw, A, TAB_SPHERES, g.spheres);
+    stage_rows(lds_raw, A, TAB_MATERIAL_FLAGS, g.material_flags);
+    stage_rows(lds_raw, A, TAB_MESHES, g.meshes);
+  }
+  if (A.lds_tables & PF_TAB_MAT) {
+    stage_rows(lds_raw, A, TAB_MATERIALS, g.materials);
+    stage_rows(lds_raw, A, TAB_DMATERIALS, g.dmaterials);
+  }
 }
 
 
@@ -147,6 +172,8 @@
   [[maybe_unused]] VIMG_LDS CuWaveRec* wrec = reinterpret_cast<VIMG_LDS CuWaveRec*>(G + 1) + wave;                      \
   [[maybe_unused]] VIMG_LDS v4f* lds_leaf = reinterpret_cast<VIMG_LDS v4f*>(reinterpret_cast<VIMG_LDS CuWaveRec*>(G + 1) + NW); \
   [[maybe_unused]] VIMG_LDS uint32_t* recw = reinterpret_cast<VIMG_LDS uint32_t*>(recs);                                \
+       \
+  [[maybe_unused]] const auto& gt = table_view<(PLAIN & PF_TABLES)>(g, A, (const VIMG_LDS unsigned char*)lds_raw);      \
   [[maybe_unused]] auto rd = [&](uint32_t r, uint32_t slot) -> v4u { return recs[r * P + slot]; };                      \
   [[maybe_unused]] auto wr = [&](uint32_t r, uint32_t slot, v4u v) { recs[r * P + slot] = v; };                         \
   [[maybe_unused]] auto flag_word = [&](uint32_t slot) -> VIMG_LDS uint32_t* { return recw + (CR_DIR * P + slot) * 4u + 3u; }; \
@@ -354,7 +381,7 @@
         hr.prim = r_hx.x;
         hr.kind = (flags & CF_KIND_SPHERE) ? 1u : 0u;
         TravRay tr{ray_o, ray_d, 0.0001f, uf(r_hx.y)};
-        make_hit_info<TEX>(g, hr, tr, hit);
+        make_hit_info<TEX>(gt, hr, tr, hit);
       }
       if (material_mode) {
         if (!hit_any) {
@@ -378,7 +405,7 @@
           result = background_emit<TEX>(g, ray_d, cone);
           finish = true;
         } else {
-          gptr<VimgMaterial> m = g.materials + hit.mat;
+          const auto m = tb_materials(gt) + hit.mat;
           if (m->type == VIMG_MAT_DIFFUSE_LIGHT) {
             result = mat_emitted(m, ray_d, hit.ns);
             finish = true;
@@ -389,11 +416,11 @@
         }
       } else {
         if (hit_any) {
-          gptr<VimgMaterial> m = g.materials + hit.mat;
+          const auto m = tb_materials(gt) + hit.mat;
           if (m->type == VIMG_MAT_DIFFUSE_LIGHT) {
             const f3 le = mat_emitted(m, ray_d, hit.ns);
             if (prev_pdf != 0) {
-              float light_pdf = surf_pdf(g, hit.prim, ray_o, hit.p, ray_d) / g.num_lights;
+              float light_pdf = surf_pdf(gt, hit.prim, ray_o, hit.p, ray_d) / g.num_lights;
               float Gt = geometric_term(ray_o, hit.p, hit.ng);
               float mis_weight = balance_heuristic(prev_pdf * Gt, light_pdf);
               result = result + throughput * mis_weight * le;
@@ -449,9 +476,9 @@
   float shadow_max_t = 0.f;
   if constexpr (!finisher_batch) {
     if (material_mode && at_vertex) {
-      gptr<VimgMaterial> m = g.materials + hit.mat;
+      const auto m = tb_materials(gt) + hit.mat;
       const f3 emitted_col = mat_emitted(m, ray_d, hit.ns);
-      Scatter sc = sample_mat<TEX>(g, hit, ray_d, rng, non_specular_bounce);
+      Scatter sc = sample_mat<TEX>(gt, hit, ray_d, rng, non_specular_bounce);
       if (!sc.valid) {
         result = throughput * emitted_col;
         finish = true;
@@ -475,7 +502,7 @@
         } else if (type == VIMG_MAT_PRINCIPLED) {
           f3 f;
           float pdf;
-          principled_eval_pdf<TEX>(g, m, ray_d, sc.wo, hit, cone, non_specular_bounce, f, pdf);
+          principled_eval_pdf<TEX>(gt, m, ray_d, sc.wo, hit, cone, non_specular_bounce, f, pdf);
           fdiv = f / pdf;
         }
         throughput = throughput * (emitted_col + fdiv);
@@ -515,20 +542,20 @@
     Scatter sc = no_scatter();
     Rng rng_l{0};
     if (at_vertex) {
-      mat_type = MT >= 0 ? uint32_t(MT) : g.materials[hit.mat].type;
+      mat_type = MT >= 0 ? uint32_t(MT) : tb_materials(gt)[hit.mat].type;
       if constexpr (TEX) {
         hit_dist = length(ray_o - hit.p);
         surface_spread_angle = spread_angle_from_curvature(hit.curvature, cone.cone_width, ray_d, hit.ns);
       }
       reg_before = non_specular_bounce;
       if constexpr (LIGHT_FIRST) {
-        lights_sample<TEX>(g, hit.p, rng, light_col, li);
+        lights_sample<TEX>(gt, hit.p, rng, light_col, li);
         nee = (li.pdf != 0.f);
       } else {
         rng_l = rng;
         if (mat_type != VIMG_MAT_DIELECTRIC) pcg_skip6(rng);
       }
-      sc = sample_mat<TEX, MT>(g, hit, ray_d, rng, reg_before);
+      sc = sample_mat<TEX, MT>(gt, hit, ray_d, rng, reg_before);
       if constexpr (TEX) nee_cone = propagate_reflect_cone(cone, surface_spread_angle * 2.f, hit_dist);
       if (sc.valid) {
         if (!sc.is_specular) non_specular_bounce = true;
@@ -553,7 +580,7 @@
     pv_lap(3);
     if constexpr (!LIGHT_FIRST) {
       if (at_vertex && mat_type != VIMG_MAT_DIELECTRIC) {
-        lights_sample<TEX>(g, hit.p, rng_l, light_col, li);
+        lights_sample<TEX>(gt, hit.p, rng_l, light_col, li);
         nee = (li.pdf != 0.f);
       }
     }
@@ -571,9 +598,9 @@
       float pdf_l = 0.f, pdf_s = 0.f;
       if constexpr (LAMB) {
         if (nee || sc.valid) {
-          gptr<DMaterial> dm = g.dmaterials + hit.mat;
+          const auto dm = tb_dmaterials(gt) + hit.mat;
           const f3 col = (dm->bits & DMAT_COLOUR) ? load3(dm->base)
-                                                  : col_at_ray_hit<TEX>(g, g.materials[hit.mat].tex, ray_d, nee_cone, hit);
+                                                  : col_at_ray_hit<TEX>(g, tb_materials(gt)[hit.mat].tex, ray_d, nee_cone, hit);
           const float cos_l = sel_max(0.0f, dot(li.wi, hit.ns)), cos_s = sel_max(0.0f, dot(sc.wo, hit.ns));
           const float dp_l = static_cast<float>(cos_l / kPi), dp_s = static_cast<float>(cos_s / kPi);
           if (nee) f_l = col * dp_l, pdf_l = dp_l;
@@ -591,7 +618,7 @@
             const f3 wo{uf(w4.x), uf(w4.y), uf(w4.z)};
             const RayCone c = second ? cone : nee_cone;
             const bool reg = second ? non_specular_bounce : reg_before;
-            eval_pdf_pair<TEX, MT>(g, hit, ray_d, wo, c, reg, f, pdf);
+            eval_pdf_pair<TEX, MT>(gt, hit, ray_d, wo, c, reg, f, pdf);
           }
           if (second) f_s = f, pdf_s = pdf;
           else f_l = f, pdf_l = pdf;
@@ -1072,6 +1099,7 @@
     for (uint32_t i = lane; i < sizeof(CuWaveRec) / 4u; i += 64u) reinterpret_cast<VIMG_LDS uint32_t*>(wrec)[i] = 0u;
     for (uint32_t i = threadIdx.x; i < A.lds_leaf * 3u; i += blockDim.x)
       lds_leaf[i] = reinterpret_cast<gptr<v4f>>(g.leaf_prims)[i];
+    if constexpr ((PLAIN & PF_TABLES) != 0u) stage_tables(g, A, (VIMG_LDS unsigned char*)lds_raw);
     for (uint32_t s = threadIdx.x; s < P; s += blockDim.x) {
       recw[(CR_DIR * P + s) * 4u + 3u] = CF_FRESH;
       ring_v[s] = static_cast<uint16_t>(s);
diff --git a/v-img_amd/csrc/render_kernels.h b/v-img_amd/csrc/render_kernels.h
--- a/v-img_amd/csrc/render_kernels.h
+++ b/v-img_amd/csrc/render_kernels.h
@@ -2,6 +2,7 @@
 #include "device_math.h"
 #include "device_scene.h"
 #include "material_terms.h"
+#include "plain_build.h"
 
 namespace vimg {
 
@@ -540,27 +541,67 @@
   return found;
 }
 
-VD f2 load_uv(const DScene& g, gptr<VimgMesh> m, uint32_t set, uint32_t vtx) {
+template <typename T>
+using lptr = const VIMG_LDS T*;
+template <uint32_t GROUPS>
+struct LdsTables {
+  const DScene& d;
+  const RenderArgs& A;
+  const VIMG_LDS unsigned char* base;
+  VD operator const DScene&() const { return d; }
+};
+template <uint32_t GROUPS>
+VD decltype(auto) table_view(const DScene& g, const RenderArgs& A, const VIMG_LDS unsigned char* lds_raw) {
+  if constexpr (GROUPS == 0u) return (g); else return LdsTables<GROUPS>{g, A, lds_raw};
+}
+VD const DScene& scn(const DScene& g) { return g; }
+template <uint32_t GROUPS>
+VD const DScene& scn(const LdsTables<GROUPS>& g) { return g.d; }
+#define VIMG_TABLE(name, GT, LT, group, slot)                                                 \
+  VD gptr<GT> tb_##name(const DScene& g) { return g.name; }                                   \
+  template <uint32_t GROUPS>                                                                  \
+  VD auto tb_##name(const LdsTables<GROUPS>& g) {                                             \
+    if constexpr ((GROUPS & (group)) != 0u)                                                   \
+      return reinterpret_cast<lptr<LT>>(g.base + g.A.tab_off[slot]);                          \
+    else                                                                                      \
+      return g.d.name;                                                                        \
+  }
+VIMG_TABLE(prims, VimgPrim, VimgPrim, PF_TAB_HIT, TAB_PRIMS)
+VIMG_TABLE(tri_shade, DTriShade, DTriShade, PF_TAB_HIT, TAB_TRI_SHADE)
+VIMG_TABLE(spheres, VimgSphere, LSphere, PF_TAB_HIT, TAB_SPHERES)
+VIMG_TABLE(material_flags, uint32_t, uint32_t, PF_TAB_HIT, TAB_MATERIAL_FLAGS)
+VIMG_TABLE(meshes, VimgMesh, VimgMesh, PF_TAB_HIT, TAB_MESHES)
+VIMG_TABLE(materials, VimgMaterial, VimgMaterial, PF_TAB_MAT, TAB_MATERIALS)
+VIMG_TABLE(dmaterials, DMaterial, DMaterial, PF_TAB_MAT, TAB_DMATERIALS)
+#undef VIMG_TABLE
+VD f3 load3(lptr<float> p) { return f3{p[0], p[1], p[2]}; }
+VD VimgPrim load_prim(lptr<VimgPrim> p) {
+  v2u v = *reinterpret_cast<const VIMG_LDS v2u*>(p);
+  return VimgPrim{v.x, v.y};
+}
+
+template <class MeshPtr>
+VD f2 load_uv(const DScene& g, MeshPtr m, uint32_t set, uint32_t vtx) {
   gptr<float> p = g.uvs + 2 * (size_t(m->uv_offset[set]) + (vtx - m->first_vertex));
   return f2{p[0], p[1]};
 }
-template <bool TEX>
-VD void tri_hit_info(const DScene& g, uint32_t tri, const HitRec& rec, uint32_t prim_id, Hit& h) {
-  gptr<DTriShade> ts = g.tri_shade + tri;
+template <bool TEX, class S>
+VD void tri_hit_info(const S& g, uint32_t tri, const HitRec& rec, uint32_t prim_id, Hit& h) {
+  const auto ts = tb_tri_shade(g) + tri;
   const f3 p0{ts->p[0], ts->p[1], ts->p[2]}, p1{ts->p[3], ts->p[4], ts->p[5]},
       p2{ts->p[6], ts->p[7], ts->p[8]};
-  gptr<VimgMesh> mesh = g.meshes + ts->mesh;
+  const auto mesh = tb_meshes(g) + ts->mesh;
   const uint32_t i0 = ts->i0, i1 = ts->i1, i2 = ts->i2;
   const uint32_t mat = mesh->material;
-  const uint32_t mflags = g.material_flags[mat];
+  const uint32_t mflags = tb_material_flags(g)[mat];
   f3 edge1 = p1 - p0, edge2 = p2 - p0;
   float u = rec.e0 * rec.inv_det, v = rec.e1 * rec.inv_det, w = rec.e2 * rec.inv_det;
   const f3 tri_normal{ts->n[0], ts->n[1], ts->n[2]};
   f3 n0 = tri_normal, n1 = tri_normal, n2 = tri_normal, shading_normal = tri_normal;
   if (mesh->has_normals) {
-    n0 = load3(g.normals + 3 * size_t(i0));
-    n1 = load3(g.normals + 3 * size_t(i1));
-    n2 = load3(g.normals + 3 * size_t(i2));
+    n0 = load3(scn(g).normals + 3 * size_t(i0));
+    n1 = load3(scn(g).normals + 3 * size_t(i1));
+    n2 = load3(scn(g).normals + 3 * size_t(i2));
     shading_normal = normalize(u * n0 + v * n1 + w * n2);
   }
   h.p = u * p0 + v * p1 + w * p2;
@@ -605,7 +646,7 @@
     get_axis(shading_normal, dpdu, dpdv);
   }
   if constexpr (TEX) {
-    const int nmap = g.materials[mat].normal_map;
+    const int nmap = tb_materials(g)[mat].normal_map;
     if (nmap >= 0) {
       f2 n_uv{u, v};
       const uint32_t nset = mesh->normal_tex_uv;
@@ -614,7 +655,7 @@
            q2 = load_uv(g, mesh, nset, i2);
         n_uv = u * q0 + v * q1 + w * q2;
       }
-      f3 n_tangent_space = normalize(col_at_uv_mipmap(g, g.textures + nmap, 0, n_uv));
+      f3 n_tangent_space = normalize(col_at_uv_mipmap(g, scn(g).textures + nmap, 0, n_uv));
       Onb onb_n_map = init_onb(shading_normal);
       f3 local_space_normal = xform_with_onb(onb_n_map, n_tangent_space);
       float ulen = length(dpdu), vlen = length(dpdv);
@@ -638,14 +679,14 @@
     h.tex_area = absf((uv1.x - uv0.x) * (uv2.y - uv0.y) - (uv2.x - uv0.x) * (uv1.y - uv0.y));
   }
 }
-template <bool TEX>
-VD void sphere_hit_info(const DScene& g, uint32_t sphere, const TravRay& r, uint32_t prim_id,
+template <bool TEX, class S>
+VD void sphere_hit_info(const S& g, uint32_t sphere, const TravRay& r, uint32_t prim_id,
                         Hit& h) {
-  gptr<VimgSphere> sp = g.spheres + sphere;
+  const auto sp = tb_spheres(g) + sphere;
   const f3 center = load3(sp->center);
   const float radius = sp->radius;
   const uint32_t mat = sp->material;
-  const uint32_t mflags = g.material_flags[mat];
+  const uint32_t mflags = tb_material_flags(g)[mat];
   h.p = r.o + r.d * r.max_t;
   const f3 normal = normalize(h.p - center);
   h.ns = normal;
@@ -672,16 +713,17 @@
     h.tex_area = 0.000001f;
   }
 }
-template <bool TEX>
-VD void make_hit_info(const DScene& g, const HitRec& rec, const TravRay& ray, Hit& h) {
-  const VimgPrim p = load_prim(g.prims + rec.prim);
+template <bool TEX, class S>
+VD void make_hit_info(const S& g, const HitRec& rec, const TravRay& ray, Hit& h) {
+  const VimgPrim p = load_prim(tb_prims(g) + rec.prim);
   if (p.type == VIMG_PRIM_TRIANGLE)
     tri_hit_info<TEX>(g, p.index, rec, rec.prim, h);
   else
     sphere_hit_info<TEX>(g, p.index, ray, rec.prim, h);
 }
 
-VD f3 mat_emitted(gptr<VimgMaterial> m, f3 ray_dir, f3 shading_normal) {
+template <class MatPtr>
+VD f3 mat_emitted(MatPtr m, f3 ray_dir, f3 shading_normal) {
   if (m->type != VIMG_MAT_DIFFUSE_LIGHT) return f3{0.f, 0.f, 0.f};
   return (dot(shading_normal, ray_dir) < 0) ? load3(m->emit) : f3{0.f, 0.f, 0.f};
 }
@@ -696,7 +738,8 @@
   float normal_mul = (i_over_o * cos_i) - sqrt_f(1.f - sin2_t);
   return (i_over_o * wi) + (normal_mul * n);
 }
-VD Scatter dielectric_sample(gptr<VimgMaterial> m, const Hit& hit, f3 wi, Rng& rng) {
+template <class MatPtr>
+VD Scatter dielectric_sample(MatPtr m, const Hit& hit, f3 wi, Rng& rng) {
   const float ior = m->ior;
   f3 wo;
   float eta;
@@ -785,12 +828,14 @@
   return 1.f + (fd90 - 1.f) * pow5(1.f - sel_max(dot(n, w), 0.f));
 }
 
-VD DMatCoat load_coat(gptr<DMatCoat> p) {
+template <class CoatPtr>
+VD DMatCoat load_coat(CoatPtr p) {
   DMatCoat c;
   c.alpha_g = p->alpha_g, c.ag2 = p->ag2, c.ag2m1 = p->ag2m1, c.pad = 0.f, c.ag2m1_d = p->ag2m1_d, c.pi_log = p->pi_log;
   return c;
 }
-VD DMatWeights load_weights(gptr<DMatWeights> p) {
+template <class WeightsPtr>
+VD DMatWeights load_weights(WeightsPtr p) {
   DMatWeights w;
   w.choose_diff = p->choose_diff, w.choose_clearcoat = p->choose_clearcoat, w.choose_metal = p->choose_metal;
   w.choose_glass = p->choose_glass, w.sum2 = p->sum2, w.sum3 = p->sum3, w.sum4 = p->sum4;
@@ -798,9 +843,10 @@
   w.mix_glass = p->mix_glass;
   return w;
 }
-VD gptr<DMaterial> dmat_at(const DScene& g, uint32_t mat) {
+template <class S>
+VD auto dmat_at(const S& g, uint32_t mat) {
   asm volatile("" : "+v"(mat));
-  return g.dmaterials + mat;
+  return tb_dmaterials(g) + mat;
 }
 template <bool TEX>
 VD bool dmat_scalars(uint32_t bits) {
@@ -812,8 +858,8 @@
   Onb frame;
   float metallic, roughness;
 };
-template <bool TEX>
-VD PrincipledCommon principled_prologue(const DScene& g, gptr<VimgMaterial> m, f3 wi, const Hit& hit) {
+template <bool TEX, class S, class MatPtr>
+VD PrincipledCommon principled_prologue(const S& g, MatPtr m, f3 wi, const Hit& hit) {
   PrincipledCommon p;
   p.dir_in = -wi;
   p.frame = Onb{hit.tu, hit.tv, hit.ns};
@@ -832,8 +878,8 @@
   return p;
 }
 
-template <bool TEX>
-VD void principled_eval_pdf(const DScene& g, gptr<VimgMaterial> m, f3 wi,
+template <bool TEX, class S, class MatPtr>
+VD void principled_eval_pdf(const S& g, MatPtr m, f3 wi,
                                                  f3 wo, const Hit& hit, RayCone cone,
                                                  bool regularize, f3& f_out, float& pdf_out) {
   const PrincipledCommon pc = principled_prologue<TEX>(g, m, wi, hit);
@@ -846,7 +892,7 @@
   f3 base_color;
   bool scalars, colour;
   {
-    gptr<DMaterial> dm = dmat_at(g, mat);
+    const auto dm = dmat_at(g, mat);
     const uint32_t bits = dm->bits;
     scalars = dmat_scalars<TEX>(bits), colour = (bits & DMAT_COLOUR) != 0;
     base_color = colour ? load3(dm->base) : col_at_ray_hit<TEX>(g, m->tex, wi, cone, hit);
@@ -858,7 +904,7 @@
   }
   auto alpha_products = [&](float& ax2, float& ay2, double& pi_axay) {
     if (scalars) {
-      gptr<DMatAlpha> a = dmat_at(g, mat)->alpha + reg;
+      const auto a = dmat_at(g, mat)->alpha + reg;
       ax2 = a->ax2, ay2 = a->ay2, pi_axay = a->pi_axay;
     } else {
       ax2 = alphax * alphax, ay2 = alphay * alphay, pi_axay = kPi * alphax * alphay;
@@ -983,9 +1029,9 @@
   f_out = eval_principled;
 }
 
-template <bool TEX, int MT = -1>
-VD Scatter sample_mat(const DScene& g, const Hit& hit, f3 wi, Rng& rng, bool regularize) {
-  gptr<VimgMaterial> m = g.materials + hit.mat;
+template <bool TEX, int MT = -1, class S>
+VD Scatter sample_mat(const S& g, const Hit& hit, f3 wi, Rng& rng, bool regularize) {
+  const auto m = tb_materials(g) + hit.mat;
   const uint32_t type = MT >= 0 ? uint32_t(MT) : m->type;
   const f3 dir_in = -wi;
   uint32_t lobe = LOBE_NONE;
@@ -1005,7 +1051,7 @@
     const float metallic = pc.metallic;
     float roughness = pc.roughness;
     const float ng_in = dot(hit.ng, dir_in);
-    gptr<DMaterial> dm = g.dmaterials + hit.mat;
+    const auto dm = tb_dmaterials(g) + hit.mat;
     const bool scalars = dmat_scalars<TEX>(dm->bits);
     const int reg = regularize ? 1 : 0;
     if (ng_in < 0) {
@@ -1119,14 +1165,14 @@
   if ((1 - (1 - g_h_dot_in * g_h_dot_in) / (eta * eta)) <= 0) return no_scatter();
   return Scatter{refracted, eta, true, true};
 }
-template <bool TEX, int MT = -1>
-VD void eval_pdf_pair(const DScene& g, const Hit& hit, f3 wi, f3 wo, RayCone cone, bool regularize,
+template <bool TEX, int MT = -1, class S>
+VD void eval_pdf_pair(const S& g, const Hit& hit, f3 wi, f3 wo, RayCone cone, bool regularize,
                       f3& f, float& pdf) {
-  gptr<VimgMaterial> m = g.materials + hit.mat;
+  const auto m = tb_materials(g) + hit.mat;
   const uint32_t type = MT >= 0 ? uint32_t(MT) : m->type;
   if (type == VIMG_MAT_LAMBERTIAN) {
     float dot_product = static_cast<float>(sel_max(0.0f, dot(wo, hit.ns)) / kPi);
-    gptr<DMaterial> dm = g.dmaterials + hit.mat;
+    const auto dm = tb_dmaterials(g) + hit.mat;
     const f3 col = (dm->bits & DMAT_COLOUR) ? load3(dm->base) : col_at_ray_hit<TEX>(g, m->tex, wi, cone, hit);
     f = col * dot_product;
     pdf = dot_product;
@@ -1163,25 +1209,27 @@
 VD void tri_light_sample_at(f3 p0, f3 p1, f3 p2, f3 tri_normal, float pdf, f3 look_from, Rng& rng, f3& hit_n, EmitterInfo& info) {
   tri_light_sample_with(p0, p1, p2, tri_normal, tri_normal, tri_normal, pdf, look_from, rng, hit_n, info);
 }
-VD void tri_light_sample(const DScene& g, uint32_t tri, f3 look_from, Rng& rng, f3& le,
+template <class S>
+VD void tri_light_sample(const S& g, uint32_t tri, f3 look_from, Rng& rng, f3& le,
                          EmitterInfo& info) {
-  gptr<DTriShade> ts = g.tri_shade + tri;
+  const auto ts = tb_tri_shade(g) + tri;
   const f3 p0{ts->p[0], ts->p[1], ts->p[2]}, p1{ts->p[3], ts->p[4], ts->p[5]},
       p2{ts->p[6], ts->p[7], ts->p[8]};
-  gptr<VimgMesh> mesh = g.meshes + ts->mesh;
+  const auto mesh = tb_meshes(g) + ts->mesh;
   f3 tri_normal{ts->n[0], ts->n[1], ts->n[2]};
   f3 n0 = tri_normal, n1 = tri_normal, n2 = tri_normal;
   if (mesh->has_normals) {
-    n0 = load3(g.normals + 3 * size_t(ts->i0));
-    n1 = load3(g.normals + 3 * size_t(ts->i1));
-    n2 = load3(g.normals + 3 * size_t(ts->i2));
+    n0 = load3(scn(g).normals + 3 * size_t(ts->i0));
+    n1 = load3(scn(g).normals + 3 * size_t(ts->i1));
+    n2 = load3(scn(g).normals + 3 * size_t(ts->i2));
   }
   f3 hit_n;
-  tri_light_sample_with(p0, p1, p2, n0, n1, n2, g.tri_area_pdf[tri] , look_from,
+  tri_light_sample_with(p0, p1, p2, n0, n1, n2, scn(g).tri_area_pdf[tri] , look_from,
                         rng, hit_n, info);
-  le = mat_emitted(g.materials + mesh->material, info.wi, hit_n);
-}
-VD float tri_surf_pdf(const DScene& g, uint32_t tri) { return g.tri_area_pdf[tri]; }
+  le = mat_emitted(tb_materials(g) + mesh->material, info.wi, hit_n);
+}
+template <class S>
+VD float tri_surf_pdf(const S& g, uint32_t tri) { return scn(g).tri_area_pdf[tri]; }
 VD void sphere_light_sample_at(f3 center, float radius, f3 look_from, Rng& rng, f3& shading_normal, EmitterInfo& info) {
   float rand1 = rand_float(rng);
   float rand2 = rand_float(rng);
@@ -1214,7 +1262,8 @@
     info = EmitterInfo{sampled_dir, pdf, sqrt_f(dist2), G};
   }
 }
-VD float sphere_surf_pdf(gptr<VimgSphere> sp, f3 look_from, f3 point_on_light, f3 dir) {
+template <class SpherePtr>
+VD float sphere_surf_pdf(SpherePtr sp, f3 look_from, f3 point_on_light, f3 dir) {
   const f3 center = load3(sp->center);
   const float radius = sp->radius;
   if (length2(look_from - center) <= radius * radius) {
@@ -1324,16 +1373,16 @@
   le = load3k(g.background.col);
   info = EmitterInfo{wi, pdf, VIMG_INF, 1.f};
 }
-template <bool TEX>
-VD void lights_sample(const DScene& g, f3 look_from, Rng& rng, f3& le, EmitterInfo& info) {
+template <bool TEX, class S>
+VD void lights_sample(const S& g, f3 look_from, Rng& rng, f3& le, EmitterInfo& info) {
   float rnd = rand_float(rng);
-  float sx = rnd * g.num_lights;
-  const int index_obj = clampi(static_cast<int>(sx), 0, static_cast<int>(g.num_lights) - 1);
-  const float prob_obj = 1.f / g.num_lights;
-  gptr<DLight> L = g.dlights + index_obj;
+  float sx = rnd * scn(g).num_lights;
+  const int index_obj = clampi(static_cast<int>(sx), 0, static_cast<int>(scn(g).num_lights) - 1);
+  const float prob_obj = 1.f / scn(g).num_lights;
+  gptr<DLight> L = scn(g).dlights + index_obj;
   const uint32_t kind = L->kind;
   if (kind == 0u) {
-    background_sample<TEX>(g, rng, le, info);
+    background_sample<TEX>(scn(g), rng, le, info);
   } else if (kind == 2u) {
     tri_light_sample(g, L->index, look_from, rng, le, info);
   } else {
@@ -1351,10 +1400,11 @@
   }
   info.pdf *= prob_obj;
 }
-VD float surf_pdf(const DScene& g, uint32_t prim_id, f3 look_from, f3 look_at, f3 dir) {
-  const VimgPrim p = load_prim(g.prims + prim_id);
+template <class S>
+VD float surf_pdf(const S& g, uint32_t prim_id, f3 look_from, f3 look_at, f3 dir) {
+  const VimgPrim p = load_prim(tb_prims(g) + prim_id);
   if (p.type == VIMG_PRIM_TRIANGLE) return tri_surf_pdf(g, p.index);
-  return sphere_surf_pdf(g.spheres + p.index, look_from, look_at, dir);
+  return sphere_surf_pdf(tb_spheres(g) + p.index, look_from, look_at, dir);
 }
 
 VD float balance_heuristic(float pdf1, float pdf2) { return pdf1 / (pdf1 + pdf2); }
diff --git a/v-img_amd/csrc/scene_upload.hip b/v-img_amd/csrc/scene_upload.hip
--- a/v-img_amd/csrc/scene_upload.hip
+++ b/v-img_amd/csrc/scene_upload.hip
@@ -405,6 +405,7 @@
   s->num_vertices = sc->num_vertices;
   s->num_tris = sc->num_tris;
   s->num_spheres = sc->num_spheres;
+  s->num_meshes = sc->num_meshes;
   for (uint32_t i = 0; i < sc->num_meshes; ++i) {
     const VimgMesh& m = sc->meshes[i];
     if (!m.has_normals || m.num_vertices == 0) continue;
@@ -427,6 +428,7 @@
   options_from_env(&s->opt);
   if (const char* e = getenv("VIMG_HIP_QUERY_BLOCKS")) s->query_launch = atoi(e) != 0 ? 1 : 0;
   if (const char* e = getenv("VIMG_HIP_PLAIN")) s->force_general = atoi(e) == 0;
+  if (const char* e = getenv("VIMG_HIP_LDS_TABLES")) s->no_lds_tables = atoi(e) == 0;
   if (s->opt.scheduler != VIMG_OPT_AUTO && (s->opt.scheduler < VIMG_SCHED_LANE || s->opt.scheduler > VIMG_SCHED_CU))
     return fail(VIMG_E_INVALID, "options: unknown scheduler");
   if (s->opt.scheduler != VIMG_OPT_AUTO && s->opt.scheduler != VIMG_SCHED_LANE && s->opt.scheduler != VIMG_SCHED_CU)
diff --git a/v-img_amd/csrc/vimg_hip.hip b/v-img_amd/csrc/vimg_hip.hip
--- a/v-img_amd/csrc/vimg_hip.hip
+++ b/v-img_amd/csrc/vimg_hip.hip
@@ -86,6 +86,7 @@
   const hipStream_t st = r.st;
   float* d_out = r.d_out;
   LaunchCfg c = make_launch(s, p, r.sx, r.sy);
+  if (c.error) return fail(VIMG_E_INVALID, c.error);
   if (prog) {
     c.args.sample_base = prog->base;
     c.args.spp_div = static_cast<float>(prog->base + p->samples);
@@ -96,6 +97,7 @@
   }
   if (int rc = ensure_pool(s, c)) return rc;
   c.args.full_stats = r.stats ? 1u : 0u;
+  drop_unread_tables(s, c, r.stats);
   if (c.args.num_local_tiles == 0 && r.sx < 0) return VIMG_OK;
   HIP_TRY(hipMemsetAsync(s->counter.p, 0, sizeof(unsigned int), st));
   if (r.stats && !(prog && prog->keep_stats)) HIP_TRY(hipMemsetAsync(s->stats.p, 0, sizeof(DeviceStats), st));
```

Result: faster. 15440 Mrays/s, median of 6 (+1.4%).
